# andy-sweet/fcdiff

Hardware: AMD Instinct MI355X
Metric: posterior samples/sec at R=200 ROIs, N=100 subj, 1024 chains; 1/2/4/8 GPUs (higher is better)
Workload: dtype f64

## Files before the change

### fcdiff_amd/csrc/fcd_api.hip

```cpp
#include <new>
#include <stdlib.h>

#include "fcd_common.h"
#include "fcd_fastmath.h"

#ifdef FCD_ABLATE
__device__ int fcd_abl_level[4];
__device__ unsigned long long *fcd_trace_buf;
void fcd_abl_refresh(hipStream_t s) {
    unsigned long long *tp = nullptr;
    if (const char *e = getenv("FCD_TRACE_PTR")) tp = (unsigned long long *)strtoull(e, nullptr, 0);
    (void)hipMemcpyToSymbolAsync(HIP_SYMBOL(fcd_trace_buf), &tp, sizeof(tp), 0, hipMemcpyHostToDevice, s);
    int v[4] = {0, 0, 0, 0};
    if (const char *e = getenv("FCD_ABL_F")) v[0] = atoi(e);
    if (const char *e = getenv("FCD_ABL_PANEL")) v[1] = atoi(e);
    if (const char *e = getenv("FCD_ABL_DIAG")) v[2] = atoi(e);
    if (const char *e = getenv("FCD_TRACE_ROW")) v[3] = atoi(e);
    (void)hipMemcpyToSymbolAsync(HIP_SYMBOL(fcd_abl_level), v, sizeof(v), 0, hipMemcpyHostToDevice, s);
}
#endif

int fcd_ws_reserve(fcd_ctx *ctx, size_t bytes) {
    if (bytes <= ctx->ws_bytes) return FCD_OK;
    FCD_HIP_TRY(hipDeviceSynchronize());
    if (ctx->ws) FCD_HIP_TRY(hipFree(ctx->ws));
    ctx->ws = nullptr;
    ctx->ws_bytes = 0;
    size_t want = bytes < (1u << 20) ? (1u << 20) : bytes;
    FCD_HIP_TRY(hipMalloc(&ctx->ws, want));
    ctx->ws_bytes = want;
    ctx->n_alloc += 1;
    return FCD_OK;
}

int fcd_fsq_reserve(fcd_ctx *ctx, size_t bytes) {
    if (bytes <= ctx->fsq_bytes) return FCD_OK;
    FCD_HIP_TRY(hipDeviceSynchronize());
    if (ctx->fsq) FCD_HIP_TRY(hipFree(ctx->fsq));
    ctx->fsq = nullptr;
    ctx->fsq_bytes = 0;
    FCD_HIP_TRY(hipMalloc(&ctx->fsq, bytes));
    ctx->fsq_bytes = bytes;
    ctx->n_alloc += 1;
    return FCD_OK;
}

int fcd_frec_reserve(fcd_ctx *ctx, size_t bytes) {
    if (bytes <= ctx->frec_bytes) return FCD_OK;
    FCD_HIP_TRY(hipDeviceSynchronize());
    if (ctx->frec) FCD_HIP_TRY(hipFree(ctx->frec));
    ctx->frec = nullptr;
    ctx->frec_bytes = 0;
    FCD_HIP_TRY(hipMalloc(&ctx->frec, bytes));
    ctx->frec_bytes = bytes;
    ctx->n_alloc += 1;
    return FCD_OK;
}

static double knob_env(const char *name) {
    const char *e = getenv(name);
    return (e && *e) ? atof(e) : 0.0;
}

void fcd_prof_begin(fcd_ctx *ctx, int slot, hipStream_t s) {
    if (!ctx->prof_on) return;
    if (ctx->prof_n[slot] >= ctx->prof_cap[slot]) {
        const int cap = ctx->prof_cap[slot] ? ctx->prof_cap[slot] * 2 : 256;
        hipEvent_t *ev = new (std::nothrow) hipEvent_t[2 * cap];
        if (!ev) return;
        for (int i = 0; i < 2 * ctx->prof_cap[slot]; ++i) ev[i] = ctx->prof_ev[slot][i];
        for (int i = 2 * ctx->prof_cap[slot]; i < 2 * cap; ++i)
            if (hipEventCreate(&ev[i]) != hipSuccess) { delete[] ev; return; }
        delete[] ctx->prof_ev[slot];
        ctx->prof_ev[slot] = ev;
        ctx->prof_cap[slot] = cap;
    }
    (void)hipEventRecord(ctx->prof_ev[slot][2 * ctx->prof_n[slot]], s);
}

void fcd_prof_end(fcd_ctx *ctx, int slot, hipStream_t s) {
    if (!ctx->prof_on || ctx->prof_n[slot] >= ctx->prof_cap[slot]) return;
    (void)hipEventRecord(ctx->prof_ev[slot][2 * ctx->prof_n[slot] + 1], s);
    ctx->prof_n[slot] += 1;
}

extern "C" {

int fcd_prof_enable(fcd_ctx *ctx, int on) {
    if (!ctx) return FCD_ERR_ARG;
    ctx->prof_on = on ? 1 : 0;
    for (int i = 0; i < FCD_PROF_SLOTS; ++i) ctx->prof_n[i] = 0;
    return FCD_OK;
}

int fcd_prof_collect(fcd_ctx *ctx, int slot, double *total_ms, int64_t *count) {
    if (!ctx || slot < 0 || slot >= FCD_PROF_SLOTS || !total_ms || !count) return FCD_ERR_ARG;
    double tot = 0.0;
    for (int i = 0; i < ctx->prof_n[slot]; ++i) {
        FCD_HIP_TRY(hipEventSynchronize(ctx->prof_ev[slot][2 * i + 1]));
        float ms = 0.f;
        FCD_HIP_TRY(hipEventElapsedTime(&ms, ctx->prof_ev[slot][2 * i], ctx->prof_ev[slot][2 * i + 1]));
        tot += ms;
    }
    *total_ms = tot;
    *count = ctx->prof_n[slot];
    ctx->prof_n[slot] = 0;
    return FCD_OK;
}

int fcd_abi_version(void) { return FCD_ABI_VERSION; }

const char *fcd_strerror(int code) {
    switch (code) {
        case FCD_OK: return "ok";
        case FCD_ERR_ARG: return "invalid argument (null pointer or non-positive size)";
        case FCD_ERR_SHAPE: return "invalid shape (number of connections must be a triangular number, Nreg >= 2)";
        case FCD_ERR_UNSUPPORTED: return "shape outside what the gfx950 kernels are built for";
        case FCD_ERR_INDEX: return "reference edge id out of range";
        case FCD_ERR_DEVICE: return "a kernel abandoned a device-side wait; the chain state is unusable";
        case FCD_ERR_COMM: return "RCCL: library not found or a call failed";
        default: break;
    }
    if (code > 0) return hipGetErrorString((hipError_t)code);
    return "unknown fcdiff_hip error";
}

const char *fcd_last_message(const fcd_ctx *ctx) { return ctx ? ctx->msg : ""; }

int fcd_ctx_create(fcd_ctx **out) {
    if (!out) return FCD_ERR_ARG;
    *out = nullptr;
    int dev = 0;
    FCD_HIP_TRY(hipGetDevice(&dev));
    hipDeviceProp_t prop;
    FCD_HIP_TRY(hipGetDeviceProperties(&prop, dev));
    fcd_ctx *ctx = new (std::nothrow) fcd_ctx();
    if (!ctx) return (int)hipErrorOutOfMemory;
    ctx->device = dev;
    ctx->num_cu = prop.multiProcessorCount > 0 ? prop.multiProcessorCount : 256;
    ctx->ws = nullptr;
    ctx->ws_bytes = 0;
    ctx->log_tab = nullptr;
    ctx->dev_err = nullptr;
    ctx->f_sure_hint = nullptr;
    ctx->fsq = nullptr;
    ctx->fsq_bytes = 0;
    ctx->frec = nullptr;
    ctx->frec_bytes = 0;
    ctx->noise_rec = nullptr;
    ctx->noise_rec_bytes = 0;
    for (int k = 0; k < FCD_ACC_N; ++k) ctx->sweep_acc[k] = fcd_sweep_acc{{nullptr, nullptr}, 0, 0, 1};
    ctx->count_ws = nullptr;
    ctx->count_ws_bytes = 0;
    ctx->rs_dev = nullptr;
    ctx->rs_J = ctx->rs_smax = 0;
    ctx->rs_max_member = -1;
    ctx->pg_dev = nullptr;
    ctx->pg_J = ctx->pg_P = ctx->pg_umax = ctx->pg_total = ctx->pg_bins_max = 0;
    ctx->pg_max_member = -1;
    ctx->pg_with_rs = 0;
    ctx->pt_dev = nullptr;
    ctx->pt_Q = ctx->pt_U = ctx->pt_umax = 0;
    ctx->pt_with_rs = 0;
    ctx->acc = nullptr;
    ctx->nan_slots = nullptr;
    ctx->dbg = nullptr;
    ctx->comm = nullptr;
    ctx->comm_world = ctx->comm_rank = 0;
    ctx->pool_counts = nullptr;
    ctx->corr_tickets = nullptr;
    ctx->corr_tickets_n = 0;
    ctx->prof_on = 0;
    for (int i = 0; i < FCD_PROF_SLOTS; ++i) {
        ctx->prof_ev[i] = nullptr;
        ctx->prof_n[i] = ctx->prof_cap[i] = 0;
    }
    ctx->msg[0] = 0;
    ctx->n_alloc = 0;
    for (int i = 0; i < FCD_KA_N; ++i) ctx->lds_attr[i] = 0;
    for (int i = 0; i < 3; ++i) ctx->pipe_occ[i] = -1;
    ctx->pipe_grid = ctx->pipe_capacity = 0;
    ctx->knobs.r_path = (int)knob_env("FCD_R_PATH");
    ctx->knobs.r_ub = (int)knob_env("FCD_R_UB");
    ctx->knobs.r_nopad = (int)knob_env("FCD_R_NOPAD");
    ctx->knobs.r_dsplit = (int)knob_env("FCD_R_DSPLIT");
    ctx->knobs.r_coop = (int)knob_env("FCD_R_COOP") == 1 ? 1 : 0;
    ctx->knobs.qr_form = (int)knob_env("FCD_QR_FORM");
    ctx->knobs.r_refill = (int)knob_env("FCD_R_REFILL");
    ctx->knobs.r_tol = knob_env("FCD_R_TOL");
    ctx->knobs.f_tol = knob_env("FCD_F_TOL");
    ctx->knobs.f_form = (int)knob_env("FCD_F_FORM");
    ctx->knobs.f_pack = (int)knob_env("FCD_F_PACK");
    ctx->knobs.corr_form = (int)knob_env("FCD_CORR_FORM");
    ctx->knobs.r_poll_limit = 0;
    ctx->knobs.r_withhold = 0;
    ctx->knobs.f_records = 0;
    ctx->knobs.f_sure = 0;
    ctx->knobs.f_runs = 0;
    ctx->knobs.r_sure = 0;
    ctx->knobs.r_sure_x = 0.0;
    ctx->knobs.partial_chunk = 0;
    ctx->knobs.tangent_chunk = 0;
    ctx->knobs.tally_in_r = (int)knob_env("FCD_TALLY_IN_R");
    ctx->knobs.r_keep_words = (int)knob_env("FCD_R_KEEP_WORDS");
    ctx->r_form_last = 0;
    ctx->n_pack = 0;
    ctx->n_pack_tally = 0;
    ctx->n_r_tally = 0;
    ctx->n_frec_pass = ctx->n_frec_build = ctx->n_fsure_pass = ctx->n_frun_pass = 0;
    ctx->n_rsure_pass = ctx->n_rsure_build = 0;
    int rc = fcd_ws_reserve(ctx, 1u << 20);
    if (rc == FCD_OK) {
        void *pin = nullptr;
        rc = (int)hipHostMalloc(&pin, sizeof(unsigned), hipHostMallocDefault);
        if (rc == FCD_OK) {
            ctx->dev_err = (volatile unsigned *)pin;
            *ctx->dev_err = 0u;
            rc = (int)hipHostMalloc(&pin, 2 * sizeof(unsigned), hipHostMallocDefault);
        }
        if (rc == FCD_OK) {
            ctx->f_sure_hint = (volatile unsigned *)pin;
            ctx->f_sure_hint[0] = 0u;
            ctx->f_sure_hint[1] = 0u;
        }
    }
    if (rc) {
        if (ctx->ws) (void)hipFree(ctx->ws);
        if (ctx->dev_err) (void)hipHostFree((void *)ctx->dev_err);
        if (ctx->f_sure_hint) (void)hipHostFree((void *)ctx->f_sure_hint);
        delete ctx;
        return rc;
    }
    {
        struct { double exp_tab[FCD_EXP_CELLS]; fcd_log_cell log_tab[FCD_LOG_CELLS]; } tabs;
        fcd_fm_make_tables(tabs.exp_tab, tabs.log_tab, exp2, log);
        hipError_t e = hipMalloc(&ctx->log_tab, sizeof(tabs));
        ctx->n_alloc += 1;
        if (e == hipSuccess) e = hipMemcpy(ctx->log_tab, &tabs, sizeof(tabs), hipMemcpyHostToDevice);
        if (e == hipSuccess) e = hipMalloc(&ctx->acc, 8 * sizeof(unsigned long long));
        ctx->n_alloc += 1;
        if (e == hipSuccess) e = hipMemset(ctx->acc, 0, 8 * sizeof(unsigned long long));
        if (e == hipSuccess) e = hipMalloc(&ctx->nan_slots, FCD_NAN_SLOTS * 16 * sizeof(unsigned long long));
        ctx->n_alloc += 1;
        if (e == hipSuccess) e = hipMemset(ctx->nan_slots, 0, FCD_NAN_SLOTS * 16 * sizeof(unsigned long long));
        if (e == hipSuccess) e = hipMalloc(&ctx->dbg, 16 * sizeof(unsigned long long));
        ctx->n_alloc += 1;
        if (e == hipSuccess) e = hipMemset(ctx->dbg, 0, 16 * sizeof(unsigned long long));
        if (e != hipSuccess) {
            fcd_ctx_destroy(ctx);
            return (int)e;
        }
    }
    *out = ctx;
    return FCD_OK;
}

int fcd_ctx_destroy(fcd_ctx *ctx) {
    if (!ctx) return FCD_OK;
    (void)fcd_comm_destroy(ctx);
    if (ctx->pool_counts) (void)hipFree(ctx->pool_counts);
    hipError_t e = hipSuccess;
    if (ctx->ws) e = hipFree(ctx->ws);
    if (ctx->log_tab) (void)hipFree(ctx->log_tab);
    if (ctx->dev_err) (void)hipHostFree((void *)ctx->dev_err);
    if (ctx->f_sure_hint) (void)hipHostFree((void *)ctx->f_sure_hint);
    if (ctx->fsq) (void)hipFree(ctx->fsq);
    if (ctx->frec) (void)hipFree(ctx->frec);
    if (ctx->noise_rec) (void)hipFree(ctx->noise_rec);
    if (ctx->count_ws) (void)hipFree(ctx->count_ws);
    if (ctx->rs_dev) (void)hipFree(ctx->rs_dev);
    if (ctx->pg_dev) (void)hipFree(ctx->pg_dev);
    if (ctx->pt_dev) (void)hipFree(ctx->pt_dev);
    if (ctx->acc) (void)hipFree(ctx->acc);
    if (ctx->nan_slots) (void)hipFree(ctx->nan_slots);
    if (ctx->dbg) (void)hipFree(ctx->dbg);
    if (ctx->corr_tickets) (void)hipFree(ctx->corr_tickets);
    for (int i = 0; i < FCD_PROF_SLOTS; ++i) {
        for (int j = 0; j < 2 * ctx->prof_cap[i]; ++j) (void)hipEventDestroy(ctx->prof_ev[i][j]);
        delete[] ctx->prof_ev[i];
    }
    delete ctx;
    return (int)e;
}

int fcd_ctx_reserve(fcd_ctx *ctx, int64_t Nreg, int64_t U, int64_t G) {
    if (!ctx || Nreg < 2 || U < 1 || G < 1) return fcd_fail(ctx, FCD_ERR_ARG, "fcd_ctx_reserve: bad argument");
    const int64_t GW = (G + 63) / 64;
    size_t need = (size_t)64 * GW * 64 * sizeof(double);
    const size_t en = (size_t)ctx->num_cu * 8 * 8 * sizeof(double);
    if (en > need) need = en;
    const fcd_sweep_plan pl = fcd_sweep_plan_for(ctx, Nreg, U, GW);
    if (pl.ws_bytes > need) need = pl.ws_bytes;
    int rc = fcd_ws_reserve(ctx, need);
    if (rc) return rc;
    if (pl.fsq_bytes) {
        rc = fcd_fsq_reserve(ctx, pl.fsq_bytes);
        if (rc) return rc;
    }
    if (pl.frec_bytes && ctx->knobs.f_records != 1 && fcd_frec_reserve(ctx, pl.frec_bytes) != FCD_OK) (void)hipGetLastError();
    return FCD_OK;
}

int fcd_ctx_set_knob(fcd_ctx *ctx, const char *name, double value) {
    if (!ctx || !name) return FCD_ERR_ARG;
    fcd_knobs &k = ctx->knobs;
    if (!strcmp(name, "r_path")) k.r_path = (int)value;
    else if (!strcmp(name, "r_ub")) k.r_ub = (int)value;
    else if (!strcmp(name, "r_nopad")) k.r_nopad = (int)value;
    else if (!strcmp(name, "r_dsplit")) k.r_dsplit = (int)value;
    else if (!strcmp(name, "r_coop")) k.r_coop = (int)value;
    else if (!strcmp(name, "qr_form")) k.qr_form = (int)value;
    else if (!strcmp(name, "r_refill")) k.r_refill = (int)value;
    else if (!strcmp(name, "r_tol")) k.r_tol = value;
    else if (!strcmp(name, "f_tol")) k.f_tol = value;
    else if (!strcmp(name, "f_form")) k.f_form = (int)value;
    else if (!strcmp(name, "f_pack")) k.f_pack = (int)value;
    else if (!strcmp(name, "f_records")) k.f_records = (int)value;
    else if (!strcmp(name, "f_sure")) k.f_sure = (int)value;
    else if (!strcmp(name, "f_runs")) k.f_runs = (int)value;
    else if (!strcmp(name, "r_sure")) k.r_sure = (int)value;
    else if (!strcmp(name, "r_sure_x")) k.r_sure_x = value;
    else if (!strcmp(name, "corr_form")) k.corr_form = (int)value;
    else if (!strcmp(name, "partial_chunk")) k.partial_chunk = (int)value;
    else if (!strcmp(name, "tangent_chunk")) k.tangent_chunk = (int)value;
    else if (!strcmp(name, "tally_in_r")) k.tally_in_r = (int)value;
    else if (!strcmp(name, "r_keep_words")) k.r_keep_words = (int)value;
    else if (!strcmp(name, "r_poll_limit")) k.r_poll_limit = (int)value;
    else if (!strcmp(name, "r_withhold")) k.r_withhold = (int)value;
    else return fcd_fail(ctx, FCD_ERR_ARG, "fcd_ctx_set_knob: unknown knob");
    return FCD_OK;
}

int fcd_ctx_check(fcd_ctx *ctx) {
    if (!ctx) return FCD_ERR_ARG;
    if (ctx->dev_err && *ctx->dev_err == 2u)
        return fcd_fail(ctx, FCD_ERR_DEVICE, "fcd_site_harmonize: a site id outside 0..B-1 reached the device");
    if (ctx->dev_err && *ctx->dev_err)
        return fcd_fail(ctx, FCD_ERR_DEVICE, "a device-side wait of the pipelined r pass was abandoned: the chain state is unusable");
    return FCD_OK;
}

int fcd_ctx_clear_error(fcd_ctx *ctx) {
    if (!ctx) return FCD_ERR_ARG;
    if (ctx->dev_err) *ctx->dev_err = 0u;
    if (ctx->acc) FCD_HIP_TRY(hipMemset(ctx->acc, 0, 8 * sizeof(unsigned long long)));
    if (ctx->nan_slots) FCD_HIP_TRY(hipMemset(ctx->nan_slots, 0, FCD_NAN_SLOTS * 16 * sizeof(unsigned long long)));
    if (ctx->corr_tickets && ctx->corr_tickets_n > 0)
        FCD_HIP_TRY(hipMemset(ctx->corr_tickets, 0, (size_t)ctx->corr_tickets_n * sizeof(unsigned)));
    return FCD_OK;
}

int fcd_ctx_stat(const fcd_ctx *ctx, const char *name, int64_t *out) {
    if (!ctx || !name || !out) return FCD_ERR_ARG;
    if (!strcmp(name, "n_alloc")) *out = ctx->n_alloc;
    else if (!strcmp(name, "ws_bytes")) *out = (int64_t)ctx->ws_bytes;
    else if (!strcmp(name, "fsq_bytes")) *out = (int64_t)ctx->fsq_bytes;
    else if (!strcmp(name, "r_form_last")) *out = ctx->r_form_last;
    else if (!strcmp(name, "pack_launches")) *out = ctx->n_pack;
    else if (!strcmp(name, "tally_f_in_pack")) *out = ctx->n_pack_tally;
    else if (!strcmp(name, "tally_f_in_r")) *out = ctx->n_r_tally;
    else if (!strcmp(name, "tally_in_r_max_rounds")) *out = R_TALLY_MAX_ROUNDS;
    else if (!strcmp(name, "f_rec_passes")) *out = ctx->n_frec_pass;
    else if (!strcmp(name, "f_rec_builds")) *out = ctx->n_frec_build;
    else if (!strcmp(name, "f_rec_bytes")) *out = (int64_t)ctx->frec_bytes;
    else if (!strcmp(name, "f_rec_min_sweeps")) *out = F_REC_MIN_SWEEPS;
    else if (!strcmp(name, "f_sure_passes")) *out = ctx->n_fsure_pass;
    else if (!strcmp(name, "f_run_passes")) *out = ctx->n_frun_pass;
    else if (!strcmp(name, "r_sure_passes")) *out = ctx->n_rsure_pass;
    else if (!strcmp(name, "r_sure_builds")) *out = ctx->n_rsure_build;
    else if (!strcmp(name, "r_sure_sites") || !strcmp(name, "r_sure_exceptions")) {
        unsigned long long v[16];
        FCD_HIP_TRY(hipMemcpy(v, ctx->dbg, sizeof(v), hipMemcpyDeviceToHost));
        *out = (int64_t)v[!strcmp(name, "r_sure_sites") ? 8 : 9];
    }
    else if (!strcmp(name, "pipe_grid")) *out = ctx->pipe_grid;
    else if (!strcmp(name, "pipe_capacity")) *out = ctx->pipe_capacity;
    else if (!strcmp(name, "comm_world")) *out = ctx->comm ? ctx->comm_world : 0;
    else if (!strcmp(name, "dev_err")) *out = ctx->dev_err ? (int64_t)*ctx->dev_err : 0;
    else if (!strcmp(name, "f_repeats") || !strcmp(name, "r_exact_rows") || !strcmp(name, "f_sure_tiles") || !strcmp(name, "f_sure_fallbacks")) {
        unsigned long long v[8];
        FCD_HIP_TRY(hipMemcpy(v, ctx->dbg, sizeof(v), hipMemcpyDeviceToHost));
        *out = (int64_t)v[name[0] == 'r' ? 1 : !strcmp(name, "f_repeats") ? 0 : !strcmp(name, "f_sure_tiles") ? 2 : 3];
    }
    else return FCD_ERR_ARG;
    return FCD_OK;
}

int64_t fcd_N_to_C(int64_t Nreg) { return fcd_tri(Nreg); }

int64_t fcd_C_to_N(int64_t C) {
    if (C < 1) return FCD_ERR_SHAPE;
    int64_t n = (int64_t)((sqrt(8.0 * (double)C + 1.0) - 1.0) * 0.5) + 1;
    while (fcd_tri(n) > C) --n;
    while (fcd_tri(n + 1) <= C) ++n;
    return fcd_tri(n) == C ? n : (int64_t)FCD_ERR_SHAPE;
}

int64_t fcd_nm_to_c(int64_t n, int64_t m) { return fcd_tri(n) + m; }

int fcd_c_to_nm(int64_t c, int64_t *n, int64_t *m) {
    if (c < 0 || !n || !m) return FCD_ERR_ARG;
    int nn, mm;
    fcd_edge_to_pair(c, nn, mm);
    *n = nn;
    *m = mm;
    return FCD_OK;
}

int64_t fcd_f_run_count(int64_t Nreg) { return Nreg < 2 ? (int64_t)FCD_ERR_SHAPE : fpr_runs((Nreg + 1) / 2); }

int fcd_f_run_locate(int64_t Nreg, int64_t t, int64_t *out9) {
    if (Nreg < 2 || Nreg > (1 << 20) || !out9 || t < 0 || t >= fpr_runs((Nreg + 1) / 2)) return FCD_ERR_ARG;
    const fpr_run R = fpr_locate((int)t, (int)Nreg);
    const int64_t v[9] = {R.n0, R.mb, R.cnt0, R.cnt1, R.tile0, R.ntile, R.cr0, R.cr1, fpr_philox_blocks(R)};
    for (int i = 0; i < 9; ++i) out9[i] = v[i];
    return FCD_OK;
}

}
```

### fcdiff_amd/csrc/fcd_common.h

```cpp
#pragma once
#include <hip/hip_runtime.h>
#include <stdint.h>
#include <stdio.h>
#include <string.h>

#include "../../include/fcdiff_hip.h"

#define FCD_PROF_SLOTS 4
#define FCD_PROF_LIK 0
#define FCD_PROF_F 1
#define FCD_PROF_RSTEP 2
#define FCD_PROF_PACK 3

struct fcd_knobs {
    int r_path;
    int r_ub;
    int r_nopad;
    int r_refill;
    int qr_form;
    int r_coop;
    int r_dsplit;
    double r_tol;
    double f_tol;
    int r_poll_limit;
    int r_withhold;
    int corr_form;
    int f_form;
    int f_pack;
    int f_records;
    int f_sure;
    int f_runs;
    int tally_in_r;
    int partial_chunk;
    int tangent_chunk;
    int r_keep_words;
    int r_sure;
    double r_sure_x;
};

enum { FCD_KA_F_GENERIC = 0, FCD_KA_F_COND, FCD_KA_F_DIFF, FCD_KA_F_PAIR, FCD_KA_F_PAIR_T = FCD_KA_F_PAIR + 4,
       FCD_KA_F_PAIR_R = FCD_KA_F_PAIR_T + 4, FCD_KA_F_PAIR_S = FCD_KA_F_PAIR_R + 4,
       FCD_KA_F_PAIR_BIG = FCD_KA_F_PAIR_S + 4, FCD_KA_R_STEP = FCD_KA_F_PAIR_BIG + 4, FCD_KA_R_PIPE = FCD_KA_R_STEP + 4, FCD_KA_CORR = FCD_KA_R_PIPE + 4, FCD_KA_COMPONENTS = FCD_KA_CORR + 1,
       FCD_KA_GLM = FCD_KA_COMPONENTS + 1,
       FCD_KA_PARTIAL = FCD_KA_GLM + 12,
       FCD_KA_EIGH = FCD_KA_PARTIAL + 1,
       FCD_KA_N = FCD_KA_EIGH + 1 };

#define FCD_NAN_SLOTS 256

enum { FCD_ACC_PAIR, FCD_ACC_COUNT, FCD_ACC_COANOMALY, FCD_ACC_REGION_SET, FCD_ACC_PATIENT_GROUP, FCD_ACC_PATIENT_TRAIT, FCD_ACC_N };
struct fcd_sweep_acc {
    uint32_t *buf[2];
    int64_t nreg, u, every;
};

struct fcd_ctx {
    int device;
    int num_cu;
    void *ws;
    size_t ws_bytes;
    fcd_knobs knobs;
    long long n_alloc;
    size_t lds_attr[FCD_KA_N];
    int pipe_occ[3];
    size_t pipe_occ_shmem[3];
    int pipe_occ_threads[3];
    int64_t pipe_grid;
    int64_t pipe_capacity;
    int r_form_last;
    long long n_pack;
    long long n_pack_tally;
    long long n_r_tally;
    long long n_frec_pass;
    long long n_frec_build;
    long long n_fsure_pass;
    long long n_frun_pass;
    long long n_rsure_pass;
    long long n_rsure_build;
    volatile unsigned *f_sure_hint;
    void *log_tab;
    volatile unsigned *dev_err;
    void *acc;
    void *nan_slots;
    void *comm;
    int comm_world, comm_rank;
    void *pool_counts;
    void *dbg;
    void *corr_tickets;
    size_t corr_tickets_n;
    void *fsq;
    size_t fsq_bytes;
    void *frec;
    size_t frec_bytes;
    void *noise_rec;
    size_t noise_rec_bytes;
    fcd_sweep_acc sweep_acc[FCD_ACC_N];
    void *count_ws;
    size_t count_ws_bytes;
    void *rs_dev;
    int64_t rs_J, rs_smax, rs_max_member;
    void *pg_dev;
    int64_t pg_J, pg_P, pg_umax, pg_max_member;
    int64_t pg_total, pg_bins_max;
    int pg_with_rs;
    void *pt_dev;
    int64_t pt_Q, pt_U, pt_umax;
    int pt_with_rs;
    int prof_on;
    hipEvent_t *prof_ev[FCD_PROF_SLOTS];
    int prof_n[FCD_PROF_SLOTS];
    int prof_cap[FCD_PROF_SLOTS];
    char msg[256];
};

#define FCD_HIP_TRY(expr)                       \
    do {                                        \
        hipError_t e__ = (expr);                \
        if (e__ != hipSuccess) return (int)e__; \
    } while (0)

#define FCD_LAUNCH_CHECK()                      \
    do {                                        \
        hipError_t e__ = hipGetLastError();     \
        if (e__ != hipSuccess) return (int)e__; \
    } while (0)

static inline int fcd_fail(fcd_ctx *ctx, int code, const char *fmt, long long a = 0, long long b = 0) {
    if (ctx) snprintf(ctx->msg, sizeof(ctx->msg), fmt, a, b);
    return code;
}
static inline int fcd_fail_who(fcd_ctx *ctx, int code, const char *who, const char *fmt, long long a = 0, long long b = 0) {
    if (ctx) {
        char tail[192];
        snprintf(tail, sizeof(tail), fmt, a, b);
        snprintf(ctx->msg, sizeof(ctx->msg), "%s: %s", who, tail);
    }
    return code;
}

static inline int fcd_sweep_acc_set(fcd_ctx *ctx, int slot, uint32_t *b0, uint32_t *b1, int64_t Nreg, int64_t U, int64_t every,
                                    const char *msg_together, const char *msg_shape, const char *msg_limit,
                                    const char *msg_every) {
    if (!ctx) return FCD_ERR_ARG;
    if (!b0 && !b1) {
        ctx->sweep_acc[slot] = fcd_sweep_acc{{nullptr, nullptr}, 0, 0, 1};
        return FCD_OK;
    }
    if (!b0 || !b1) return fcd_fail(ctx, FCD_ERR_ARG, msg_together);
    if (Nreg < 2 || U < 1) return fcd_fail(ctx, FCD_ERR_SHAPE, msg_shape, Nreg, U);
    if (msg_limit) return fcd_fail(ctx, FCD_ERR_UNSUPPORTED, msg_limit, Nreg, U);
    if (every < 1) return fcd_fail(ctx, FCD_ERR_ARG, msg_every, every);
    ctx->sweep_acc[slot] = fcd_sweep_acc{{b0, b1}, Nreg, U, every};
    return FCD_OK;
}

static inline int fcd_static_lds_check(fcd_ctx *ctx, const void *fn, int *done) {
    if (*done) return FCD_OK;
    hipFuncAttributes fa;
    hipError_t e = hipFuncGetAttributes(&fa, fn);
    if (e != hipSuccess) return (int)e;
    if (fa.sharedSizeBytes != 0) {
        return fcd_fail(ctx, FCD_ERR_UNSUPPORTED, "kernel carries %lld bytes of static LDS: its table addresses assume none",
                        (long long)fa.sharedSizeBytes);
    }
    *done = 1;
    return FCD_OK;
}

int fcd_comm_allreduce_counts(fcd_ctx *ctx, long long *counts, hipStream_t stream);
int fcd_ws_reserve(fcd_ctx *ctx, size_t bytes);
int fcd_corr_edges_at(fcd_ctx *ctx, const double *ts, int64_t S, int64_t Nreg, int64_t T, int fisher_z, double *out, size_t ws_off,
                      int64_t S_slices, hipStream_t stream);
size_t fcd_corr_edges_ws_bytes(const fcd_ctx *ctx, int64_t S, int64_t Nreg, int64_t T, int64_t S_slices);
struct fcd_shrunk_ws {
    size_t o_redge, o_A, o_live, o_rowF, o_F, o_mean, o_isd, o_q, end;
    int PL, RT, NBT;
};
void fcd_corr_shrunk_plan(int64_t SC, int64_t Nreg, int64_t T, size_t base, fcd_shrunk_ws &w, bool with_A = true);
int fcd_corr_shrunk_at(fcd_ctx *ctx, const double *x, int64_t Sc, int64_t Nreg, int64_t T, const int32_t *n_frames, int64_t s0,
                       int64_t S_call, int shrink_mode, double shrink_value, const fcd_shrunk_ws &w, size_t edges_off, double *A,
                       double *alpha, int32_t *info, hipStream_t stream);
int fcd_fsq_reserve(fcd_ctx *ctx, size_t bytes);
int fcd_frec_reserve(fcd_ctx *ctx, size_t bytes);
static inline int fcd_lds_attr(fcd_ctx *ctx, int slot, const void *fn, size_t shmem) {
    if (shmem <= 64 * 1024 || shmem <= ctx->lds_attr[slot]) return FCD_OK;
    hipError_t e = hipFuncSetAttribute(fn, hipFuncAttributeMaxDynamicSharedMemorySize, (int)shmem);
    if (e != hipSuccess) return (int)e;
    ctx->lds_attr[slot] = shmem;
    return FCD_OK;
}
struct fcd_tally_f {
    const uint8_t *f_state;
    int64_t C, G;
    int GW;
    unsigned long long *acc;
    uint32_t *cnt_f;
};
constexpr int R_TALLY_MAX_ROUNDS = 5;
struct fcd_geo;
template <typename T>
int fcd_pair_tally_launch(fcd_ctx *ctx, const uint8_t *f_state, const uint64_t *r_bits, int64_t Nreg, int64_t U, int64_t G,
                          const fcd_geo &g, T *acc, bool accumulate, hipStream_t s);
int fcd_count_ws_reserve(fcd_ctx *ctx, int64_t Nreg, int64_t U, int64_t G);
int fcd_count_ws_grow(fcd_ctx *ctx, size_t bytes);
int fcd_count_tally_launch(fcd_ctx *ctx, const uint64_t *r_bits, int64_t Nreg, int64_t U, int64_t G, const fcd_geo &g,
                           uint32_t *hist_patient, uint32_t *hist_region, hipStream_t s);
int fcd_coanomaly_tally_launch(fcd_ctx *ctx, const uint64_t *r_bits, int64_t Nreg, int64_t U, int64_t G, const fcd_geo &g,
                               uint32_t *region_pairs, uint32_t *patient_pairs, hipStream_t s);
int fcd_region_set_ws_reserve(fcd_ctx *ctx, int64_t Nreg, int64_t U, int64_t G);
int fcd_region_set_tally_launch(fcd_ctx *ctx, const uint64_t *r_bits, int64_t Nreg, int64_t U, int64_t G, const fcd_geo &g,
                                uint32_t *hist_set, uint32_t *hist_prev, hipStream_t s);
int fcd_patient_group_ws_reserve(fcd_ctx *ctx, int64_t Nreg, int64_t U, int64_t G);
int fcd_patient_group_tally_launch(fcd_ctx *ctx, const uint64_t *r_bits, int64_t Nreg, int64_t U, int64_t G, const fcd_geo &g,
                                   uint32_t *hist_group, uint32_t *hist_joint, hipStream_t s);
int fcd_patient_trait_ws_reserve(fcd_ctx *ctx, int64_t Nreg, int64_t U, int64_t G);
int fcd_patient_trait_tally_launch(fcd_ctx *ctx, const uint64_t *r_bits, int64_t Nreg, int64_t U, int64_t G, const fcd_geo &g,
                                   uint32_t *trait_hist, int64_t *trait_sum, hipStream_t s);
void fcd_prof_begin(fcd_ctx *ctx, int slot, hipStream_t s);
void fcd_prof_end(fcd_ctx *ctx, int slot, hipStream_t s);

#define FCD_H_LNGAMMA 0
#define FCD_H_LNPI0 3
#define FCD_H_LNPI1 4

#define FCD_KIND_INIT_F 0u
#define FCD_KIND_INIT_R 1u
#define FCD_KIND_F 2u
#define FCD_KIND_R 3u

__host__ __device__ static inline int64_t fcd_tri(int64_t n) { return n * (n - 1) / 2; }

__host__ __device__ static inline void fcd_edge_to_pair(int64_t c, int &n, int &m) {
    int64_t nn = (int64_t)((sqrt(8.0 * (double)c + 1.0) - 1.0) * 0.5) + 1;
    while (fcd_tri(nn) > c) --nn;
    while (fcd_tri(nn + 1) <= c) ++nn;
    n = (int)nn;
    m = (int)(c - fcd_tri(nn));
}

__host__ __device__ static inline int64_t fcd_pair_to_edge(int n, int m, int mode) {
    if (mode == FCD_EDGE_REFERENCE || n > m) return fcd_tri(n) + m;
    return fcd_tri(m) + n;
}

struct fcd_u4 {
    uint32_t x, y, z, w;
};

__host__ __device__ static inline fcd_u4 fcd_philox(uint32_t c0, uint32_t c1, uint32_t c2, uint32_t c3,
                                                    uint32_t k0, uint32_t k1) {
#pragma unroll
    for (int r = 0; r < 10; ++r) {
        uint64_t p0 = (uint64_t)0xD2511F53u * c0;
        uint64_t p1 = (uint64_t)0xCD9E8D57u * c2;
        uint32_t n0 = (uint32_t)(p1 >> 32) ^ c1 ^ k0;
        uint32_t n1 = (uint32_t)p1;
        uint32_t n2 = (uint32_t)(p0 >> 32) ^ c3 ^ k1;
        uint32_t n3 = (uint32_t)p0;
        c0 = n0; c1 = n1; c2 = n2; c3 = n3;
        k0 += 0x9E3779B9u;
        k1 += 0xBB67AE85u;
    }
    return fcd_u4{c0, c1, c2, c3};
}

__host__ __device__ static inline double fcd_u53(uint32_t hi, uint32_t lo) {
    uint64_t w = ((uint64_t)hi << 32) | lo;
    return (double)(w >> 11) * (1.0 / 9007199254740992.0);
}

__host__ __device__ static inline double fcd_u32(uint32_t w) { return (double)w * (1.0 / 4294967296.0); }
__host__ __device__ static inline uint32_t fcd_word(const fcd_u4 &x, int i) { return i == 0 ? x.x : i == 1 ? x.y : i == 2 ? x.z : x.w; }

__host__ __device__ static inline double fcd_site_uniform(uint64_t seed, uint32_t idx, uint32_t chain,
                                                          uint32_t sweep, uint32_t kind, int half) {
    fcd_u4 x = fcd_philox(idx, chain, sweep, kind, (uint32_t)seed, (uint32_t)(seed >> 32));
    return half ? fcd_u53(x.z, x.w) : fcd_u53(x.x, x.y);
}

__device__ static inline int fcd_draw_f(double a0, double a1, double a2, double x) {
    double mx = fmax(a0, fmax(a1, a2));
    double e0 = exp(a0 - mx), e1 = exp(a1 - mx), e2 = exp(a2 - mx);
    double t = x * ((e0 + e1) + e2);
    return (t < e0) ? 0 : ((t < e0 + e1) ? 1 : 2);
}

#define FCD_DRAW_F_MARGIN 1e-6f
__host__ __device__ static inline float fcd_draw_f_eta(float delta) { return expm1f(2.0f * delta) * 1.001f + 2e-5f; }
__device__ static inline int fcd_draw_f_fast(double b1, double b2, double x, float eta, float floor_rel, bool *amb) {
    const double mx = fmax(0.0, fmax(b1, b2));
    const float e0 = __expf((float)(0.0 - mx)), e1 = __expf((float)(b1 - mx)), e2 = __expf((float)(b2 - mx));
    const float s = (e0 + e1) + e2;
    const float t = (float)x * s;
    const float m = 2.0f * eta * (s - 1.0f) + floor_rel * s;
    *amb = !(fabsf(t - e0) >= m && fabsf(t - (e0 + e1)) >= m);
    return (t < e0) ? 0 : ((t < e0 + e1) ? 1 : 2);
}
__device__ static inline int fcd_draw_f_fast32(float bf1, float bf2, float xf, float eta, float floor_rel, bool *amb) {
    const float mx = fmaxf(0.f, fmaxf(bf1, bf2));
    const float e0 = __expf(0.f - mx), e1 = __expf(bf1 - mx), e2 = __expf(bf2 - mx);
    const float s = (e0 + e1) + e2;
    const float t = xf * s;
    const float m = 2.0f * eta * (s - 1.0f) + floor_rel * s;
    *amb = !(fabsf(t - e0) >= m && fabsf(t - (e0 + e1)) >= m);
    return (t < e0) ? 0 : ((t < e0 + e1) ? 1 : 2);
}
__device__ static inline bool fcd_draw_f_sure(float bf1, float bf2, float xf, float eta, int *k) {
    const float mx = fmaxf(0.f, fmaxf(bf1, bf2)), mn = fminf(0.f, fminf(bf1, bf2));
    const float mid = ((bf1 + bf2) - mx) - mn;
    *k = (bf2 >= mx) ? 2 : ((bf1 >= mx) ? 1 : 0);
    return (mx - mid) - eta > 15.01f && xf > 1e-6f && xf < 0.999999f;
}
__host__ __device__ static inline float fcd_f32_sum_err(int n_terms, float B) { return (float)(n_terms + 1) * 5.97e-8f * 1.01f * B; }
__host__ __device__ static inline float fcd_f32_offset_err(float cm, float B) { return 2.0f * 5.97e-8f * 1.01f * (cm + B); }

__device__ static inline double fcd_logit(double x) { return log(x / (1.0 - x)); }
__device__ static inline int fcd_draw_r(double s0, double s1, double x) { return fcd_logit(x) < (s1 - s0) ? 1 : 0; }
#define FCD_LOGIT_FAST_ERR 2e-5
__device__ static inline double fcd_logit_fast(double x) {
    const float a = __log2f((float)x), b = __log2f((float)(1.0 - x));
    return (double)((a - b) * 0.69314718f);
}

__device__ static inline double fcd_wave_sum(double v) {
#pragma unroll
    for (int o = 32; o > 0; o >>= 1) v += __shfl_xor(v, o, 64);
    return v;
}

__device__ static inline uint32_t fcd_sel_mask(uint32_t a, uint32_t b, uint64_t mask) {
    uint32_t out;
    asm("v_cndmask_b32 %0, %1, %2, %3" : "=v"(out) : "v"(a), "v"(b), "s"(mask));
    return out;
}

__host__ __device__ static inline uint64_t fcd_active_mask(int w, int64_t G) {
    const int64_t rem = G - (int64_t)w * 64;
    return rem >= 64 ? ~0ull : ((1ull << rem) - 1ull);
}

#ifdef __HIPCC__
constexpr int R_NB = 16;
__device__ __forceinline__ uint2 spread2(uint32_t x16) {
    uint32_t lo = x16 & 0xFFu, hi = (x16 >> 8) & 0xFFu;
    lo = (lo | (lo << 12)) & 0x000F000Fu;
    hi = (hi | (hi << 12)) & 0x000F000Fu;
    lo = (lo | (lo << 6)) & 0x03030303u;
    hi = (hi | (hi << 6)) & 0x03030303u;
    return make_uint2(lo, hi);
}
__device__ __forceinline__ uint64_t fcd_lane_word(uint64_t v, int j) {
    const uint32_t lo = (uint32_t)__builtin_amdgcn_readlane((int)(uint32_t)v, j);
    const uint32_t hi = (uint32_t)__builtin_amdgcn_readlane((int)(uint32_t)(v >> 32), j);
    return ((uint64_t)hi << 32) | lo;
}
__device__ __forceinline__ uint2 fcd_r_pair_bytes(const uint64_t *__restrict__ r_bits, int Nreg, int U, int w, int u, int b,
                                                  int lane) {
    const int ml = b * R_NB + (lane & (R_NB - 1));
    const uint64_t mine = r_bits[((int64_t)w * Nreg + (ml < Nreg ? ml : Nreg - 1)) * U + u];
    uint32_t v = 0;
#pragma unroll
    for (int j = 0; j < R_NB; ++j) {
        const int m = b * R_NB + j;
        v |= (m < Nreg ? (uint32_t)((fcd_lane_word(mine, j) >> lane) & 1ull) : 0u) << j;
    }
    return spread2(v);
}

template <int CTRL>
__device__ __forceinline__ uint32_t fcd_dpp_u32(uint32_t v) {
    return (uint32_t)__builtin_amdgcn_update_dpp(0, (int)v, CTRL, 0xF, 0xF, false);
}
__device__ __forceinline__ uint32_t fcd_wave_sum4(const uint32_t (&p)[4], int lane) {
    const bool b0 = lane & 1, b1 = lane & 2;
    const uint32_t x01 = (b0 ? p[1] : p[0]) + fcd_dpp_u32<0xB1>(b0 ? p[0] : p[1]);
    const uint32_t x23 = (b0 ? p[3] : p[2]) + fcd_dpp_u32<0xB1>(b0 ? p[2] : p[3]);
    uint32_t y = (b1 ? x23 : x01) + fcd_dpp_u32<0x4E>(b1 ? x01 : x23);
    y += fcd_dpp_u32<0x124>(y);
    y += fcd_dpp_u32<0x128>(y);
    y += __shfl_xor(y, 16, 64);
    y += __shfl_xor(y, 32, 64);
    return y;
}

template <int WAVES>
__device__ __forceinline__ void fcd_tally_f_block(const fcd_tally_f &a, int lin, int nblk, unsigned long long (*red)[3]) {
    const uint8_t *__restrict__ f_state = a.f_state;
    uint32_t *cnt_f = a.cnt_f;
    const int64_t C = a.C, G = a.G;
    const int GW = a.GW;
    const int lane = threadIdx.x & 63, wave = __builtin_amdgcn_readfirstlane((int)(threadIdx.x >> 6));
    const int sub = lane & 3, wrow = lane >> 2;
    unsigned long long tot1 = 0, tot2 = 0, n_edges = 0;
    const int own_e = ((lane * 11) >> 5) & 3, own_j = lane - 3 * own_e;
    constexpr int TE = 4;
    for (int64_t c0 = ((int64_t)lin * WAVES + wave) * TE; c0 < C; c0 += (int64_t)nblk * WAVES * TE) {
        const int ne = (int)(C - c0 < TE ? C - c0 : TE);
        const bool owner = cnt_f && lane < 3 * ne;
        uint32_t old = 0;
        if (owner) old = cnt_f[c0 * 3 + lane];
        uint32_t s1 = 0, s2 = 0;
        for (int wg = 0; wg < GW; wg += 16) {
            const int w = wg + wrow;
            uint4 vv[TE];
#pragma unroll
            for (int t = 0; t < TE; ++t) {
                const int64_t c = (c0 + t < C) ? c0 + t : C - 1;
                vv[t] = *reinterpret_cast<const uint4 *>(f_state + ((int64_t)(w < GW ? w : 0) * C + c) * 64 + sub * 16);
            }
            const uint32_t act = (w < GW) ? (uint32_t)(fcd_active_mask(w, G) >> (sub * 16)) & 0xFFFFu : 0u;
            uint32_t p[TE];
#pragma unroll
            for (int t = 0; t < TE; ++t) {
                uint4 v = vv[t];
                if (act != 0xFFFFu) {
                    v.x &= (((act & 15u) * 0x00204081u) & 0x01010101u) * 0xFFu;
                    v.y &= ((((act >> 4) & 15u) * 0x00204081u) & 0x01010101u) * 0xFFu;
                    v.z &= ((((act >> 8) & 15u) * 0x00204081u) & 0x01010101u) * 0xFFu;
                    v.w &= ((((act >> 12) & 15u) * 0x00204081u) & 0x01010101u) * 0xFFu;
                }
                const uint32_t ones = __popc(v.x & 0x01010101u) + __popc(v.y & 0x01010101u) + __popc(v.z & 0x01010101u) +
                                      __popc(v.w & 0x01010101u);
                const uint32_t twos = __popc(v.x & 0x02020202u) + __popc(v.y & 0x02020202u) + __popc(v.z & 0x02020202u) +
                                      __popc(v.w & 0x02020202u);
                p[t] = ones | (twos << 16);
            }
            const uint32_t s = fcd_wave_sum4(p, lane);
            s1 += s & 0xFFFFu;
            s2 += s >> 16;
        }
#pragma unroll
        for (int t = 0; t < TE; ++t) {
            if (t < ne) {
                tot1 += (uint32_t)__builtin_amdgcn_readlane((int)s1, t);
                tot2 += (uint32_t)__builtin_amdgcn_readlane((int)s2, t);
            }
        }
        const uint32_t ones = __shfl(s1, own_e, 64), twos = __shfl(s2, own_e, 64);
        const uint32_t add = own_j == 0 ? (uint32_t)G - ones - twos : (own_j == 1 ? ones : twos);
        n_edges += (unsigned long long)ne;
        if (owner) cnt_f[c0 * 3 + lane] = old + add;
    }
    if (!a.acc) return;
    if (lane == 0) {
        red[wave][0] = n_edges * (unsigned long long)G - tot1 - tot2;
        red[wave][1] = tot1;
        red[wave][2] = tot2;
    }
    __syncthreads();
    if (threadIdx.x < 3) {
        unsigned long long t = 0;
        for (int q = 0; q < WAVES; ++q) t += red[q][threadIdx.x];
        if (t) {
            const unsigned long long old = atomicAdd(&a.acc[1 + threadIdx.x], t);
            asm volatile("" ::"v"(old));
        }
    }
    __syncthreads();
}
#endif

struct fcd_geo {
    int64_t C;
    int GW;
};

static inline int fcd_geo_check(fcd_ctx *ctx, int64_t Nreg, int64_t U, int64_t G, int64_t chain0, fcd_geo &g) {
    if (!ctx) return FCD_ERR_ARG;
    if (Nreg < 2 || U < 1 || G < 1)
        return fcd_fail(ctx, FCD_ERR_SHAPE, "need Nreg >= 2, U >= 1, G >= 1 (Nreg=%lld, U=%lld)", Nreg, U);
    if (Nreg > 46340 || U > (1 << 20) || G > (1ll << 31) || chain0 < 0 || chain0 + G > (1ll << 32))
        return fcd_fail(ctx, FCD_ERR_UNSUPPORTED, "shape out of range (Nreg=%lld, G=%lld)", Nreg, G);
    g.C = fcd_tri(Nreg);
    g.GW = (int)((G + 63) / 64);
    if (g.GW > 65535) return fcd_fail(ctx, FCD_ERR_UNSUPPORTED, "G=%lld exceeds 65535 chain words per launch", G);
    if ((Nreg + 1) / 2 * U > (1ll << 32) || (g.C + 1) / 2 > (1ll << 32))
        return fcd_fail(ctx, FCD_ERR_UNSUPPORTED, "site index exceeds the 32-bit counter word");
    return FCD_OK;
}

enum { FCD_F_GENERIC = 0, FCD_F_PAIR = 1, FCD_F_PAIRX = 2, FCD_F_DIFF = 3 };
constexpr int FP_EC = 8;
constexpr int FT_W = FP_EC / 2;
__host__ __device__ static inline int64_t fpt_tiles(int64_t i) {
    const int64_t j = i >> 1;
    return (i & 1) ? (j + 1) * (j + 1) : j * (j + 1);
}
constexpr int FR_W = 4 * FT_W;
constexpr int FR_WAVES = 8;
struct fpr_run {
    int n0, mb;
    int cnt0, cnt1;
    int tile0, ntile;
    int64_t cr0, cr1;
};
__host__ __device__ static inline int64_t fpr_runs(int64_t i) {
    const int64_t q = i >> 3;
    return 4 * q * (q + 1) + (i & 7) * (q + 1);
}
__host__ __device__ static inline fpr_run fpr_locate(int t, int Nreg) {
    int q = (int)((sqrtf((float)t + 1.f) - 1.f) * 0.5f);
    while ((int64_t)4 * (q + 1) * (q + 2) <= t) ++q;
    while ((int64_t)4 * q * (q + 1) > t) --q;
    const int rem = t - 4 * q * (q + 1);
    const int i = 8 * q + rem / (q + 1);
    fpr_run R;
    R.n0 = 2 * i;
    R.mb = FR_W * (rem % (q + 1));
    const int c0 = R.n0 - R.mb, c1 = R.n0 + 1 - R.mb;
    R.cnt0 = c0 < FR_W ? c0 : FR_W;
    R.cnt1 = R.n0 + 1 < Nreg ? (c1 < FR_W ? c1 : FR_W) : 0;
    R.tile0 = (int)fpt_tiles(i) + R.mb / FT_W;
    R.ntile = ((c1 + 1 < FR_W ? c1 + 1 : FR_W) + FT_W - 1) / FT_W;
    R.cr0 = ((int64_t)R.n0 * (R.n0 - 1) >> 1) + R.mb;
    R.cr1 = R.cr0 + R.n0;
    return R;
}
__host__ __device__ static inline int fpr_philox_blocks(const fpr_run &R) {
    int n = 0;
    if (R.cnt0 > 0) n += (int)(((R.cr0 + R.cnt0 - 1) >> 2) - (R.cr0 >> 2)) + 1;
    if (R.cnt1 > 0) n += (int)(((R.cr1 + R.cnt1 - 1) >> 2) - (R.cr1 >> 2)) + 1;
    return n;
}
constexpr int F_REC_PIECES = 6;
struct fcd_f_edge_rec {
    double d1, d2;
    float a;
    float b[6];
    float pad;
};
#define FCD_F_SURE_T 16.0
#define FCD_F_SURE_DELTA_CAP 0.03125f
#define FCD_F_SURE_DRIFT 6.0
__host__ __device__ static inline int fcd_f_edge_mode(double c1, double c2, const float *b, float delta, double T) {
    if (!(delta <= FCD_F_SURE_DELTA_CAP)) return -1;
    const double c12 = c1 - c2;
    if (-(c1 + (double)b[1]) > T && -(c2 + (double)b[3]) > T) return 0;
    if (c1 + (double)b[0] > T && c12 + (double)b[4] > T) return 1;
    if (c2 + (double)b[2] > T && -(c12 + (double)b[5]) > T) return 2;
    return -1;
}
__host__ __device__ static inline float fcd_f_edge_delta(double c1, double c2, int NPAIR, float a) {
    const float cm = fmaxf((float)fabs(c1), (float)fabs(c2)) * 1.0000002f;
    return fcd_f32_sum_err(NPAIR, a) + fcd_f32_offset_err(cm, a);
}
constexpr size_t F_REC_CAP = (size_t)256 << 20;
constexpr int F_REC_MIN_SWEEPS = 10;
struct fcd_sweep_plan {
    int f_form, f_EC;
    size_t f_shmem;
    int f_NW;
    bool r_blocked, r_idx32;
    int r_ub;
    size_t r_shmem;
    size_t fsq_bytes;
    size_t frec_bytes, frec_edge, frec_votes, f_shmem_rec;
    size_t P[2], f_S, r_S, r_Sn, marks, r_U, ws_bytes;
    size_t rs_bnd, rs_dtab, rs_mword, rs_rowflag, rs_visit, rs_fneq, rs_bytes;
};
fcd_sweep_plan fcd_sweep_plan_for(const fcd_ctx *ctx, int64_t Nreg, int64_t U, int64_t GW);
struct fcd_sweep_call {
    const double *S_B, *lM, *lMf, *lMd, *hyper;
    uint8_t *f_state;
    uint64_t *r_bits;
    int64_t Nreg, U, G, chain0;
    uint64_t seed;
    int edge_mode;
    hipStream_t s;
    fcd_geo g;
    fcd_sweep_plan pl;
};
int fcd_sweep_call_check(fcd_ctx *ctx, fcd_sweep_call &c, bool f_pass, bool r_pass, const char *who);
struct fcd_sweep_step {
    int64_t sweep;
    uint8_t *fsq;
    bool f_packed;
    bool r_packed;
    bool ru_ready;
    const void *f_rec;
    bool sentinels_in_place;
    const fcd_tally_f *tally_f;
    bool tally_f_done;
    bool r_flip;
    bool f_sure;
    bool f_all;
    bool r_sure;
};
int fcd_gibbs_f_pass(fcd_ctx *ctx, const fcd_sweep_call &c, const fcd_sweep_step &st);
int fcd_gibbs_r_pass(fcd_ctx *ctx, const fcd_sweep_call &c, fcd_sweep_step &st);
#define R_SURE_T 16.0
#define R_SURE_X 1e-6
constexpr double R_SURE_MIN_SHARE = 0.9;
int fcd_gibbs_r_bounds_build(fcd_ctx *ctx, const fcd_sweep_call &c);

#ifdef FCD_ABLATE
extern __device__ int fcd_abl_level[4];
#ifdef FCD_TRACE_ONLY
#define FCD_ABL(slot, lvl) false
#else
#define FCD_ABL(slot, lvl) (fcd_abl_level[slot] >= (lvl))
#endif
void fcd_abl_refresh(hipStream_t s);
extern __device__ unsigned long long *fcd_trace_buf;
#define FCD_TRACE(rec, slot)                                                                      \
    do {                                                                                          \
        if (fcd_trace_buf && threadIdx.x == 0) fcd_trace_buf[(size_t)(rec) * 8 + (slot)] = wall_clock64(); \
    } while (0)
#define FCD_TRACE_VAL(rec, slot, v)                                                               \
    do {                                                                                          \
        if (fcd_trace_buf && threadIdx.x == 0) fcd_trace_buf[(size_t)(rec) * 8 + (slot)] = (unsigned long long)(v); \
    } while (0)
#define FCD_TRACE_AT(t0, rec, slot)                                                               \
    do {                                                                                          \
        if (fcd_trace_buf && threadIdx.x == (t0)) fcd_trace_buf[(size_t)(rec) * 8 + (slot)] = wall_clock64(); \
    } while (0)
#define FCD_TRACE_VAL_AT(t0, rec, slot, v)                                                        \
    do {                                                                                          \
        if (fcd_trace_buf && threadIdx.x == (t0)) fcd_trace_buf[(size_t)(rec) * 8 + (slot)] = (unsigned long long)(v); \
    } while (0)
#else
#define FCD_ABL(slot, lvl) false
#define FCD_TRACE(rec, slot) do { } while (0)
#define FCD_TRACE_VAL(rec, slot, v) do { } while (0)
#define FCD_TRACE_AT(t0, rec, slot) do { } while (0)
#define FCD_TRACE_VAL_AT(t0, rec, slot, v) do { } while (0)
static inline void fcd_abl_refresh(hipStream_t) {}
#endif
```

### fcdiff_amd/csrc/fcd_gibbs.hip

```cpp
#include "fcd_common.h"
#include <chrono>

namespace {

__global__ __launch_bounds__(256) void gibbs_init_f(uint8_t *__restrict__ f_state, int64_t C, int GW, uint32_t chain0,
                                                    uint64_t seed) {
    const int lane = threadIdx.x & 63;
    const int64_t item = (int64_t)blockIdx.x * 4 + (threadIdx.x >> 6);
    const int64_t n_pairs = (C + 1) / 2;
    if (item >= n_pairs * GW) return;
    const int w = (int)(item / n_pairs);
    const int64_t pr = item % n_pairs;
    const uint32_t chain = chain0 + (uint32_t)w * 64u + lane;
    const fcd_u4 x = fcd_philox((uint32_t)pr, chain, 0u, FCD_KIND_INIT_F, (uint32_t)seed, (uint32_t)(seed >> 32));
    const int f0 = min((int)(fcd_u53(x.x, x.y) * 3.0), 2);
    const int f1 = min((int)(fcd_u53(x.z, x.w) * 3.0), 2);
    const int64_t c = pr * 2;
    f_state[((int64_t)w * C + c) * 64 + lane] = (uint8_t)f0;
    if (c + 1 < C) f_state[((int64_t)w * C + c + 1) * 64 + lane] = (uint8_t)f1;
}

__global__ __launch_bounds__(256) void gibbs_init_r(uint64_t *__restrict__ r_bits, int Nreg, int U, int GW,
                                                    uint32_t chain0, uint64_t seed, double pi) {
    const int lane = threadIdx.x & 63;
// ... 735 lines not shown
#ifdef FCD_ABLATE
    FCD_TRACE_VAL(trec, 4, tr_terms);
    FCD_TRACE_VAL(trec, 5, tr_draw);
    FCD_TRACE_VAL(trec, 6, tr_rest);
#endif
    FCD_TRACE(trec, 3);
}

__global__ __launch_bounds__(64 * FP_EC) void gibbs_f_records_kernel(const double *__restrict__ S_B, const double *__restrict__ lMf,
                                                                     const double *__restrict__ hyper, int Nreg, int U,
                                                                     char *__restrict__ frec, unsigned *__restrict__ any_tile,
                                                                     unsigned *__restrict__ votes, int n_votes) {
    const int NPAIR = (U + 1) >> 1;
    const fpt_tile T = fpt_locate((int)blockIdx.x, Nreg);
    for (int i = (int)(blockIdx.x * blockDim.x + threadIdx.x); i < n_votes; i += (int)(gridDim.x * blockDim.x)) votes[i] = 0u;
    auto has = [&](int e) -> bool { return (e % FT_W) < (e < FT_W ? T.cnt0 : T.cnt1); };
    auto cid = [&](int e) -> int64_t { return (e < FT_W ? T.cr0 : T.cr1) + (e % FT_W); };
    fcd_f4v *dst4 = reinterpret_cast<fcd_f4v *>(frec) + (size_t)blockIdx.x * NPAIR * (FP_EC * F_REC_PIECES);
    for (int ep = threadIdx.x; ep < FP_EC * NPAIR; ep += blockDim.x) {
        const int e = ep / NPAIR, pr = ep - e * NPAIR;
        if (!has(e)) continue;
        const int u = 2 * pr;
        const double2 *su = reinterpret_cast<const double2 *>(lMf + cid(e) * U * 6) + u * 3;
        double2 A[3], B[3];
#pragma unroll
        for (int l = 0; l < 3; ++l) {
            A[l] = su[l];
            B[l] = (u + 1 < U) ? su[3 + l] : make_double2(0.0, 0.0);
        }
#pragma unroll
        for (int s2 = 0; s2 < 8; ++s2)
            if (s2 != 5 && s2 != 7) dst4[(pr * FP_EC + e) * F_REC_PIECES + (s2 < 5 ? s2 : 5)] = fp_pair_piece(A, B, s2);
    }
    const int e = (int)(threadIdx.x >> 6), lane = threadIdx.x & 63;
    __shared__ int open_edges;
    if (threadIdx.x == 0) open_edges = 0;
    __syncthreads();
    if (has(e)) {
        const int64_t c = cid(e);
        const double2 *su = reinterpret_cast<const double2 *>(lMf + c * U * 6) + (lane < U ? lane : 0) * 3;
        const float a = fp_edge_bound(su, lane < U);
        double b[6] = {0.0, 0.0, 0.0, 0.0, 0.0, 0.0};
        bool finite = true;
        if (lane < U) {
#pragma unroll
            for (int l = 0; l < 3; ++l) {
                const double v[3] = {su[l].x, su[l].y, su[l].x - su[l].y};
                finite = finite && isfinite(v[0]) && isfinite(v[1]);
#pragma unroll
                for (int q = 0; q < 3; ++q) {
                    b[2 * q] = l == 0 ? v[q] : fmin(b[2 * q], v[q]);
                    b[2 * q + 1] = l == 0 ? v[q] : fmax(b[2 * q + 1], v[q]);
                }
            }
        }
        finite = __ballot(!finite) == 0ull;
#pragma unroll
        for (int q = 0; q < 6; ++q) b[q] = fcd_wave_sum(b[q]);
        if (lane == 0) {
            fcd_f_edge_rec k = {};
            const double sb0 = S_B[c * 3 + 0];
            k.d1 = S_B[c * 3 + 1] - sb0;
            k.d2 = S_B[c * 3 + 2] - sb0;
            k.a = a;
            const double slack = 8e-15 * (double)a;
#pragma unroll
            for (int q = 0; q < 6; ++q)
                k.b[q] = !finite ? __builtin_nanf("") : (q & 1) ? __double2float_ru(b[q] + slack) : __double2float_rd(b[q] - slack);
            reinterpret_cast<fcd_f_edge_rec *>(frec + (size_t)gridDim.x * NPAIR * (FP_EC * F_REC_PIECES * 16))[c] = k;
            const double c1 = (hyper[FCD_H_LNGAMMA + 1] - hyper[FCD_H_LNGAMMA + 0]) + k.d1;
            const double c2 = (hyper[FCD_H_LNGAMMA + 2] - hyper[FCD_H_LNGAMMA + 0]) + k.d2;
            if (fcd_f_edge_mode(c1, c2, k.b, fcd_f_edge_delta(c1, c2, NPAIR, a), FCD_F_SURE_T - FCD_F_SURE_DRIFT) < 0) open_edges = 1;
        }
    }
    __syncthreads();
    if (threadIdx.x == 0 && (T.cnt0 > 0 || T.cnt1 > 0)) any_tile[open_edges ? 1 : 0] = 1u;
}
__global__ void gibbs_f_hint_kernel(unsigned *__restrict__ any_tile, volatile unsigned *hint, unsigned build, const double *lM,
                                    const double *hyper) {
    const unsigned any = any_tile[0] != 0u ? 1u : 0u, all = (any && any_tile[1] == 0u) ? 1u : 0u;
    any_tile[0] = 0u;
    any_tile[1] = 0u;
    reinterpret_cast<unsigned long long *>(any_tile)[1] = (unsigned long long)(uintptr_t)lM;
    reinterpret_cast<unsigned long long *>(any_tile)[2] = (unsigned long long)(uintptr_t)hyper;
    for (int i = 0; i < 5; ++i) reinterpret_cast<double *>(any_tile)[7 + i] = hyper[i];
    __hip_atomic_store(const_cast<unsigned *>(hint), 4u * build + 2u * all + any, __ATOMIC_RELEASE, __HIP_MEMORY_SCOPE_SYSTEM);
}

constexpr int FPR_AMB = 8;
__device__ __attribute__((noinline)) int fcd_f_run_edge(const char *__restrict__ rec, const fcd_f_edge_rec *__restrict__ ke_p,
                                                        const double *__restrict__ hyper, uint4 Z, int U, uint32_t xw, float margin) {
    const int NPAIR = (U + 1) >> 1, NG = (NPAIR + 7) >> 3;
    auto term = [&](int p, uint32_t slot) -> fcd_f2v {
        const uint32_t s2 = slot >> 1;
        return *reinterpret_cast<const fcd_f2v *>(rec + (size_t)p * (FP_EC * F_REC_PIECES * 16) + (s2 < 5 ? s2 : 5) * 16 + (slot & 1u) * 8);
    };
    fcd_f2v acc = {0.f, 0.f}, acc1 = {0.f, 0.f};
#pragma unroll 1
    for (int g = 0; g < NG; ++g) {
        const uint32_t zs = g == 0 ? Z.x : g == 1 ? Z.y : g == 2 ? Z.z : Z.w;
        const int np = NPAIR - 8 * g;
        if (np >= 8) {
#pragma unroll 1
            for (int p = 0; p < 8; p += 2) {
                const fcd_f2v v0 = term(8 * g + p, (zs >> (4 * p)) & 15u), v1 = term(8 * g + p + 1, (zs >> (4 * p + 4)) & 15u);
                if (g == 0 && p == 0) {
                    acc = v0;
                    acc1 = v1;
                } else {
                    acc += v0;
                    acc1 += v1;
                }
            }
        } else {
#pragma unroll 1
            for (int p = 0; p < np; ++p) acc += term(8 * g + p, (zs >> (4 * p)) & 15u);
        }
    }
    acc += acc1;
    const fcd_f_edge_rec ke = *ke_p;
    const double lg1 = hyper[FCD_H_LNGAMMA + 1] - hyper[FCD_H_LNGAMMA + 0], lg2 = hyper[FCD_H_LNGAMMA + 2] - hyper[FCD_H_LNGAMMA + 0];
    const double c1 = lg1 + ke.d1, c2 = lg2 + ke.d2;
    const float cm = fmaxf((float)fabs(c1), (float)fabs(c2)) * 1.0000002f;
    const float eta = fcd_draw_f_eta(fcd_f32_sum_err(NPAIR, ke.a) + fcd_f32_offset_err(cm, ke.a));
    const float bf1 = (float)c1 + acc.x, bf2 = (float)c2 + acc.y, xf = (float)xw * 2.3283064e-10f;
    bool amb = false;
    int k;
    if (margin > 1.f || __ballot(!fcd_draw_f_sure(bf1, bf2, xf, eta, &k)) != 0ull) k = fcd_draw_f_fast32(bf1, bf2, xf, eta, margin, &amb);
    return k | (__ballot(amb) != 0ull ? FPR_AMB : 0);
}

__device__ __forceinline__ uint32_t fpr_spread16(uint32_t m) {
    m = (m | (m << 8)) & 0x00FF00FFu;
    m = (m | (m << 4)) & 0x0F0F0F0Fu;
    m = (m | (m << 2)) & 0x33333333u;
    return (m | (m << 1)) & 0x55555555u;
}
__device__ __forceinline__ uint2 fpr_row_word(uint32_t K) {
    const uint32_t v = 3u * (K & 0x33333333u) + ((K >> 2) & 0x33333333u);
    uint32_t lo = v & 0xFFFFu, hi = v >> 16;
    lo = (lo | (lo << 8)) & 0x00FF00FFu;
    hi = (hi | (hi << 8)) & 0x00FF00FFu;
    lo = (lo | (lo << 4)) & 0x0F0F0F0Fu;
    hi = (hi | (hi << 4)) & 0x0F0F0F0Fu;
    return make_uint2(lo << 2, hi << 2);
}

__global__ __launch_bounds__(64 * FR_WAVES) void gibbs_f_run_kernel(const double *__restrict__ S_B, const double *__restrict__ lMf,
                                                           const double *__restrict__ hyper, uint8_t *__restrict__ f_state,
                                                           const uint32_t *__restrict__ r_U, int Nreg, int U, int64_t C, int GW,
                                                           uint32_t chain0, uint64_t seed, uint32_t sweep, float margin,
                                                           uint2 *__restrict__ f_S, int NBLK, unsigned long long *__restrict__ dbg,
                                                           const char *__restrict__ frec, const double *__restrict__ lM, int n_tiles,
                                                           unsigned *__restrict__ votes) {
    static_assert(16 % FR_WAVES == 0, "a workgroup's chain words lie in one group of 16");
    static_assert(FR_W == R_NB && FR_W == 16 && FT_W == 4, "a run is one block of the r pass's f words: sixteen columns, four tiles");
    __shared__ uint32_t vote[FR_WAVES];
    const int NPAIR = (U + 1) >> 1;
    const fpr_run R = fpr_locate((int)blockIdx.x, Nreg);
    const int lane = threadIdx.x & 63;
    const int wv = (int)(threadIdx.x >> 6);
    const int w = __builtin_amdgcn_readfirstlane((int)(blockIdx.y * (blockDim.x >> 6)) + wv);
    const size_t rec_tile = (size_t)NPAIR * (FP_EC * F_REC_PIECES * 16);
    const fcd_f_edge_rec *edge_c = reinterpret_cast<const fcd_f_edge_rec *>(frec + (size_t)n_tiles * rec_tile);
    const int lr = (lane >> 4) & 1, lj = lane & (FR_W - 1);
    const bool present = lane < 2 * FR_W && lj < (lr ? R.cnt1 : R.cnt0);
    int mode = -1;
    if (present) {
        const fcd_f_edge_rec k = edge_c[(lr ? R.cr1 : R.cr0) + lj];
        const double c1 = (hyper[FCD_H_LNGAMMA + 1] - hyper[FCD_H_LNGAMMA + 0]) + k.d1;
        const double c2 = (hyper[FCD_H_LNGAMMA + 2] - hyper[FCD_H_LNGAMMA + 0]) + k.d2;
        mode = fcd_f_edge_mode(c1, c2, k.b, fcd_f_edge_delta(c1, c2, NPAIR, k.a), FCD_F_SURE_T);
    }
    const uint32_t pm = (uint32_t)__ballot(present), dm = (uint32_t)__ballot(mode >= 0);
    const uint32_t m1 = (uint32_t)__ballot(mode == 1), m2 = (uint32_t)__ballot(mode == 2);
    uint32_t oe = 0;
    if (w < GW) {
        const uint32_t chain = chain0 + (uint32_t)w * 64u + lane;
        uint32_t out = 0;
#pragma unroll
        for (int r = 0; r < 2; ++r) {
            const int cnt = r ? R.cnt1 : R.cnt0;
            if (cnt == 0) continue;
            const int64_t cr = r ? R.cr1 : R.cr0;
            const int64_t b1 = (cr + cnt - 1) >> 2;
#pragma unroll 1
            for (int64_t b = cr >> 2; b <= b1; ++b) {
                const fcd_u4 rnd = fcd_philox((uint32_t)b, chain, sweep, FCD_KIND_F, (uint32_t)seed, (uint32_t)(seed >> 32));
                const int j0 = (int)(4 * b - cr);
#pragma unroll
                for (int q = 0; q < 4; ++q) {
                    const float xf = (float)fcd_word(rnd, q) * 2.3283064e-10f;
                    const bool bad = !(xf > 1e-6f && xf < 0.999999f);
                    if (bad && j0 + q >= 0 && j0 + q < cnt) out |= 1u << (FR_W * r + j0 + q);
                }
            }
        }
        if (__ballot(out != 0u) != 0ull) {
#pragma unroll
            for (int o = 32; o > 0; o >>= 1) out |= (uint32_t)__shfl_xor((int)out, o, 64);
            oe = (uint32_t)__builtin_amdgcn_readfirstlane((int)out);
        }
        uint32_t K0 = (fpr_spread16(m1 & 0xFFFFu) | (fpr_spread16(m2 & 0xFFFFu) << 1));
        uint32_t K1 = (fpr_spread16(m1 >> 16) | (fpr_spread16(m2 >> 16) << 1));
        const uint32_t X = (pm & ~dm) | oe;
        if (__builtin_expect(X != 0u, 0)) {
            const uint4 *__restrict__ ru = reinterpret_cast<const uint4 *>(r_U) + (int64_t)w * Nreg * 64;
            uint32_t x = X;
#pragma unroll 1
            while (x != 0u) {
                const int e = __builtin_ctz(x);
                x &= x - 1u;
                const int r = e >> 4, j = e & (FR_W - 1);
                const int64_t c = (r ? R.cr1 : R.cr0) + j;
                const char *rec = frec + (size_t)(R.tile0 + j / FT_W) * rec_tile + (size_t)(r * FT_W + j % FT_W) * (F_REC_PIECES * 16);
                const fcd_u4 rnd = fcd_philox((uint32_t)(c >> 2), chain, sweep, FCD_KIND_F, (uint32_t)seed, (uint32_t)(seed >> 32));
                const uint32_t xw = fcd_word(rnd, (int)(c & 3));
                const int n = R.n0 + r, m = R.mb + j;
                const uint4 vn = ru[(uint32_t)(n * 64) + (uint32_t)lane], vm = ru[(uint32_t)(m * 64) + (uint32_t)lane];
                const uint4 Z = make_uint4((vn.x ^ vm.x) | ((vn.x & vm.x) << 2), (vn.y ^ vm.y) | ((vn.y & vm.y) << 2),
                                           (vn.z ^ vm.z) | ((vn.z & vm.z) << 2), (vn.w ^ vm.w) | ((vn.w & vm.w) << 2));
                uint32_t k = (uint32_t)fcd_f_run_edge(rec, edge_c + c, hyper, Z, U, xw, margin);
                if (k & FPR_AMB) {
                    const double lg1 = hyper[FCD_H_LNGAMMA + 1] - hyper[FCD_H_LNGAMMA + 0], lg2 = hyper[FCD_H_LNGAMMA + 2] - hyper[FCD_H_LNGAMMA + 0];
                    k = (uint32_t)fcd_f_exact_edge(lMf + c * U * 6, lg1 + (S_B[c * 3 + 1] - S_B[c * 3 + 0]), lg2 + (S_B[c * 3 + 2] - S_B[c * 3 + 0]),
                                                   Z.x, Z.y, Z.z, Z.w, U, xw);
                    if (lane == 0) atomicAdd(dbg, 1ull);
                    const bool open = (k & FCD_F_OPEN) != 0;
                    k &= 3u;
                    if (__ballot(open) != 0ull) {
                        const uint32_t ka = (uint32_t)fcd_f_abs_edge(lM, S_B, hyper, ru, c, n, m, U, chain, sweep, seed);
                        if (open) k = ka;
                    }
                }
                if (r) K1 = (K1 & ~(3u << (2 * j))) | (k << (2 * j));
                else K0 = (K0 & ~(3u << (2 * j))) | (k << (2 * j));
            }
        }
#pragma unroll
        for (int r = 0; r < 2; ++r) {
            const int cnt = r ? R.cnt1 : R.cnt0;
            if (cnt == 0) continue;
            uint8_t *line = f_state + ((int64_t)w * C + (r ? R.cr1 : R.cr0)) * 64;
            const uint32_t Kr = r ? K1 : K0;
            if (((X >> (FR_W * r)) & 0xFFFFu) == 0u) {
                if ((lane >> 2) < cnt) {
                    const uint32_t v = ((Kr >> (2 * (lane >> 2))) & 3u) * 0x01010101u;
                    reinterpret_cast<uint4 *>(line)[lane] = make_uint4(v, v, v, v);
                }
            } else {
#pragma unroll 1
                for (int j = 0; j < cnt; ++j) (line + j * 64)[(uint32_t)lane] = (uint8_t)((Kr >> (2 * j)) & 3u);
            }
        }
        if (f_S) {
            const bool full = R.n0 + 2 - R.mb >= FR_W;
            if (full) {
                const int jd = R.n0 + 1 - R.mb;
                const uint32_t K0d = jd < FR_W ? K0 | (((K1 >> (2 * (jd - 1))) & 3u) << (2 * jd)) : K0;
                uint2 *word = f_S + (int64_t)w * Nreg * NBLK * 64 + lane;
                word[(int64_t)(R.n0 * NBLK + R.mb / R_NB) * 64] = fpr_row_word(K0d);
                if (R.n0 + 1 < Nreg) word[(int64_t)((R.n0 + 1) * NBLK + R.mb / R_NB) * 64] = fpr_row_word(K1);
            }
#pragma unroll 1
            for (int q = 0; q < R.ntile; ++q) {
                fpt_tile T;
                T.n0 = R.n0;
                T.mb = R.mb + FT_W * q;
                T.cnt0 = min(FT_W, T.n0 - T.mb);
                T.cnt1 = T.n0 + 1 < Nreg ? min(FT_W, T.n0 + 1 - T.mb) : 0;
                T.cr0 = R.cr0 + FT_W * q;
                T.cr1 = R.cr1 + FT_W * q;
                const uint32_t kt = ((K0 >> (8 * q)) & 0xFFu) | (((K1 >> (8 * q)) & 0xFFu) << 8);
                if (full) fpt_write_f_words<false>(T, kt, w, lane, f_S, Nreg, NBLK);
                else fpt_write_f_words<true>(T, kt, w, lane, f_S, Nreg, NBLK);
            }
        }
    }
    uint32_t ot = 0;
#pragma unroll
    for (int q = 0; q < 4; ++q)
        if (oe & (0x000F000Fu << (FT_W * q))) ot |= 1u << q;
    if (lane == 0) vote[wv] = ot;
    __syncthreads();
    if (wv == 0) {
        const uint32_t v = lane < (int)(blockDim.x >> 6) ? vote[lane & (FR_WAVES - 1)] : 0u;
        uint32_t bm = 0;
#pragma unroll
        for (int q = 0; q < 4; ++q)
            if (__ballot((v >> q) & 1u) != 0ull) bm |= 1u << q;
        const int w0 = (int)(blockIdx.y * (blockDim.x >> 6)), wpg = (int)(blockDim.x >> 6);
        const int n_wg = (min(16, GW - (w0 & ~15)) + wpg - 1) / wpg;
        bool last = true;
        if (n_wg > 1) {
            uint32_t all = 0;
            if (lane == 0) {
                unsigned *word = votes + (size_t)blockIdx.x * (size_t)((GW + 15) >> 4) + (size_t)(w0 >> 4);
                const uint32_t mine = 0x10000u | (bm << (4 * ((w0 & 15) / wpg)));
                all = atomicAdd(word, mine) + mine;
                if ((int)(all >> 16) == n_wg) atomicExch(word, 0u);
            }
            all = (uint32_t)__builtin_amdgcn_readfirstlane((int)all);
            last = (int)(all >> 16) == n_wg;
            bm = (all | (all >> 4) | (all >> 8) | (all >> 12)) & 15u;
        }
        uint32_t n_sure = 0, n_back = 0;
#pragma unroll
        for (int q = 0; q < 4; ++q) {
            const uint32_t tm = (0x000F000Fu << (FT_W * q)) & pm;
            if (last && tm != 0u && (tm & ~dm) == 0u) {
                if ((bm >> q) & 1u) n_back += 1;
                else n_sure += 1;
            }
        }
        if (lane == 0) {
            if (n_sure) atomicAdd(dbg + 2, (unsigned long long)n_sure);
            if (n_back) atomicAdd(dbg + 3, (unsigned long long)n_back);
        }
    }
}

template <int EC>
__global__ __launch_bounds__(1024, 8) void gibbs_f_pairx_kernel(const double *__restrict__ S_B, const double *__restrict__ lMf,
                                                                const double *__restrict__ hyper, uint8_t *__restrict__ f_state,
                                                                const uint32_t *__restrict__ r_U, int Nreg, int U, int64_t C,
                                                                int GW, uint32_t chain0, uint64_t seed, uint32_t sweep,
                                                                float margin, uint8_t *__restrict__ fsq,
                                                                unsigned long long *__restrict__ dbg, const double *__restrict__ lM) {
    extern __shared__ __attribute__((aligned(256))) double ptile[];
    const int NPAIR = (U + 1) >> 1, NW16 = (U + 15) >> 4;
    const int64_t c0 = (int64_t)blockIdx.x * EC;
    const int ne = (int)((C - c0 < EC) ? (C - c0) : EC);
    const int lane = threadIdx.x & 63;
    const int w = __builtin_amdgcn_readfirstlane((int)(blockIdx.y * (blockDim.x >> 6) + (threadIdx.x >> 6)));
    int wn, wm;
    fcd_edge_to_pair(c0, wn, wm);
    const uint32_t *__restrict__ ru = r_U + (int64_t)(w < GW ? w : 0) * Nreg * (NW16 <= 4 ? 4 : NW16) * 64;
    const uint32_t ul = (uint32_t)lane;
    const uint32_t sn = NW16 <= 4 ? 256u : (uint32_t)NW16 * 64u, sg = NW16 <= 4 ? 1u : 64u, lo = NW16 <= 4 ? ul * 4u : ul;
    auto ruw = [&](int n, int g) -> uint32_t { return ru[(uint32_t)n * sn + (uint32_t)g * sg + lo]; };
    uint32_t rn_c = ruw(wn, 0), rm_c = ruw(wm, 0);
    float4 *edge_k = reinterpret_cast<float4 *>(reinterpret_cast<char *>(ptile) + (size_t)EC * NPAIR * 128);
    if (threadIdx.x < EC) edge_k[threadIdx.x] = make_float4(0.f, 0.f, 0.f, 0.f);
    __syncthreads();
    {
        const int wv = (int)(threadIdx.x >> 6);
        double2 *scratch = reinterpret_cast<double2 *>(reinterpret_cast<char *>(edge_k) + 128) + wv * (2 * 24);
        fcd_f2v *dst = reinterpret_cast<fcd_f2v *>(ptile);
        const int slot = lane & 15, pl = lane >> 4;
        const int x0 = slot & 1, x1 = (slot >> 1) & 1, a0 = (slot >> 2) & 1, a1 = slot >> 3;
        const bool valid = !((x0 & a0) | (x1 & a1));
        const int l0 = a0 ? 1 : (x0 ? 2 : 0), l1 = a1 ? 1 : (x1 ? 2 : 0);
        const int NG4 = (NPAIR + 3) >> 2;
        const int groups = ne * NG4, nwv = (int)(blockDim.x >> 6);
        const int row_d2 = U * 3;
        const double2 *__restrict__ src = reinterpret_cast<const double2 *>(lMf + c0 * U * 6);
        for (int g0 = wv; g0 < groups; g0 += 2 * nwv) {
            double2 v[2];
            int eq[2][2];
#pragma unroll
            for (int t = 0; t < 2; ++t) {
                const int g = g0 + t * nwv;
                const int gc = g < groups ? g : groups - 1;
                const int e = gc / NG4, q = gc - e * NG4;
                eq[t][0] = e;
                eq[t][1] = q;
                const int i2 = q * 24 + lane;
                if (lane < 24 && i2 < row_d2) {
                    const double *p2 = reinterpret_cast<const double *>(src + (e * row_d2 + i2));
                    v[t] = make_double2(__builtin_nontemporal_load(p2), __builtin_nontemporal_load(p2 + 1));
                } else {
                    v[t] = make_double2(0.0, 0.0);
                }
            }
#pragma unroll
            for (int t = 0; t < 2; ++t)
                if (lane < 24) scratch[t * 24 + lane] = v[t];
            __builtin_amdgcn_fence(__ATOMIC_RELEASE, "wavefront");
            __builtin_amdgcn_wave_barrier();
            __builtin_amdgcn_fence(__ATOMIC_ACQUIRE, "wavefront");
#pragma unroll
            for (int t = 0; t < 2; ++t) {
                const int g = g0 + t * nwv;
                const int pr = eq[t][1] * 4 + pl;
                const double2 va = scratch[t * 24 + pl * 6 + l0], vb = scratch[t * 24 + pl * 6 + 3 + l1];
                fcd_f2v r = {0.f, 0.f};
                if (valid) {
                    r.x = (float)(va.x + vb.x);
                    r.y = (float)(va.y + vb.y);
                }
                if (g < groups && pr < NPAIR) dst[(eq[t][0] * NPAIR + pr) * 16 + slot] = r;
                if (g < groups && lane < 8) {
                    float a = 0.f;
#pragma unroll
                    for (int l = 0; l < 3; ++l) {
                        const double2 q = scratch[t * 24 + lane * 3 + l];
                        a = fmaxf(a, fmaxf((float)fabs(q.x), (float)fabs(q.y)));
                    }
                    atomicAdd(&edge_k[eq[t][0]].w, a * 1.0000002f);
                }
            }
            __builtin_amdgcn_fence(__ATOMIC_RELEASE, "wavefront");
            __builtin_amdgcn_wave_barrier();
            __builtin_amdgcn_fence(__ATOMIC_ACQUIRE, "wavefront");
        }
    }
    __syncthreads();
    const double lg1 = hyper[FCD_H_LNGAMMA + 1] - hyper[FCD_H_LNGAMMA + 0];
    const double lg2 = hyper[FCD_H_LNGAMMA + 2] - hyper[FCD_H_LNGAMMA + 0];
    if ((int)threadIdx.x < ne) {
        const int64_t c = c0 + threadIdx.x;
        const double c1 = lg1 + (S_B[c * 3 + 1] - S_B[c * 3 + 0]), c2 = lg2 + (S_B[c * 3 + 2] - S_B[c * 3 + 0]);
        const float cm = fmaxf((float)fabs(c1), (float)fabs(c2)) * 1.0000002f;
        const float a = edge_k[threadIdx.x].w;
        edge_k[threadIdx.x] = make_float4((float)c1, (float)c2, fcd_draw_f_eta(fcd_f32_sum_err(NPAIR + 1, a) + fcd_f32_offset_err(cm, a)), 0.f);
    }
    __syncthreads();
    if (w >= GW) return;
    if (FCD_ABL(0, 3)) return;
    const uint32_t chain = chain0 + (uint32_t)w * 64u + lane;
    const uint32_t k0 = (uint32_t)seed, k1 = (uint32_t)(seed >> 32);
    fcd_u4 rnd = {0, 0, 0, 0};
    const int NG = (NPAIR + 7) >> 3;
    const uint32_t tile_off = (uint32_t)(uintptr_t)(__attribute__((address_space(3))) char *)ptile;

    for (int e = 0; e < ne; ++e) {
        const int64_t c = c0 + e;
        int nn = wn, nm = wm + 1;
        if (nm == nn) {
            nm = 0;
            nn = (nn + 1 < Nreg) ? nn + 1 : nn;
        }
        const uint32_t tb = __builtin_amdgcn_readfirstlane(tile_off + (uint32_t)(e * NPAIR * 128));
        fcd_f2v acc = {0.f, 0.f}, acc1 = {0.f, 0.f};
        for (int g = 0; g < NG; ++g) {
            const bool last = g + 1 == NG;
            const int pn = last ? nn : wn, pm = last ? nm : wm, pg = last ? 0 : g + 1;
// ... 232 lines not shown
    }
    partial[((int64_t)s * GW + w) * 64 + lane] = acc;
}

__global__ __launch_bounds__(64) void gibbs_rsum_kernel(const uint64_t *__restrict__ r_bits, int64_t NU, int64_t G,
                                                        unsigned int *__restrict__ out) {
    const int w = blockIdx.x, lane = threadIdx.x;
    const uint64_t *rw = r_bits + (int64_t)w * NU;
    unsigned int ones = 0;
    for (int64_t i = blockIdx.y; i < NU; i += gridDim.y) ones += (unsigned int)((rw[i] >> lane) & 1ull);
    const int64_t g = (int64_t)w * 64 + lane;
    if (g < G && ones) atomicAdd(&out[g], ones);
}

__global__ void gibbs_logjoint_fold(const double *__restrict__ partial, int64_t GWx64, int64_t G, double *__restrict__ out) {
    const int64_t g = (int64_t)blockIdx.x * blockDim.x + threadIdx.x;
    if (g >= G) return;
    double acc = 0.0;
    for (int s = 0; s < LJ_SLICES; ++s) acc += partial[(int64_t)s * GWx64 + g];
    out[g] = acc;
}

__global__ void export_f_kernel(const uint8_t *__restrict__ f_state, int64_t C, int64_t G, uint8_t *__restrict__ f) {
    const int64_t i = (int64_t)blockIdx.x * blockDim.x + threadIdx.x;
    if (i >= G * C) return;
    const int64_t g = i / C, c = i % C;
    f[i] = f_state[((g >> 6) * C + c) * 64 + (g & 63)];
}
__global__ void export_r_kernel(const uint64_t *__restrict__ r_bits, int64_t NU, int64_t G, uint8_t *__restrict__ r) {
    const int64_t i = (int64_t)blockIdx.x * blockDim.x + threadIdx.x;
    if (i >= G * NU) return;
    const int64_t g = i / NU, j = i % NU;
    r[i] = (uint8_t)((r_bits[(g >> 6) * NU + j] >> (g & 63)) & 1ull);
}
__global__ void import_f_kernel(const uint8_t *__restrict__ f, int64_t C, int64_t G, int GW, uint8_t *__restrict__ f_state) {
    const int64_t i = (int64_t)blockIdx.x * blockDim.x + threadIdx.x;
    if (i >= (int64_t)GW * C * 64) return;
    const int64_t lane = i & 63, c = (i >> 6) % C, w = (i >> 6) / C;
    const int64_t g = w * 64 + lane;
    f_state[i] = g < G ? f[g * C + c] : 0;
}
__global__ __launch_bounds__(256) void import_r_kernel(const uint8_t *__restrict__ r, int64_t NU, int64_t G, int GW,
                                                       uint64_t *__restrict__ r_bits) {
    const int lane = threadIdx.x & 63;
    const int64_t word = (int64_t)blockIdx.x * 4 + (threadIdx.x >> 6);
    if (word >= (int64_t)GW * NU) return;
    const int64_t w = word / NU, j = word % NU;
    const int64_t g = w * 64 + lane;
    const uint64_t ball = __ballot(g < G ? (r[g * NU + j] != 0) : false);
    if (lane == 0) r_bits[word] = ball;
}

__global__ void philox_uniforms_kernel(const uint32_t *__restrict__ ctr4, int64_t n, uint64_t seed, double *__restrict__ out) {
    const int64_t i = (int64_t)blockIdx.x * blockDim.x + threadIdx.x;
    if (i >= n) return;
    const fcd_u4 x = fcd_philox(ctr4[i * 4 + 0], ctr4[i * 4 + 1], ctr4[i * 4 + 2], ctr4[i * 4 + 3], (uint32_t)seed,
                                (uint32_t)(seed >> 32));
    out[i * 2 + 0] = fcd_u53(x.x, x.y);
    out[i * 2 + 1] = fcd_u53(x.z, x.w);
}

void f_step_geometry(int64_t U, int GW, int &Ec, int &wpb, size_t &shmem) {
    wpb = GW < 16 ? GW : 16;
    const size_t per_edge = (size_t)U * 72;
    int64_t e = (int64_t)(32 * 1024 / per_edge);
    if (e < 1) e = 1;
    if (e > 8) e = 8;
    if (e > 1) e &= ~1ll;
    Ec = (int)e;
    shmem = per_edge * Ec;
}

template <bool COND>
int launch_f(fcd_ctx *ctx, const double *S_B, const double *lM, const double *hyper, uint8_t *f_state,
             const uint64_t *r_bits, int64_t Nreg, int64_t U, int64_t G, const fcd_geo &g, int64_t chain0, uint64_t seed,
             int64_t sweep, double *cond_f, hipStream_t s) {
    int Ec, wpb;
    size_t shmem;
    f_step_geometry(U, g.GW, Ec, wpb, shmem);
    if (shmem > 160 * 1024)
        return fcd_fail(ctx, FCD_ERR_UNSUPPORTED, "f step: one edge's table row (U=%lld patients) exceeds the 160 KiB LDS", U);
    {
        int rc = fcd_lds_attr(ctx, COND ? FCD_KA_F_COND : FCD_KA_F_GENERIC, reinterpret_cast<const void *>(&gibbs_f_kernel<COND>), shmem);
        if (rc) return rc;
    }
    dim3 grid((unsigned)((g.C + Ec - 1) / Ec), (unsigned)((g.GW + wpb - 1) / wpb));
    hipLaunchKernelGGL(gibbs_f_kernel<COND>, grid, dim3(64 * wpb), shmem, s, S_B, lM, hyper, f_state, r_bits, (int)Nreg,
                       (int)U, g.C, g.GW, G, Ec, (uint32_t)chain0, seed, (uint32_t)sweep, cond_f);
    FCD_LAUNCH_CHECK();
    return FCD_OK;
}

}

extern "C" int fcd_gibbs_state_size(int64_t Nreg, int64_t U, int64_t G, size_t *f_bytes, size_t *r_bytes) {
    if (Nreg < 2 || U < 1 || G < 1 || !f_bytes || !r_bytes) return FCD_ERR_ARG;
    const int64_t GW = (G + 63) / 64;
    *f_bytes = (size_t)(GW * fcd_tri(Nreg) * 64);
    *r_bytes = (size_t)(GW * Nreg * U * 8);
    return FCD_OK;
}

extern "C" int fcd_gibbs_init(fcd_ctx *ctx, uint8_t *f_state, uint64_t *r_bits, int64_t Nreg, int64_t U, int64_t G,
                              int64_t chain0, uint64_t seed, double pi, fcd_stream stream) {
    fcd_geo g;
    int rc = fcd_geo_check(ctx, Nreg, U, G, chain0, g);
    if (rc) return rc;
    if (!f_state || !r_bits) return fcd_fail(ctx, FCD_ERR_ARG, "fcd_gibbs_init: null pointer");
    hipStream_t s = (hipStream_t)stream;
    const int64_t items_f = (g.C + 1) / 2 * g.GW;
    hipLaunchKernelGGL(gibbs_init_f, dim3((unsigned)((items_f + 3) / 4)), dim3(256), 0, s, f_state, g.C, g.GW,
                       (uint32_t)chain0, seed);
    FCD_LAUNCH_CHECK();
    const int64_t items_r = (Nreg + 1) / 2 * U * g.GW;
    hipLaunchKernelGGL(gibbs_init_r, dim3((unsigned)((items_r + 3) / 4)), dim3(256), 0, s, r_bits, (int)Nreg, (int)U, g.GW,
                       (uint32_t)chain0, seed, pi);
    FCD_LAUNCH_CHECK();
    return FCD_OK;
}

extern "C" int fcd_gibbs_edge_tables(fcd_ctx *ctx, const double *lM, int64_t Nreg, int64_t U, double *lMf,
                                     fcd_stream stream) {
    if (!ctx || !lM || !lMf) return fcd_fail(ctx, FCD_ERR_ARG, "fcd_gibbs_edge_tables: null pointer");
    if (Nreg < 2 || U < 1) return fcd_fail(ctx, FCD_ERR_SHAPE, "need Nreg >= 2 and U >= 1 (Nreg=%lld, U=%lld)", Nreg, U);
    const int64_t n_items = fcd_tri(Nreg) * U;
    int64_t blocks = (n_items + 255) / 256;
    const int64_t cap = (int64_t)ctx->num_cu * 16;
    if (blocks > cap) blocks = cap;
    hipLaunchKernelGGL(edge_tables_kernel, dim3((unsigned)blocks), dim3(256), 0, (hipStream_t)stream, lM, n_items, lMf);
    FCD_LAUNCH_CHECK();
    return FCD_OK;
}

int fcd_sweep_call_check(fcd_ctx *ctx, fcd_sweep_call &c, bool f_pass, bool r_pass, const char *who) {
    int rc = fcd_geo_check(ctx, c.Nreg, c.U, c.G, c.chain0, c.g);
    if (rc) return rc;
    const bool null = (f_pass && !c.S_B) || !c.lM || !c.hyper || !c.f_state || !c.r_bits;
    if (null || (r_pass && c.edge_mode != FCD_EDGE_REFERENCE && c.edge_mode != FCD_EDGE_SYMMETRIC)) {
        snprintf(ctx->msg, sizeof(ctx->msg), null ? "%s: null pointer" : "%s: bad edge_mode", who);
        return FCD_ERR_ARG;
    }
    if (r_pass && c.edge_mode == FCD_EDGE_REFERENCE && c.Nreg == 2)
        return fcd_fail(ctx, FCD_ERR_INDEX, "reference edge ids: index 1 is out of bounds for axis 0 with size 1 (Nreg=2)");
    c.pl = fcd_sweep_plan_for(ctx, c.Nreg, c.U, c.g.GW);
    return FCD_OK;
}

extern "C" int fcd_gibbs_f_step(fcd_ctx *ctx, const double *S_B, const double *lM, const double *lMf, const double *hyper,
                                uint8_t *f_state, const uint64_t *r_bits, int64_t Nreg, int64_t U, int64_t G,
                                int64_t chain0, uint64_t seed, int64_t sweep, fcd_stream stream) {
    fcd_sweep_call c = {S_B, lM, lMf, nullptr, hyper, f_state, const_cast<uint64_t *>(r_bits) , Nreg, U, G,
                        chain0, seed, FCD_EDGE_SYMMETRIC, (hipStream_t)stream};
    int rc = fcd_sweep_call_check(ctx, c, true, false, "fcd_gibbs_f_step");
    return rc ? rc : fcd_gibbs_f_pass(ctx, c, fcd_sweep_step{sweep});
}

int fcd_gibbs_f_pass(fcd_ctx *ctx, const fcd_sweep_call &c, const fcd_sweep_step &st) {
    const fcd_sweep_plan &pl = c.pl;
    const fcd_geo &g = c.g;
    const int64_t Nreg = c.Nreg, U = c.U;
    hipStream_t s = c.s;
    const int form = c.lMf ? pl.f_form : FCD_F_GENERIC;
    if (form == FCD_F_GENERIC)
        return launch_f<false>(ctx, c.S_B, c.lM, c.hyper, c.f_state, c.r_bits, Nreg, U, c.G, g, c.chain0, c.seed, st.sweep,
                               nullptr, s);
    fcd_abl_refresh(s);
    const int wpb = g.GW < 16 ? g.GW : 16;
    float margin = FCD_DRAW_F_MARGIN;
    if ((float)ctx->knobs.f_tol > margin) margin = (float)ctx->knobs.f_tol;
    int rc;
    if (form == FCD_F_PAIR || form == FCD_F_PAIRX) {
        rc = fcd_ws_reserve(ctx, pl.ws_bytes);
        if (rc) return rc;
        uint32_t *r_U = (uint32_t *)((char *)ctx->ws + pl.r_U);
        if (!st.ru_ready) {
            const int64_t items = (int64_t)g.GW * Nreg * pl.f_NW;
            hipLaunchKernelGGL(pack_ru_kernel, dim3((unsigned)((items + 3) / 4)), dim3(256), 0, s, c.r_bits, (int)Nreg, (int)U,
                               pl.f_NW, g.GW, r_U);
            FCD_LAUNCH_CHECK();
        }
        dim3 grid((unsigned)((g.C + pl.f_EC - 1) / pl.f_EC), (unsigned)((g.GW + wpb - 1) / wpb));
        const bool pt = st.f_packed && form == FCD_F_PAIR;
        if (st.f_rec && (!pt || !pl.frec_bytes || ctx->frec_bytes < pl.frec_bytes))
            return fcd_fail(ctx, FCD_ERR_ARG, "f pass: prebuilt records asked for where the plan has none");
        const size_t f_shmem = st.f_rec ? pl.f_shmem_rec : pl.f_shmem;
        if (st.f_packed && (form != FCD_F_PAIR || !pl.r_blocked || st.fsq))
            return fcd_fail(ctx, FCD_ERR_ARG, "f pass: packed f words asked for where the plan has none");
        uint2 *f_S = pt ? (uint2 *)((char *)ctx->ws + pl.f_S) : nullptr;
        const int NBLK = (int)((Nreg + R_NB - 1) / R_NB);
        if (pt) grid.x = (unsigned)fpt_tiles((Nreg + 1) / 2);
#define FCD_F_ARGS c.S_B, c.lMf, c.hyper, c.f_state, r_U, (int)Nreg, (int)U, g.C, g.GW, (uint32_t)c.chain0, c.seed, (uint32_t)st.sweep, margin, st.fsq
#define FCD_LAUNCH_F(KERN, SLOT, EXTRA)                                                                            \
    do {                                                                                                      \
        rc = fcd_lds_attr(ctx, SLOT, reinterpret_cast<const void *>(&KERN), f_shmem);                         \
        if (rc) return rc;                                                                                    \
        {                                                                                                     \
            static int lds0 = 0;               \
            rc = fcd_static_lds_check(ctx, reinterpret_cast<const void *>(&KERN), &lds0);                     \
            if (rc) return rc;                                                                                \
        }                                                                                                     \
        fcd_prof_begin(ctx, FCD_PROF_F, s);                                                                   \
        hipLaunchKernelGGL(KERN, grid, dim3(64 * wpb), f_shmem, s, FCD_F_ARGS, EXTRA);                        \
        fcd_prof_end(ctx, FCD_PROF_F, s);                                                                     \
    } while (0)
#define FCD_PX (unsigned long long *)ctx->dbg, c.lM
#define FCD_PT f_S, NBLK, (unsigned long long *)ctx->dbg, (const char *)st.f_rec, c.lM
        const bool sure = form == FCD_F_PAIR && pt && st.f_rec && st.f_sure && !(margin > 1.f) && ctx->knobs.f_sure != 1;
        if (sure && ctx->knobs.f_runs != 1 && (st.f_all || ctx->knobs.f_runs == 2)) {
            const int rw = wpb < FR_WAVES ? wpb : FR_WAVES;
            dim3 rgrid((unsigned)fpr_runs((Nreg + 1) / 2), (unsigned)((g.GW + rw - 1) / rw));
            fcd_prof_begin(ctx, FCD_PROF_F, s);
            hipLaunchKernelGGL(gibbs_f_run_kernel, rgrid, dim3(64 * rw), 0, s, c.S_B, c.lMf, c.hyper, c.f_state, r_U, (int)Nreg, (int)U, g.C,
                               g.GW, (uint32_t)c.chain0, c.seed, (uint32_t)st.sweep, margin, f_S, NBLK, (unsigned long long *)ctx->dbg,
                               (const char *)st.f_rec, c.lM, (int)grid.x, (unsigned *)((char *)st.f_rec + pl.frec_votes));
            fcd_prof_end(ctx, FCD_PROF_F, s);
            ctx->n_frec_pass += 1;
            ctx->n_fsure_pass += 1;
            ctx->n_frun_pass += 1;
        } else if (sure) {
            if (pl.f_NW == 1) FCD_LAUNCH_F((gibbs_f_pair_kernel<1, true, true, true>), FCD_KA_F_PAIR_S + 0, FCD_PT);
            else if (pl.f_NW == 2) FCD_LAUNCH_F((gibbs_f_pair_kernel<2, true, true, true>), FCD_KA_F_PAIR_S + 1, FCD_PT);
            else if (pl.f_NW == 3) FCD_LAUNCH_F((gibbs_f_pair_kernel<3, true, true, true>), FCD_KA_F_PAIR_S + 2, FCD_PT);
            else FCD_LAUNCH_F((gibbs_f_pair_kernel<4, true, true, true>), FCD_KA_F_PAIR_S + 3, FCD_PT);
            ctx->n_frec_pass += 1;
            ctx->n_fsure_pass += 1;
        } else if (form == FCD_F_PAIR && pt && st.f_rec) {
            if (pl.f_NW == 1) FCD_LAUNCH_F((gibbs_f_pair_kernel<1, true, true>), FCD_KA_F_PAIR_R + 0, FCD_PT);
            else if (pl.f_NW == 2) FCD_LAUNCH_F((gibbs_f_pair_kernel<2, true, true>), FCD_KA_F_PAIR_R + 1, FCD_PT);
            else if (pl.f_NW == 3) FCD_LAUNCH_F((gibbs_f_pair_kernel<3, true, true>), FCD_KA_F_PAIR_R + 2, FCD_PT);
            else FCD_LAUNCH_F((gibbs_f_pair_kernel<4, true, true>), FCD_KA_F_PAIR_R + 3, FCD_PT);
            ctx->n_frec_pass += 1;
        } else if (form == FCD_F_PAIR && pt) {
            if (pl.f_NW == 1) FCD_LAUNCH_F((gibbs_f_pair_kernel<1, true>), FCD_KA_F_PAIR_T + 0, FCD_PT);
            else if (pl.f_NW == 2) FCD_LAUNCH_F((gibbs_f_pair_kernel<2, true>), FCD_KA_F_PAIR_T + 1, FCD_PT);
            else if (pl.f_NW == 3) FCD_LAUNCH_F((gibbs_f_pair_kernel<3, true>), FCD_KA_F_PAIR_T + 2, FCD_PT);
            else FCD_LAUNCH_F((gibbs_f_pair_kernel<4, true>), FCD_KA_F_PAIR_T + 3, FCD_PT);
        } else if (form == FCD_F_PAIR) {
            if (pl.f_NW == 1) FCD_LAUNCH_F((gibbs_f_pair_kernel<1, false>), FCD_KA_F_PAIR + 0, FCD_PT);
            else if (pl.f_NW == 2) FCD_LAUNCH_F((gibbs_f_pair_kernel<2, false>), FCD_KA_F_PAIR + 1, FCD_PT);
            else if (pl.f_NW == 3) FCD_LAUNCH_F((gibbs_f_pair_kernel<3, false>), FCD_KA_F_PAIR + 2, FCD_PT);
            else FCD_LAUNCH_F((gibbs_f_pair_kernel<4, false>), FCD_KA_F_PAIR + 3, FCD_PT);
        } else {
            if (pl.f_EC == 8) FCD_LAUNCH_F(gibbs_f_pairx_kernel<8>, FCD_KA_F_PAIR_BIG + 0, FCD_PX);
            else if (pl.f_EC == 4) FCD_LAUNCH_F(gibbs_f_pairx_kernel<4>, FCD_KA_F_PAIR_BIG + 1, FCD_PX);
            else if (pl.f_EC == 2) FCD_LAUNCH_F(gibbs_f_pairx_kernel<2>, FCD_KA_F_PAIR_BIG + 2, FCD_PX);
            else FCD_LAUNCH_F(gibbs_f_pairx_kernel<1>, FCD_KA_F_PAIR_BIG + 3, FCD_PX);
        }
#undef FCD_PT
#undef FCD_PX
#undef FCD_LAUNCH_F
#undef FCD_F_ARGS
        FCD_LAUNCH_CHECK();
        return FCD_OK;
    }
    rc = fcd_lds_attr(ctx, FCD_KA_F_DIFF, reinterpret_cast<const void *>(&gibbs_f_diff_kernel), pl.f_shmem);
    if (rc) return rc;
    dim3 grid((unsigned)((g.C + pl.f_EC - 1) / pl.f_EC), (unsigned)((g.GW + wpb - 1) / wpb));
    fcd_prof_begin(ctx, FCD_PROF_F, s);
    hipLaunchKernelGGL(gibbs_f_diff_kernel, grid, dim3(64 * wpb), pl.f_shmem, s, c.S_B, c.lMf, c.hyper, c.f_state, c.r_bits,
                       (int)Nreg, (int)U, g.C, g.GW, pl.f_EC, (uint32_t)c.chain0, c.seed, (uint32_t)st.sweep, margin, c.lM);
    fcd_prof_end(ctx, FCD_PROF_F, s);
    FCD_LAUNCH_CHECK();
    return FCD_OK;
}

extern "C" int fcd_gibbs_mstep(fcd_ctx *ctx, const int64_t *counts, int64_t Nreg, int64_t U, double *hyper,
                               fcd_stream stream) {
    if (!ctx || !counts || !hyper) return fcd_fail(ctx, FCD_ERR_ARG, "fcd_gibbs_mstep: null pointer");
    if (Nreg < 2 || U < 1) return fcd_fail(ctx, FCD_ERR_SHAPE, "need Nreg >= 2 and U >= 1 (Nreg=%lld, U=%lld)", Nreg, U);
    hipLaunchKernelGGL(gibbs_mstep_kernel, dim3(1), dim3(1), 0, (hipStream_t)stream,
                       reinterpret_cast<const long long *>(counts), (double)fcd_tri(Nreg), (double)(Nreg * U), hyper);
    FCD_LAUNCH_CHECK();
    return FCD_OK;
}

static int launch_tally(fcd_ctx *ctx, const uint8_t *f_state, const uint64_t *r_bits, int64_t Nreg, int64_t U, int64_t G,
                        const fcd_geo &g, int64_t *counts, uint32_t *cnt_f, uint32_t *cnt_r, double *hyper, uint32_t *r_U,
                        int ru_words, hipStream_t s, bool f_done = false, uint2 *r_S = nullptr, uint32_t *marks = nullptr) {
    tally_args a;
    a.f_state = f_state; a.r_bits = r_bits;
    a.C = g.C; a.NU = Nreg * U; a.G = G;
    a.GW = g.GW; a.Nreg = (int)Nreg; a.U = (int)U; a.NW = ru_words;
    a.marks = r_U ? marks : nullptr; a.r_S = a.marks ? r_S : nullptr;
    a.NBLK = (int)((Nreg + R_NB - 1) / R_NB);
    a.acc = (counts || hyper) ? (unsigned long long *)ctx->acc : nullptr;
    a.counts_out = reinterpret_cast<unsigned long long *>(counts);
    a.cnt_f = cnt_f; a.cnt_r = cnt_r;
    a.hyper = hyper; a.r_U = r_U;
    int64_t blocks = (g.C + 63) / 64;
    const int64_t cap = (int64_t)ctx->num_cu * 2;
    if (blocks > cap) blocks = cap;
    a.n_f_blocks = f_done ? 0 : (int)blocks;
    {
        int64_t rb = (a.NU + 1023) / 1024;
        if (rb > 64) rb = 64;
        a.n_r_blocks = (int)rb;
        if (rb > a.n_f_blocks) blocks = rb;
    }
    if (r_U) {
        const int64_t n_marks = a.marks ? (int64_t)g.GW * U * a.NBLK : 0;
        int64_t ru_blocks = ((int64_t)g.GW * Nreg * a.NW + (a.r_S ? n_marks : (n_marks + 63) / 64) + 15) / 16;
        if (ru_blocks > ctx->num_cu) ru_blocks = ctx->num_cu;
        blocks += ru_blocks;
    }
    hipLaunchKernelGGL(gibbs_tally_kernel, dim3((unsigned)blocks), dim3(1024), 0, s, a);
    FCD_LAUNCH_CHECK();
    return FCD_OK;
}

extern "C" int fcd_gibbs_tally(fcd_ctx *ctx, const uint8_t *f_state, const uint64_t *r_bits, int64_t Nreg, int64_t U,
                               int64_t G, int64_t *counts, uint32_t *cnt_f, uint32_t *cnt_r, fcd_stream stream) {
    fcd_geo g;
    int rc = fcd_geo_check(ctx, Nreg, U, G, 0, g);
    if (rc) return rc;
    if (!f_state || !r_bits) return fcd_fail(ctx, FCD_ERR_ARG, "fcd_gibbs_tally: null pointer");
    if ((cnt_f == nullptr) != (cnt_r == nullptr)) return fcd_fail(ctx, FCD_ERR_ARG, "fcd_gibbs_tally: cnt_f and cnt_r go together");
    if (!counts && !cnt_f) return FCD_OK;
    return launch_tally(ctx, f_state, r_bits, Nreg, U, G, g, counts, cnt_f, cnt_r, nullptr, nullptr, 0, (hipStream_t)stream);
}

extern "C" int fcd_gibbs_stats(fcd_ctx *ctx, const uint8_t *f_state, const uint64_t *r_bits, int64_t Nreg, int64_t U,
                               int64_t G, int64_t *counts, fcd_stream stream) {
    fcd_geo g;
    int rc = fcd_geo_check(ctx, Nreg, U, G, 0, g);
    if (rc) return rc;
    if (!f_state || !r_bits || !counts) return fcd_fail(ctx, FCD_ERR_ARG, "fcd_gibbs_stats: null pointer");
    return launch_tally(ctx, f_state, r_bits, Nreg, U, G, g, counts, nullptr, nullptr, nullptr, nullptr, 0, (hipStream_t)stream);
}

extern "C" int fcd_gibbs_accumulate(fcd_ctx *ctx, const uint8_t *f_state, const uint64_t *r_bits, int64_t Nreg,
                                    int64_t U, int64_t G, uint32_t *cnt_f, uint32_t *cnt_r, fcd_stream stream) {
    fcd_geo g;
    int rc = fcd_geo_check(ctx, Nreg, U, G, 0, g);
    if (rc) return rc;
    if (!f_state || !r_bits || !cnt_f || !cnt_r) return fcd_fail(ctx, FCD_ERR_ARG, "fcd_gibbs_accumulate: null pointer");
    return launch_tally(ctx, f_state, r_bits, Nreg, U, G, g, nullptr, cnt_f, cnt_r, nullptr, nullptr, 0, (hipStream_t)stream);
}

static int acc_launch_pair(fcd_ctx *ctx, const fcd_sweep_call &c, const fcd_geo &g, const fcd_sweep_acc &a, hipStream_t s) {
    return fcd_pair_tally_launch<uint32_t>(ctx, c.f_state, c.r_bits, c.Nreg, c.U, c.G, g, a.buf[0], true, s);
}
static int acc_launch_count(fcd_ctx *ctx, const fcd_sweep_call &c, const fcd_geo &g, const fcd_sweep_acc &a, hipStream_t s) {
    return fcd_count_tally_launch(ctx, c.r_bits, c.Nreg, c.U, c.G, g, a.buf[0], a.buf[1], s);
}
static int acc_launch_coanomaly(fcd_ctx *ctx, const fcd_sweep_call &c, const fcd_geo &g, const fcd_sweep_acc &a, hipStream_t s) {
    return fcd_coanomaly_tally_launch(ctx, c.r_bits, c.Nreg, c.U, c.G, g, a.buf[0], a.buf[1], s);
}
static int acc_launch_region_set(fcd_ctx *ctx, const fcd_sweep_call &c, const fcd_geo &g, const fcd_sweep_acc &a, hipStream_t s) {
    return fcd_region_set_tally_launch(ctx, c.r_bits, c.Nreg, c.U, c.G, g, a.buf[0], a.buf[1], s);
}
static int acc_launch_patient_group(fcd_ctx *ctx, const fcd_sweep_call &c, const fcd_geo &g, const fcd_sweep_acc &a, hipStream_t s) {
    return fcd_patient_group_tally_launch(ctx, c.r_bits, c.Nreg, c.U, c.G, g, a.buf[0], a.buf[1], s);
}
static int acc_launch_patient_trait(fcd_ctx *ctx, const fcd_sweep_call &c, const fcd_geo &g, const fcd_sweep_acc &a, hipStream_t s) {
    return fcd_patient_trait_tally_launch(ctx, c.r_bits, c.Nreg, c.U, c.G, g, a.buf[0], (int64_t *)a.buf[1], s);
}
static const struct {
    const char *msg_shape;
    int (*launch)(fcd_ctx *, const fcd_sweep_call &, const fcd_geo &, const fcd_sweep_acc &, hipStream_t);
    int (*reserve)(fcd_ctx *, int64_t Nreg, int64_t U, int64_t G);
} SWEEP_ACC[FCD_ACC_N] = {
    {"fcd_gibbs_run: the attached pair accumulator was made for Nreg=%lld, U=%lld", acc_launch_pair, nullptr},
    {"fcd_gibbs_run: the attached count accumulator was made for Nreg=%lld, U=%lld", acc_launch_count, fcd_count_ws_reserve},
    {"fcd_gibbs_run: the attached co-anomaly accumulator was made for Nreg=%lld, U=%lld", acc_launch_coanomaly, nullptr},
    {"fcd_gibbs_run: the attached region-set accumulator was made for Nreg=%lld, U=%lld", acc_launch_region_set,
     fcd_region_set_ws_reserve},
    {"fcd_gibbs_run: the attached patient-group accumulator was made for Nreg=%lld, U=%lld", acc_launch_patient_group,
     fcd_patient_group_ws_reserve},
    {"fcd_gibbs_run: the attached patient-trait accumulator was made for Nreg=%lld, U=%lld", acc_launch_patient_trait,
     fcd_patient_trait_ws_reserve},
};

static int fcd_f_sure_hint_wait(fcd_ctx *ctx, hipStream_t s, bool &any, bool &all) {
    const unsigned build = (unsigned)(ctx->n_frec_build & 0x3fffffff);
    const auto t0 = std::chrono::steady_clock::now();
    unsigned v = *ctx->f_sure_hint;
    for (unsigned spin = 1; (v >> 2) != build; ++spin, v = *ctx->f_sure_hint) {
        if ((spin & 1023u) == 0 && std::chrono::steady_clock::now() - t0 > std::chrono::seconds(2)) {
            FCD_HIP_TRY(hipStreamSynchronize(s));
            v = *ctx->f_sure_hint;
            if ((v >> 2) != build) return fcd_fail(ctx, FCD_ERR_DEVICE, "f pass: the record build left no hint");
            break;
        }
    }
    any = (v & 1u) != 0u;
    all = (v & 2u) != 0u;
    return FCD_OK;
}
static int fcd_r_sure_hint_wait(fcd_ctx *ctx, hipStream_t s, bool &share, bool &any) {
    const unsigned build = (unsigned)(ctx->n_rsure_build & 0x3fffffff);
    const auto t0 = std::chrono::steady_clock::now();
    unsigned v = ctx->f_sure_hint[1];
    for (unsigned spin = 1; (v >> 2) != build; ++spin, v = ctx->f_sure_hint[1]) {
        if ((spin & 1023u) == 0 && std::chrono::steady_clock::now() - t0 > std::chrono::seconds(2)) {
            FCD_HIP_TRY(hipStreamSynchronize(s));
            v = ctx->f_sure_hint[1];
            if ((v >> 2) != build) return fcd_fail(ctx, FCD_ERR_DEVICE, "r pass: the bound build left no hint");
            break;
        }
    }
    share = (v & 1u) != 0u;
    any = (v & 2u) != 0u;
    return FCD_OK;
}

static int sweep_loop(fcd_ctx *ctx, const fcd_sweep_call &c, int64_t sweep0, int64_t n_sweeps, int64_t mstep_every,
                      int64_t accumulate_from, int64_t *counts, uint32_t *cnt_f, uint32_t *cnt_r, double *hyper_m,
                      unsigned acc_mask) {
    if (n_sweeps < 0 || sweep0 < 0 || sweep0 + n_sweeps > (1ll << 32))
        return fcd_fail(ctx, FCD_ERR_ARG, "sweep range [%lld, +%lld) outside the 32-bit counter word", sweep0, n_sweeps);
    const fcd_sweep_plan &pl = c.pl;
    const fcd_geo &g = c.g;
    const int64_t Nreg = c.Nreg, U = c.U, G = c.G;
    hipStream_t s = c.s;
    const bool pair_form = c.lMf && (pl.f_form == FCD_F_PAIR || pl.f_form == FCD_F_PAIRX);
    fcd_sweep_step st = {sweep0};
    uint8_t *fsq = nullptr;
    if (pl.fsq_bytes && c.lMf && c.lMd && c.edge_mode == FCD_EDGE_SYMMETRIC) {
        int rc = fcd_fsq_reserve(ctx, pl.fsq_bytes);
        if (rc) return rc;
        fsq = (uint8_t *)ctx->fsq;
    }
    const bool packed_ok = pl.f_form == FCD_F_PAIR && c.lMf && c.lMd && pl.r_blocked && pl.r_idx32 &&
                           c.edge_mode == FCD_EDGE_SYMMETRIC && ctx->knobs.f_pack != 1 && !ctx->knobs.r_refill;
    if (pair_form) {
        int rc = fcd_ws_reserve(ctx, pl.ws_bytes);
        if (rc) return rc;
    }
    const int64_t pt_sweeps = packed_ok ? n_sweeps - 1 : 0;
    bool use_rec = pl.frec_bytes && ctx->knobs.f_records != 1 && pt_sweeps >= (ctx->knobs.f_records == 2 ? 1 : F_REC_MIN_SWEEPS);
    if (use_rec && fcd_frec_reserve(ctx, pl.frec_bytes) != FCD_OK) {
        (void)hipGetLastError();
        use_rec = false;
    }
    bool rec_built = false;
    if (use_rec) {
        ctx->n_frec_build += 1;
        hipLaunchKernelGGL(gibbs_f_records_kernel, dim3((unsigned)fpt_tiles((Nreg + 1) / 2)), dim3(64 * FP_EC), 0, s, c.S_B, c.lMf,
                           c.hyper, (int)Nreg, (int)U, (char *)ctx->frec, (unsigned *)((unsigned long long *)ctx->dbg + 4),
                           (unsigned *)((char *)ctx->frec + pl.frec_votes), (int)((pl.frec_bytes - pl.frec_votes) / sizeof(unsigned)));
        FCD_LAUNCH_CHECK();
        hipLaunchKernelGGL(gibbs_f_hint_kernel, dim3(1), dim3(1), 0, s, (unsigned *)((unsigned long long *)ctx->dbg + 4), ctx->f_sure_hint,
                           (unsigned)(ctx->n_frec_build & 0x3fffffff), c.lM, c.hyper);
        FCD_LAUNCH_CHECK();
        rec_built = true;
    }
    const fcd_knobs &kn = ctx->knobs;
    const bool rs_ok = pl.rs_bytes && kn.r_sure != 1 && !(kn.r_tol > 16.0 * FCD_LOGIT_FAST_ERR) && !kn.r_path && !kn.r_coop &&
                       !kn.r_dsplit;
    int rs_state = 0;
    for (int64_t i = 0; i < n_sweeps; ++i) {
        st.sweep = sweep0 + i;
        st.f_packed = packed_ok && st.r_packed;
        st.fsq = st.f_packed ? nullptr : fsq;
        if (rs_state == 1 && st.f_packed) {
            bool share = false, any = false;
            int rc = fcd_r_sure_hint_wait(ctx, s, share, any);
            if (rc) return rc;
            rs_state = (kn.r_sure == 2 || share) ? 2 : -1;
        }
        if (rec_built && st.f_packed && !st.f_rec) {
            int rc = fcd_f_sure_hint_wait(ctx, s, st.f_sure, st.f_all);
            if (rc) return rc;
            st.f_rec = ctx->frec;
            if (rs_ok && (st.f_sure || kn.r_sure == 2)) {
                rc = fcd_gibbs_r_bounds_build(ctx, c);
                if (rc) return rc;
                rs_state = 1;
            } else {
                rs_state = -1;
            }
        }
        st.r_sure = rs_state == 2 && st.f_packed && st.r_packed;
        int rc = fcd_gibbs_f_pass(ctx, c, st);
        if (rc) return rc;
        const bool last = i + 1 == n_sweeps;
        const bool do_m = mstep_every > 0 && (i + 1) % mstep_every == 0;
        const bool do_a = cnt_f && st.sweep >= accumulate_from;
        fcd_tally_f tf;
        tf.f_state = c.f_state; tf.C = g.C; tf.G = G; tf.GW = g.GW;
        tf.acc = (do_m || (last && counts)) ? (unsigned long long *)ctx->acc : nullptr;
        tf.cnt_f = do_a ? cnt_f : nullptr;
        st.tally_f = (tf.acc || tf.cnt_f) ? &tf : nullptr;
        rc = fcd_gibbs_r_pass(ctx, c, st);
        if (rc) {
            if (tf.acc) (void)hipMemsetAsync(ctx->acc, 0, 8 * sizeof(unsigned long long), s);
            return rc;
        }
        st.sentinels_in_place = pair_form && ctx->r_form_last == 2;
        uint32_t *r_U_next = (pair_form && !last) ? (uint32_t *)((char *)ctx->ws + pl.r_U) : nullptr;
        const bool r_next = packed_ok && r_U_next;
        const bool keep_words = ctx->knobs.r_keep_words == 1;
        uint2 *r_S_next = (r_next && keep_words) ? (uint2 *)((char *)ctx->ws + (st.r_flip ? pl.r_Sn : pl.r_S)) : nullptr;
        int64_t *cts = (last ? counts : nullptr);
        const bool pooled = do_m && ctx->comm != nullptr;
        int64_t *tally_counts = pooled ? (int64_t *)ctx->pool_counts : cts;
        if (do_m || do_a || cts || r_U_next) {
            rc = launch_tally(ctx, c.f_state, c.r_bits, Nreg, U, G, g, tally_counts, do_a ? cnt_f : nullptr, do_a ? cnt_r : nullptr,
                              (do_m && !pooled) ? hyper_m : nullptr, r_U_next, pl.f_NW, s, st.tally_f_done, r_S_next,
                              r_next ? (uint32_t *)((char *)ctx->ws + pl.marks) : nullptr);
            if (rc) {
                if (tf.acc) (void)hipMemsetAsync(ctx->acc, 0, 8 * sizeof(unsigned long long), s);
                return rc;
            }
        }
        if (pooled) {
            rc = fcd_comm_allreduce_counts(ctx, (long long *)ctx->pool_counts, s);
            if (rc) return rc;
            hipLaunchKernelGGL(gibbs_mstep_kernel, dim3(1), dim3(1), 0, s, (const long long *)ctx->pool_counts, (double)g.C,
                               (double)(Nreg * U), hyper_m);
            FCD_LAUNCH_CHECK();
            if (cts) FCD_HIP_TRY(hipMemcpyAsync(cts, ctx->pool_counts, 8 * sizeof(long long), hipMemcpyDeviceToDevice, s));
        } else if (cts && ctx->comm) {
            rc = fcd_comm_allreduce_counts(ctx, (long long *)cts, s);
            if (rc) return rc;
        }
        if (acc_mask && st.sweep >= accumulate_from) {
            for (int k = 0; k < FCD_ACC_N; ++k) {
                const fcd_sweep_acc &a = ctx->sweep_acc[k];
                if (!(acc_mask >> k & 1u) || (st.sweep - accumulate_from) % a.every != 0) continue;
                rc = SWEEP_ACC[k].launch(ctx, c, g, a, s);
                if (rc) return rc;
            }
        }
        st.ru_ready = r_U_next != nullptr;
        st.r_packed = r_next;
        if (r_next && !keep_words) st.r_flip = !st.r_flip;
    }
    return FCD_OK;
}

extern "C" int fcd_gibbs_run(fcd_ctx *ctx, const double *S_B, const double *lM, const double *lMf, const double *lMd,
                             double *hyper, uint8_t *f_state, uint64_t *r_bits, int64_t Nreg, int64_t U, int64_t G,
                             int64_t chain0, uint64_t seed, int64_t sweep0, int64_t n_sweeps, int edge_mode,
                             int64_t mstep_every, int64_t accumulate_from, int64_t *counts, uint32_t *cnt_f, uint32_t *cnt_r,
                             fcd_stream stream) {
    fcd_sweep_call c = {S_B, lM, lMf, lMd, hyper, f_state, r_bits, Nreg, U, G, chain0, seed, edge_mode, (hipStream_t)stream};
    int rc = fcd_sweep_call_check(ctx, c, true, true, "fcd_gibbs_run");
    if (rc) return rc;
    if ((cnt_f == nullptr) != (cnt_r == nullptr)) return fcd_fail(ctx, FCD_ERR_ARG, "fcd_gibbs_run: cnt_f and cnt_r go together");
    if (mstep_every < 0) return fcd_fail(ctx, FCD_ERR_ARG, "fcd_gibbs_run: mstep_every < 0");
    unsigned acc_mask = 0;
    for (int k = 0; k < FCD_ACC_N; ++k) {
        const fcd_sweep_acc &a = ctx->sweep_acc[k];
        if (!a.buf[0]) continue;
        if (a.nreg != Nreg || a.u != U) return fcd_fail(ctx, FCD_ERR_SHAPE, SWEEP_ACC[k].msg_shape, a.nreg, a.u);
        acc_mask |= 1u << k;
    }
    for (int k = 0; k < FCD_ACC_N; ++k) {
        if (!(acc_mask >> k & 1u) || !SWEEP_ACC[k].reserve) continue;
        rc = SWEEP_ACC[k].reserve(ctx, Nreg, U, G);
        if (rc) return rc;
    }
    return sweep_loop(ctx, c, sweep0, n_sweeps, mstep_every, accumulate_from, counts, cnt_f, cnt_r, hyper, acc_mask);
}

extern "C" int fcd_gibbs_sweeps(fcd_ctx *ctx, const double *S_B, const double *lM, const double *lMf, const double *lMd,
                                const double *hyper,
                                uint8_t *f_state, uint64_t *r_bits, int64_t Nreg, int64_t U, int64_t G, int64_t chain0,
                                uint64_t seed, int64_t sweep0, int64_t n_sweeps, int edge_mode, int64_t *counts,
                                fcd_stream stream) {
    fcd_sweep_call c = {S_B, lM, lMf, lMd, hyper, f_state, r_bits, Nreg, U, G, chain0, seed, edge_mode, (hipStream_t)stream};
    int rc = fcd_sweep_call_check(ctx, c, true, true, "fcd_gibbs_sweeps");
    if (rc) return rc;
    rc = sweep_loop(ctx, c, sweep0, n_sweeps, 0, 0, nullptr, nullptr, nullptr, nullptr, 0u);
    if (rc) return rc;
    if (counts && n_sweeps > 0) return fcd_gibbs_stats(ctx, f_state, r_bits, Nreg, U, G, counts, stream);
    return FCD_OK;
}

extern "C" int fcd_gibbs_logjoint(fcd_ctx *ctx, const double *S_B, const double *lM, const double *hyper,
                                  const uint8_t *f_state, const uint64_t *r_bits, int64_t Nreg, int64_t U, int64_t G,
                                  double *out, fcd_stream stream) {
    fcd_geo g;
    int rc = fcd_geo_check(ctx, Nreg, U, G, 0, g);
    if (rc) return rc;
    if (!S_B || !lM || !hyper || !f_state || !r_bits || !out) return fcd_fail(ctx, FCD_ERR_ARG, "fcd_gibbs_logjoint: null pointer");
    const size_t need = (size_t)LJ_SLICES * g.GW * 64 * sizeof(double);
    rc = fcd_ws_reserve(ctx, need);
    if (rc) return rc;
    hipStream_t s = (hipStream_t)stream;
    hipLaunchKernelGGL(gibbs_logjoint_kernel, dim3((unsigned)g.GW, LJ_SLICES), dim3(64), 0, s, S_B, lM, hyper, f_state,
                       r_bits, (int)Nreg, (int)U, g.C, g.GW, (double *)ctx->ws);
    FCD_LAUNCH_CHECK();
    hipLaunchKernelGGL(gibbs_logjoint_fold, dim3((unsigned)((G + 255) / 256)), dim3(256), 0, s, (const double *)ctx->ws,
                       (int64_t)g.GW * 64, G, out);
    FCD_LAUNCH_CHECK();
    return FCD_OK;
}

extern "C" int fcd_gibbs_chain_rsum(fcd_ctx *ctx, const uint64_t *r_bits, int64_t Nreg, int64_t U, int64_t G, uint32_t *out,
                                    fcd_stream stream) {
    fcd_geo g;
    int rc = fcd_geo_check(ctx, Nreg, U, G, 0, g);
    if (rc) return rc;
    if (!r_bits || !out) return fcd_fail(ctx, FCD_ERR_ARG, "fcd_gibbs_chain_rsum: null pointer");
    hipStream_t s = (hipStream_t)stream;
    FCD_HIP_TRY(hipMemsetAsync(out, 0, (size_t)G * sizeof(uint32_t), s));
    const int64_t NU = Nreg * U;
    const int slices = (int)(NU < 64 ? NU : 64);
    hipLaunchKernelGGL(gibbs_rsum_kernel, dim3((unsigned)g.GW, (unsigned)slices), dim3(64), 0, s, r_bits, NU, G, out);
    FCD_LAUNCH_CHECK();
    return FCD_OK;
}

extern "C" int fcd_gibbs_conditionals(fcd_ctx *ctx, const double *S_B, const double *lM, const double *hyper,
                                      const uint8_t *f_state, const uint64_t *r_bits, int64_t Nreg, int64_t U,
                                      int64_t G, int edge_mode, double *cond_f, double *cond_r, fcd_stream stream) {
    fcd_geo g;
    int rc = fcd_geo_check(ctx, Nreg, U, G, 0, g);
    if (rc) return rc;
    if (!S_B || !lM || !hyper || !f_state || !r_bits) return fcd_fail(ctx, FCD_ERR_ARG, "fcd_gibbs_conditionals: null pointer");
    if (edge_mode != FCD_EDGE_REFERENCE && edge_mode != FCD_EDGE_SYMMETRIC)
        return fcd_fail(ctx, FCD_ERR_ARG, "fcd_gibbs_conditionals: edge_mode %lld", edge_mode);
    if (edge_mode == FCD_EDGE_REFERENCE && Nreg == 2 && cond_r)
        return fcd_fail(ctx, FCD_ERR_INDEX, "reference edge ids: index 1 is out of bounds for axis 0 with size 1 (Nreg=2)");
    hipStream_t s = (hipStream_t)stream;
    if (cond_f) {
        rc = launch_f<true>(ctx, S_B, lM, hyper, const_cast<uint8_t *>(f_state), r_bits, Nreg, U, G, g, 0, 0, 0, cond_f, s);
        if (rc) return rc;
    }
    if (cond_r) {
        if (U > 65535 || Nreg > 65535) return fcd_fail(ctx, FCD_ERR_UNSUPPORTED, "fcd_gibbs_conditionals: grid too large");
        hipLaunchKernelGGL(gibbs_cond_r_kernel, dim3((unsigned)U, (unsigned)g.GW, (unsigned)Nreg), dim3(64), 0, s, lM, hyper,
                           f_state, r_bits, (int)Nreg, (int)U, g.C, G, edge_mode, cond_r);
        FCD_LAUNCH_CHECK();
    }
    return FCD_OK;
}

extern "C" int fcd_gibbs_export_state(fcd_ctx *ctx, const uint8_t *f_state, const uint64_t *r_bits, int64_t Nreg,
                                      int64_t U, int64_t G, uint8_t *f, uint8_t *r, fcd_stream stream) {
    fcd_geo g;
    int rc = fcd_geo_check(ctx, Nreg, U, G, 0, g);
    if (rc) return rc;
    if (!f_state || !r_bits || !f || !r) return fcd_fail(ctx, FCD_ERR_ARG, "fcd_gibbs_export_state: null pointer");
    hipStream_t s = (hipStream_t)stream;
    hipLaunchKernelGGL(export_f_kernel, dim3((unsigned)((G * g.C + 255) / 256)), dim3(256), 0, s, f_state, g.C, G, f);
    FCD_LAUNCH_CHECK();
// ... 31 lines not shown
```

### fcdiff_amd/csrc/fcd_gibbs_r.hip

```cpp
#include <stdlib.h>

#include <type_traits>

#include "fcd_common.h"

namespace {


__global__ __launch_bounds__(256) void region_tables_kernel(const double *__restrict__ lM, int Nreg, int U, int mode,
                                                            double *__restrict__ lMd) {
    const int64_t total = (int64_t)U * Nreg * Nreg;
    for (int64_t rec = (int64_t)blockIdx.x * blockDim.x + threadIdx.x; rec < total; rec += (int64_t)gridDim.x * blockDim.x) {
        const int m = (int)(rec % Nreg);
        const int n = (int)((rec / Nreg) % Nreg);
        const int u = (int)(rec / ((int64_t)Nreg * Nreg));
        double *o = lMd + rec * 6;
        if (m == n) {
#pragma unroll
            for (int x = 0; x < 6; ++x) o[x] = 0.0;
        } else {
            const double *p = lM + (fcd_pair_to_edge(n, m, mode) * U + u) * 9;
#pragma unroll
            for (int k = 0; k < 3; ++k) {
                o[k * 2 + 0] = p[k * 3 + 2] - p[k * 3 + 0];
// ... 993 lines not shown
                const uint2 fwb = fro[ulane], fwa = (fro - a_back)[ulane];
                const uint2 za = make_uint2(fwa.x | rpb.x, fwa.y | rpb.y), zb = make_uint2(fwb.x | rcur.x, fwb.y | rcur.y);
                const uint32_t ra = pb_off + (uint32_t)(stop * (R_NB / 2) * 288), rb = pb_off + (uint32_t)((R_NB + stop) * (R_NB / 2) * 288);
                vstop = (e + (four(za, ra, 0) + four(za, ra, 4))) + (four(zb, rb, 0) + four(zb, rb, 4));
            }
            if (__ballot(fabs(vstop) < a.tol) != 0ull) {
                uint32_t ul3 = ulane;
                asm volatile("" : "+v"(ul3));
                vstop += pipe_exact_corr((uint32_t)((B0 + stop) * ((U + 1) >> 1) + (u >> 1)), a.chain0 + (uint32_t)w * 64u + ul3,
                                         a.sweep, a.seed, u & 1);
            }
            const uint32_t t = vstop > 0.0 ? 1u : 0u;
            fresh |= t << stop;
            const int sh = 8 * ((stop >> 1) & 3) + (stop & 1);
            if ((stop >> 1) < 4) rcur.x = (rcur.x & ~(1u << sh)) | (t << sh);
            else rcur.y = (rcur.y & ~(1u << sh)) | (t << sh);
            i0 = stop + 1;
        }
#pragma unroll
        for (int i = 0; i < R_NB; ++i) {
            if (i < nb) {
                const uint64_t ball = __ballot((fresh >> i) & 1u);
                if (lane == 0) a.r_bits[((int64_t)w * Nreg + B0 + i) * U + u] = ball;
                __hip_atomic_store(reinterpret_cast<unsigned long long *>(const_cast<double *>(Pw) + i * 64 + ulane), R_SENT,
                                   __ATOMIC_RELAXED, __HIP_MEMORY_SCOPE_AGENT);
            }
        }
        rpb = spread2(fresh);
        FCD_TRACE_AT(tr0, trec, 2);
        {
            uint32_t ul2 = ulane;
            asm volatile("" : "+v"(ul2));
            unsigned long long *dst = reinterpret_cast<unsigned long long *>(a.r_Sn + (wu * NBLK + b) * 64 + ul2);
            const unsigned long long val = (unsigned long long)rpb.x | ((unsigned long long)rpb.y << 32);
            __hip_atomic_store(dst, val, __ATOMIC_RELAXED, __HIP_MEMORY_SCOPE_AGENT);
        }
        asm volatile("s_waitcnt vmcnt(0)" ::: "memory");
        if (lane == 0 && !a.withhold) __hip_atomic_store(a.flags + wu * NBLK + b, 1u, __ATOMIC_RELAXED, __HIP_MEMORY_SCOPE_AGENT);
        FCD_TRACE_AT(tr0, trec, 4);
        __builtin_amdgcn_s_setprio(0);
    }
}

template <int UB, int WPE>
__global__ __launch_bounds__(1024, WPE) void gibbs_r_pipe_kernel(const r_step_args a, volatile unsigned *err) {
    extern __shared__ __attribute__((aligned(16))) double smem[];
    const int blk = blockIdx.x;
    if (blk < a.nD) {
        if (a.tf.f_state) fcd_tally_f_block<16>(a.tf, blk, a.nD, reinterpret_cast<unsigned long long (*)[3]>(smem));
        const int half = a.dsplit ? blk / a.u_n : -1;
        for (int wg = 0; wg < a.nWG; ++wg) pipe_diag(a, a.u_lo + (a.dsplit ? blk % a.u_n : blk), wg, half, smem, err);
    } else {
        int item = blk - a.nD;
        if (a.npad) {
            if (blk >= a.ncu + a.nD) {
                item -= a.npad;
            } else if (blk >= a.ncu) {
                return;
            }
        }
        const int row = item % R_NB, uc = item / R_NB;
        for (int wg = 0; wg < a.nWG; ++wg) pipe_panel<UB>(a, row, uc, wg, smem, err);
    }
}

template <int UB, int WPE>
__global__ __launch_bounds__(1024, WPE) void gibbs_r_step_kernel(const r_step_args a) {
    extern __shared__ __attribute__((aligned(16))) double smem[];
    const int blk = blockIdx.x;
    if (blk < a.nD) {
        r_role_diag(a, a.s - 1, a.u_lo + blk % a.u_n, blk / a.u_n, smem);
    } else {
        int item = blk - a.nD;
        if (a.npad) {
            if (blk >= a.ncu + a.nD) {
                item -= a.npad;
            } else if (blk >= a.ncu) {
                return;
            }
        }
        const int rows = (a.Nreg - a.s * R_NB < R_NB) ? (a.Nreg - a.s * R_NB) : R_NB;
        const int nUC = (a.u_n + UB - 1) / UB;
        r_role_panel<UB>(a, a.s, item % rows, (item / rows) % nUC, item / (rows * nUC), smem);
    }
}

constexpr int R_WAVES = 4;
__global__ __launch_bounds__(64 * R_WAVES) void gibbs_r_simple(const double *__restrict__ lM, const double *__restrict__ hyper,
                                                               const uint8_t *__restrict__ f_state,
                                                               uint64_t *__restrict__ r_bits, int Nreg, int U, int64_t C,
                                                               uint32_t chain0, uint64_t seed, uint32_t sweep, int mode) {
    extern __shared__ uint64_t sh_r[];
    uint64_t *mask = sh_r;
    double *part = reinterpret_cast<double *>(sh_r + Nreg);
    const int u = blockIdx.x, w = blockIdx.y;
    const int tid = threadIdx.x, lane = tid & 63;
    const int wave = __builtin_amdgcn_readfirstlane(tid >> 6);
    uint64_t *__restrict__ rcol = r_bits + (int64_t)w * Nreg * U + u;
    for (int n = tid; n < Nreg; n += 64 * R_WAVES) mask[n] = rcol[(int64_t)n * U];
    __syncthreads();
    const uint8_t *__restrict__ fw = f_state + (int64_t)w * C * 64 + lane;
    const double *__restrict__ lMu = lM + (int64_t)u * 9;
    const double lnpi0 = hyper[FCD_H_LNPI0], lnpi1 = hyper[FCD_H_LNPI1];
    const uint32_t chain = chain0 + (uint32_t)w * 64u + lane;
    const uint32_t k0 = (uint32_t)seed, k1 = (uint32_t)(seed >> 32);
    fcd_u4 rnd = {0, 0, 0, 0};

    for (int n = 0; n < Nreg; ++n) {
        double s0 = 0.0, s1 = 0.0;
#pragma unroll 4
        for (int m = wave; m < Nreg; m += R_WAVES) {
            const bool valid = (m != n);
            const int64_t c = valid ? fcd_pair_to_edge(n, m, mode) : 0;
            const int k = fw[c * 64];
            const uint32_t bit = (uint32_t)((mask[m] >> lane) & 1ull);
            const double *p = lMu + (c * U) * 9 + k * 3;
            const double v0 = p[bit * 2];
            const double v1 = p[2 - bit];
            s0 += valid ? v0 : 0.0;
            s1 += valid ? v1 : 0.0;
        }
        part[(wave * 2 + 0) * 64 + lane] = s0;
        part[(wave * 2 + 1) * 64 + lane] = s1;
        __syncthreads();
        if (wave == 0) {
            double t0 = part[0 * 64 + lane], t1 = part[1 * 64 + lane];
#pragma unroll
            for (int j = 1; j < R_WAVES; ++j) {
                t0 += part[(j * 2 + 0) * 64 + lane];
                t1 += part[(j * 2 + 1) * 64 + lane];
            }
            rnd = fcd_philox((uint32_t)(n * ((U + 1) >> 1) + (u >> 1)), chain, sweep, FCD_KIND_R, k0, k1);
            const double x = (u & 1) ? fcd_u53(rnd.z, rnd.w) : fcd_u53(rnd.x, rnd.y);
            const uint64_t ball = __ballot(fcd_draw_r(lnpi0 + t0, lnpi1 + t1, x));
            if (lane == 0) mask[n] = ball;
        }
        __syncthreads();
    }
    for (int n = tid; n < Nreg; n += 64 * R_WAVES) rcol[(int64_t)n * U] = mask[n];
}

struct r_sparse_args {
    const double *lMd, *hyper;
    const uint2 *f_S;
    uint2 *r_Sn;
    uint64_t *r_bits;
    const double *bnd;
    const double *dtab;
    const uint2 *mword;
    const uint32_t *rowflag;
    uint64_t *visit;
    uint32_t *fneq;
    unsigned long long *cnt;
    int Nreg, U, NBLK, GW;
    int64_t G;
    uint32_t chain0, sweep;
    uint64_t seed;
    double tol, x_lo;
};

constexpr int RS_WAVES = 4;

__global__ __launch_bounds__(256) void gibbs_r_bounds_kernel(const double *__restrict__ lMd, const fcd_f_edge_rec *__restrict__ erec,
                                                             const double *__restrict__ hyper0, int Nreg, int U, int NBLK,
                                                             double *__restrict__ bnd, double *__restrict__ dtab,
                                                             uint2 *__restrict__ mword, uint32_t *__restrict__ rowflag,
                                                             unsigned long long *__restrict__ n_decided) {
    extern __shared__ uint8_t km[];
    __shared__ int open_row;
    const int n = (int)blockIdx.x, NPAIR = (U + 1) >> 1;
    if (threadIdx.x == 0) open_row = 0;
    __syncthreads();
    const double g1 = hyper0[FCD_H_LNGAMMA + 1] - hyper0[FCD_H_LNGAMMA + 0], g2 = hyper0[FCD_H_LNGAMMA + 2] - hyper0[FCD_H_LNGAMMA + 0];
    for (int m = threadIdx.x; m < NBLK * R_NB; m += blockDim.x) {
        int k = 0;
        if (m < Nreg && m != n) {
            const fcd_f_edge_rec rec = erec[fcd_pair_to_edge(n, m, FCD_EDGE_SYMMETRIC)];
            const double c1 = g1 + rec.d1, c2 = g2 + rec.d2;
            k = fcd_f_edge_mode(c1, c2, rec.b, fcd_f_edge_delta(c1, c2, NPAIR, rec.a), FCD_F_SURE_T - FCD_F_SURE_DRIFT);
            if (k < 0) {
                k = 3;
                open_row = 1;
            }
        }
        km[m] = (uint8_t)k;
    }
    __syncthreads();
    const bool open = open_row != 0;
    if (threadIdx.x == 0) rowflag[n] = open ? 1u : 0u;
    for (int b = threadIdx.x; b < NBLK; b += blockDim.x) {
        uint32_t v[2] = {0u, 0u};
        for (int p = 0; p < R_NB / 2; ++p) {
            const uint32_t k0 = km[b * R_NB + 2 * p] & 3u, k1 = km[b * R_NB + 2 * p + 1] & 3u;
            v[p >> 2] |= (((k0 == 3u ? 0u : k0) * 3u + (k1 == 3u ? 0u : k1)) << 2) << (8 * (p & 3));
        }
        mword[n * NBLK + b] = make_uint2(v[0], v[1]);
    }
    const int lane = threadIdx.x & 63, wave = (int)(threadIdx.x >> 6);
    const double off = hyper0[FCD_H_LNPI1] - hyper0[FCD_H_LNPI0];
    unsigned long long dec = 0;
    for (int u = wave; u < U; u += (int)(blockDim.x >> 6)) {
        const double *__restrict__ row = lMd + ((int64_t)u * Nreg + n) * Nreg * 6;
        double *__restrict__ drow = dtab + ((int64_t)u * Nreg + n) * Nreg;
        double hi = 0.0, lo = 0.0, base = 0.0, mag = 0.0;
        bool bad = false;
        for (int m = lane; m < Nreg; m += 64) {
            if (m == n) continue;
            const int k = km[m];
            const double *p = row + m * 6;
            double mx, mn;
            if (k < 3) {
                const double t0 = p[2 * k], t1 = p[2 * k + 1];
                bad = bad || !isfinite(t0) || !isfinite(t1);
                mx = fmax(t0, t1);
                mn = fmin(t0, t1);
                base += t0;
                drow[m] = t1 - t0;
            } else {
                drow[m] = 0.0;
                mx = mn = p[0];
                bad = bad || !isfinite(p[0]);
                for (int x = 1; x < 6; ++x) {
                    bad = bad || !isfinite(p[x]);
                    mx = fmax(mx, p[x]);
                    mn = fmin(mn, p[x]);
                }
            }
            hi += mx;
            lo += mn;
            mag += fmax(fabs(mx), fabs(mn));
        }
        hi = fcd_wave_sum(hi);
        lo = fcd_wave_sum(lo);
        base = fcd_wave_sum(base);
        mag = fcd_wave_sum(mag);
        bad = __ballot(bad) != 0ull;
        if (lane == 0) {
            const double slack = (double)(Nreg + 8) * 1.2e-16 * mag;
            const double nan = __builtin_nan("");
            const int64_t NU = (int64_t)Nreg * U, i = (int64_t)n * U + u;
            const double h = bad ? nan : hi + slack, l = bad ? nan : lo - slack;
            bnd[i] = h;
            bnd[NU + i] = l;
            drow[n] = (bad || open) ? nan : base;
            if (!open && (h + off < -R_SURE_T || l + off > R_SURE_T)) dec += 1;
        }
    }
    if (lane == 0 && dec) atomicAdd(n_decided, dec);
}

__global__ void gibbs_r_hint_kernel(unsigned long long *__restrict__ n_decided, volatile unsigned *hint, unsigned build,
                                    double total, double share) {
    const unsigned long long d = *n_decided;
    *n_decided = 0ull;
    __hip_atomic_store(const_cast<unsigned *>(hint), 4u * build + (d > 0ull ? 2u : 0u) + ((double)d >= share * total ? 1u : 0u),
                       __ATOMIC_RELEASE, __HIP_MEMORY_SCOPE_SYSTEM);
}

__global__ __launch_bounds__(64 * RS_WAVES) void gibbs_r_range_kernel(const r_sparse_args a) {
    __shared__ unsigned red[2];
    if (threadIdx.x < 2) red[threadIdx.x] = 0u;
    __syncthreads();
    const int lane = threadIdx.x & 63;
    const int n = __builtin_amdgcn_readfirstlane((int)(blockIdx.x * RS_WAVES + (threadIdx.x >> 6)));
    const int w = (int)blockIdx.y;
    const int Nreg = a.Nreg, U = a.U, NBLK = a.NBLK, NPAIR = (U + 1) >> 1;
    if (n < Nreg) {
        const uint64_t act = fcd_active_mask(w, a.G);
        const bool rf = a.rowflag[n] != 0u;
        bool neq = false;
        if (!rf) {
            const uint2 *__restrict__ fw = a.f_S + ((int64_t)w * Nreg + n) * NBLK * 64 + lane;
            const uint2 *__restrict__ mw = a.mword + n * NBLK;
            for (int b = 0; b < NBLK; ++b) {
                const uint2 f = fw[b * 64], m = mw[b];
                neq = neq || f.x != m.x || f.y != m.y;
            }
        }
        const bool off_modes = rf || (__ballot(neq) & act) != 0ull;
        const double off = a.hyper[FCD_H_LNPI1] - a.hyper[FCD_H_LNPI0];
        const double x_lo = a.x_lo, x_hi = 1.0 - a.x_lo;
        const uint32_t chain = a.chain0 + (uint32_t)w * 64u + (uint32_t)lane;
        const int64_t NU = (int64_t)Nreg * U;
        uint64_t dec0, dec1;
        {
            const int ul = lane < U ? lane : U - 1;
            const double hi = a.bnd[(int64_t)n * U + ul], lo = a.bnd[NU + (int64_t)n * U + ul];
            const bool d0 = hi + off < -R_SURE_T, d1 = !d0 && lo + off > R_SURE_T;
            dec0 = __ballot(!rf && lane < U && d0);
            dec1 = __ballot(!rf && lane < U && d1);
        }
        const uint64_t all_u = U >= 64 ? ~0ull : ((1ull << U) - 1ull);
        uint64_t visit = all_u & ~(dec0 | dec1), ones = 0ull;
        unsigned n_sure = 0u, n_exc = 0u;
        if (off_modes) {
            n_exc = (unsigned)__builtin_popcountll(dec0 | dec1);
            visit = all_u;
        } else {
            for (int j = 0; j < NPAIR; ++j) {
                if ((((dec0 | dec1) >> (2 * j)) & 3ull) == 0ull) continue;
                const fcd_u4 x = fcd_philox((uint32_t)(n * NPAIR + j), chain, a.sweep, FCD_KIND_R, (uint32_t)a.seed, (uint32_t)(a.seed >> 32));
#pragma unroll
                for (int h = 0; h < 2; ++h) {
                    const int u = 2 * j + h;
                    const bool d0 = (dec0 >> u) & 1ull, d1 = (dec1 >> u) & 1ull;
                    if (u >= U || !(d0 || d1)) continue;
                    const double xx = h ? fcd_u53(x.z, x.w) : fcd_u53(x.x, x.y);
                    const bool out = d0 ? !(xx >= x_lo) : !(xx <= x_hi);
                    if ((__ballot(out) & act) != 0ull) {
                        n_exc += 1u;
                        visit |= 1ull << u;
                    } else {
                        n_sure += 1u;
                        if (d1) ones |= 1ull << u;
                    }
                }
            }
        }
        if (lane == 0) {
            a.visit[(int64_t)w * Nreg + n] = visit;
            a.fneq[(int64_t)w * Nreg + n] = off_modes ? 1u : 0u;
            if (n_sure) atomicAdd(&red[0], n_sure);
            if (n_exc) atomicAdd(&red[1], n_exc);
        }
        if (lane < U && !((visit >> lane) & 1ull)) a.r_bits[((int64_t)w * Nreg + n) * U + lane] = ((ones >> lane) & 1ull) ? act : 0ull;
    }
    __syncthreads();
    if (threadIdx.x < 2 && red[threadIdx.x]) atomicAdd(&a.cnt[threadIdx.x], (unsigned long long)red[threadIdx.x]);
}

__device__ __forceinline__ void rs_wave_sync() {
    __builtin_amdgcn_fence(__ATOMIC_RELEASE, "wavefront");
    __builtin_amdgcn_wave_barrier();
    __builtin_amdgcn_fence(__ATOMIC_ACQUIRE, "wavefront");
}

constexpr int RS_SEG = 32;
constexpr int RS_MAXCH = 16;
static_assert(RS_SEG == 16 || RS_SEG == 32, "the walk's segment is 16 or 32 sites");
static inline size_t rs_walk_lds(int NBLK) {
    return (size_t)(RS_SEG * 64 + RS_SEG * RS_SEG + NBLK * R_NB + 2 * RS_MAXCH) * 8 + (size_t)RS_SEG * 64 * 4 + (size_t)RS_SEG * 4;
}
__device__ __forceinline__ double rs_lane_f64(double v, int j) {
    return __longlong_as_double((long long)fcd_lane_word((uint64_t)__double_as_longlong(v), j));
}
__device__ __forceinline__ uint64_t rs_uniform64(uint64_t v) {
    const uint32_t lo = (uint32_t)__builtin_amdgcn_readfirstlane((int)(uint32_t)v);
    const uint32_t hi = (uint32_t)__builtin_amdgcn_readfirstlane((int)(uint32_t)(v >> 32));
    return ((uint64_t)hi << 32) | lo;
}
__global__ __launch_bounds__(64) void gibbs_r_sparse_kernel(const r_sparse_args a) {
    extern __shared__ uint64_t rs_lds[];
    constexpr int S = RS_SEG;
    const int lane = (int)threadIdx.x;
    const int Nreg = a.Nreg, U = a.U, NBLK = a.NBLK, NP = NBLK * R_NB, NPAIR = (U + 1) >> 1;
    const int u = (int)(blockIdx.x % (unsigned)U), w = (int)(blockIdx.x / (unsigned)U);
    double *Pl = reinterpret_cast<double *>(rs_lds);
    double *Dl = Pl + S * 64;
    uint64_t *rm = reinterpret_cast<uint64_t *>(Dl + S * S);
    uint64_t *vm = rm + NP;
    uint64_t *sw = vm + RS_MAXCH;
    float *thl = reinterpret_cast<float *>(sw + RS_MAXCH);
    int *sn = reinterpret_cast<int *>(thl + S * 64);
    uint64_t *__restrict__ rcol = a.r_bits + (int64_t)w * Nreg * U + u;
    const int nchunk = (Nreg + 63) >> 6;
    for (int c0 = 0; c0 < nchunk; c0 += 4) {
        uint64_t col[4], vis[4];
#pragma unroll
        for (int k = 0; k < 4; ++k) {
            const int m = (c0 + k) * 64 + lane, mc = m < Nreg ? m : 0;
            col[k] = rcol[(int64_t)mc * U];
            vis[k] = a.visit[(int64_t)w * Nreg + mc];
        }
#pragma unroll
        for (int k = 0; k < 4; ++k) {
            const int m = (c0 + k) * 64 + lane;
            if (m < NP) rm[m] = m < Nreg ? col[k] : 0ull;
            const uint64_t todo = __ballot(m < Nreg && ((vis[k] >> u) & 1ull));
            if (lane == 0 && c0 + k < nchunk) vm[c0 + k] = todo;
        }
    }
    rs_wave_sync();
    const double off = a.hyper[FCD_H_LNPI1] - a.hyper[FCD_H_LNPI0];
    const uint32_t chain = a.chain0 + (uint32_t)w * 64u + (uint32_t)lane;
    const uint32_t k0 = (uint32_t)a.seed, k1 = (uint32_t)(a.seed >> 32);
    const double *__restrict__ utab = a.dtab + (int64_t)u * Nreg * Nreg;
    auto uniform_of = [&](int n) -> double {
        const fcd_u4 x = fcd_philox((uint32_t)(n * NPAIR + (u >> 1)), chain, a.sweep, FCD_KIND_R, k0, k1);
        return (u & 1) ? fcd_u53(x.z, x.w) : fcd_u53(x.x, x.y);
    };
    int pos = 0;
    for (;;) {
        int cnt = 0, last = -1;
        for (int c = 0; c < nchunk; ++c) {
            uint64_t t = rs_uniform64(vm[c]);
            if (c < (pos >> 6) || cnt >= S) t = 0ull;
            else if (c == (pos >> 6)) t &= ~0ull << (pos & 63);
            const int before = (int)__builtin_popcountll(t & ((1ull << lane) - 1ull));
            const bool mine = ((t >> lane) & 1ull) && cnt + before < S;
            const uint64_t take = __ballot(mine);
            if (mine) sn[cnt + before] = c * 64 + lane;
            if (lane == 0) sw[c] = take;
            if (take) last = c * 64 + 63 - (int)__builtin_clzll(take);
            cnt += (int)__builtin_popcountll(take);
        }
        if (cnt == 0) break;
        pos = last + 1;
        rs_wave_sync();
        const int nj = sn[lane < cnt ? lane : 0];
        const double basej = utab[(int64_t)nj * Nreg + nj];
        const uint32_t fnj = a.fneq[(int64_t)w * Nreg + nj];
        const uint64_t wj = lane < cnt ? rm[nj] : 0ull;
        double d[S];
#pragma unroll
        for (int i = 0; i < S; ++i) d[i] = 0.0;
// ... 178 lines not shown
        r_step_args ac = a;
        volatile unsigned *errp = ctx->dev_err;
        void *kargs[2] = {(void *)&ac, (void *)&errp};
        hipError_t e = hipLaunchCooperativeKernel(fn, dim3((unsigned)(a.nD + a.nP + a.npad)), dim3(threads), kargs, (unsigned)shmem, s);
        if (e == hipErrorCooperativeLaunchTooLarge) {
            (void)hipGetLastError();
            *fits = false;
            return FCD_OK;
        }
        if (e != hipSuccess) return (int)e;
    } else {
        hipLaunchKernelGGL((gibbs_r_pipe_kernel<UB, WPE>), dim3((unsigned)(a.nD + a.nP + a.npad)), dim3(threads), shmem, s, a, ctx->dev_err);
    }
    fcd_prof_end(ctx, FCD_PROF_RSTEP, s);
    FCD_LAUNCH_CHECK();
    return FCD_OK;
}

template <class F>
int with_ub(int ub, F &&f) {
    if (ub == 4) return f(std::integral_constant<int, 4>(), std::integral_constant<int, 4>());
    if (ub == 2) return f(std::integral_constant<int, 2>(), std::integral_constant<int, 8>());
    return f(std::integral_constant<int, 1>(), std::integral_constant<int, 8>());
}
}

fcd_sweep_plan fcd_sweep_plan_for(const fcd_ctx *ctx, int64_t Nreg, int64_t U, int64_t GW) {
    fcd_sweep_plan p = {};
    p.f_NW = (int)((U + 15) / 16);
    const int f_form = ctx->knobs.f_form;
    const bool words_ok = GW * Nreg * p.f_NW < INT32_MAX / 4;
    const size_t pair_shmem = (size_t)FP_EC * ((U + 1) / 2) * 128 + FP_EC * 16 + (size_t)FP_EC * U * 48;
    const size_t per_edge = (size_t)((U + 1) / 2) * 128, extra = 128 + 16 * 48 * 16;
    if ((size_t)U * 48 > 160 * 1024) {
        p.f_form = FCD_F_GENERIC;
    } else if (f_form != FCD_F_PAIRX && f_form != FCD_F_DIFF && p.f_NW <= 4 && pair_shmem <= 96 * 1024 && words_ok) {
        p.f_form = FCD_F_PAIR;
        p.f_EC = FP_EC;
        p.f_shmem = pair_shmem;
    } else if (f_form != FCD_F_DIFF && words_ok && per_edge + extra <= 160 * 1024) {
        int ec = 8;
        while (ec > 1 && (size_t)ec * per_edge + extra > 80 * 1024) ec >>= 1;
        p.f_form = FCD_F_PAIRX;
        p.f_EC = ec;
        p.f_shmem = (size_t)ec * per_edge + extra;
    } else {
        int64_t e = (int64_t)(24 * 1024 / ((size_t)U * 48));
        if (e < 1) e = 1;
        if (e > 8) e = 8;
        if (e > 1) e &= ~1ll;
        p.f_form = FCD_F_DIFF;
        p.f_EC = (int)e;
        p.f_shmem = (size_t)U * 48 * e;
    }
    const bool pair_form = p.f_form == FCD_F_PAIR || p.f_form == FCD_F_PAIRX;
    const int64_t NBLK = (Nreg + R_NB - 1) / R_NB;
    const size_t per_u = (size_t)NBLK * ((R_NB / 2) * 36 + R_NB * 6) * sizeof(double);
    p.r_blocked = per_u <= 156 * 1024 && Nreg + U <= 65535;
    p.r_idx32 = GW * Nreg * NBLK <= INT32_MAX / 4 && fcd_tri(Nreg) * 64 <= INT32_MAX && GW * U * R_NB <= INT32_MAX / 64;
    p.r_ub = ((size_t)4 * per_u <= 160 * 1024 && U >= 2) ? 2 : 1;
    {
        const int v = ctx->knobs.r_ub;
        if ((v == 1 || v == 2 || v == 4) && (size_t)v * per_u <= 156 * 1024) p.r_ub = v;
    }
    const size_t d_need = (size_t)(GW < 16 ? D_LDS_SPREAD : D_LDS_COMPACT) * sizeof(double);
    p.r_shmem = (size_t)p.r_ub * per_u > d_need ? (size_t)p.r_ub * per_u : d_need;
    const size_t fsq = (size_t)GW * Nreg * Nreg * 64;
    p.fsq_bytes = (pair_form && fsq <= ((size_t)8 << 30)) ? fsq : 0;
    if (p.f_form == FCD_F_PAIR && p.r_blocked && p.r_idx32) {
        const size_t NPAIR = (size_t)(U + 1) / 2;
        p.f_shmem_rec = (size_t)FP_EC * NPAIR * 128 + FP_EC * 16 + 64;
        p.frec_edge = (size_t)fpt_tiles((Nreg + 1) / 2) * NPAIR * FP_EC * F_REC_PIECES * 16;
        p.frec_votes = p.frec_edge + (size_t)fcd_tri(Nreg) * sizeof(fcd_f_edge_rec);
        p.frec_bytes = p.frec_votes + (size_t)fpr_runs((Nreg + 1) / 2) * (size_t)((GW + 15) / 16) * sizeof(unsigned);
        if (p.frec_bytes > F_REC_CAP) p.frec_bytes = 0;
    }
    size_t r_end = 0;
    if (p.r_blocked) {
        const size_t t_bytes = (size_t)GW * U * R_NB * 64 * sizeof(double);
        const size_t s_bytes = (size_t)GW * U * NBLK * 64 * sizeof(uint2);
        p.P[1] = t_bytes;
        p.f_S = 2 * t_bytes;
        p.r_S = p.f_S + (size_t)GW * Nreg * NBLK * 64 * sizeof(uint2);
        p.r_Sn = p.r_S + s_bytes;
        p.marks = p.r_Sn + s_bytes;
        r_end = p.marks + (size_t)GW * U * NBLK * sizeof(uint32_t) + 512;
    }
    p.r_U = (r_end + 511) / 512 * 512;
    p.ws_bytes = p.r_U + (pair_form ? (size_t)GW * Nreg * (p.f_NW <= 4 ? 4 : p.f_NW) * 64 * sizeof(uint32_t) : 0);
    if (p.frec_bytes && U <= 64) {
        auto up = [](size_t x) { return (x + 511) / 512 * 512; };
        p.rs_bnd = up(p.ws_bytes);
        p.rs_dtab = up(p.rs_bnd + (size_t)2 * Nreg * U * sizeof(double));
        p.rs_mword = up(p.rs_dtab + (size_t)U * Nreg * Nreg * sizeof(double));
        p.rs_rowflag = up(p.rs_mword + (size_t)Nreg * NBLK * sizeof(uint2));
        p.rs_visit = up(p.rs_rowflag + (size_t)Nreg * sizeof(uint32_t));
        p.rs_fneq = up(p.rs_visit + (size_t)GW * Nreg * sizeof(uint64_t));
        p.ws_bytes = up(p.rs_fneq + (size_t)GW * Nreg * sizeof(uint32_t));
        p.rs_bytes = p.ws_bytes - p.rs_bnd;
    }
    return p;
}

extern "C" int fcd_gibbs_region_tables(fcd_ctx *ctx, const double *lM, int64_t Nreg, int64_t U, int edge_mode, double *lMd,
                                       fcd_stream stream) {
    if (!ctx || !lM || !lMd) return fcd_fail(ctx, FCD_ERR_ARG, "fcd_gibbs_region_tables: null pointer");
    if (Nreg < 2 || U < 1) return fcd_fail(ctx, FCD_ERR_SHAPE, "need Nreg >= 2 and U >= 1 (Nreg=%lld, U=%lld)", Nreg, U);
    if (edge_mode != FCD_EDGE_REFERENCE && edge_mode != FCD_EDGE_SYMMETRIC)
        return fcd_fail(ctx, FCD_ERR_ARG, "fcd_gibbs_region_tables: edge_mode %lld", edge_mode);
    if (edge_mode == FCD_EDGE_REFERENCE && Nreg == 2)
        return fcd_fail(ctx, FCD_ERR_INDEX, "reference edge ids: index 1 is out of bounds for axis 0 with size 1 (Nreg=2)");
    const int64_t total = U * Nreg * Nreg;
    int64_t blocks = (total + 255) / 256;
    const int64_t cap = (int64_t)ctx->num_cu * 16;
    if (blocks > cap) blocks = cap;
    hipLaunchKernelGGL(region_tables_kernel, dim3((unsigned)blocks), dim3(256), 0, (hipStream_t)stream, lM, (int)Nreg, (int)U,
                       edge_mode, lMd);
    FCD_LAUNCH_CHECK();
    return FCD_OK;
}

extern "C" int fcd_gibbs_r_step(fcd_ctx *ctx, const double *lM, const double *lMd, const double *hyper,
                                const uint8_t *f_state, uint64_t *r_bits, int64_t Nreg, int64_t U, int64_t G,
                                int64_t chain0, uint64_t seed, int64_t sweep, int edge_mode, fcd_stream stream) {
    fcd_sweep_call c = {nullptr, lM, nullptr, lMd, hyper, const_cast<uint8_t *>(f_state) , r_bits, Nreg, U, G,
                        chain0, seed, edge_mode, (hipStream_t)stream};
    fcd_sweep_step st = {sweep};
    int rc = fcd_sweep_call_check(ctx, c, false, true, "fcd_gibbs_r_step");
    return rc ? rc : fcd_gibbs_r_pass(ctx, c, st);
}

int fcd_gibbs_r_bounds_build(fcd_ctx *ctx, const fcd_sweep_call &c) {
    const fcd_sweep_plan &pl = c.pl;
    if (!pl.rs_bytes || !ctx->frec || !c.lMd || !ctx->f_sure_hint)
        return fcd_fail(ctx, FCD_ERR_ARG, "r pass: bound build without the call's record table");
    int rc = fcd_ws_reserve(ctx, pl.ws_bytes);
    if (rc) return rc;
    char *ws = (char *)ctx->ws;
    const int Nreg = (int)c.Nreg, U = (int)c.U, NBLK = (Nreg + R_NB - 1) / R_NB;
    unsigned long long *dbg = (unsigned long long *)ctx->dbg;
    ctx->n_rsure_build += 1;
    hipLaunchKernelGGL(gibbs_r_bounds_kernel, dim3((unsigned)Nreg), dim3(256), (size_t)NBLK * R_NB, c.s, c.lMd,
                       (const fcd_f_edge_rec *)((const char *)ctx->frec + pl.frec_edge), (const double *)(dbg + 11), Nreg, U, NBLK,
                       (double *)(ws + pl.rs_bnd), (double *)(ws + pl.rs_dtab), (uint2 *)(ws + pl.rs_mword),
                       (uint32_t *)(ws + pl.rs_rowflag), dbg + 10);
    FCD_LAUNCH_CHECK();
    hipLaunchKernelGGL(gibbs_r_hint_kernel, dim3(1), dim3(1), 0, c.s, dbg + 10, ctx->f_sure_hint + 1,
                       (unsigned)(ctx->n_rsure_build & 0x3fffffff), (double)c.Nreg * (double)c.U, R_SURE_MIN_SHARE);
    FCD_LAUNCH_CHECK();
    return FCD_OK;
}

int fcd_gibbs_r_pass(fcd_ctx *ctx, const fcd_sweep_call &c, fcd_sweep_step &st) {
    st.tally_f_done = false;
    if (ctx->dev_err && *ctx->dev_err) return fcd_fail(ctx, FCD_ERR_DEVICE, "r pass: a device-side wait was abandoned in an earlier call");
    const fcd_sweep_plan &pl = c.pl;
    const fcd_geo &g = c.g;
    const int64_t Nreg = c.Nreg, U = c.U;
    const int edge_mode = c.edge_mode;
    hipStream_t s = c.s;
    if (!c.lMd || !pl.r_blocked) {
        const size_t shmem = (size_t)Nreg * 8 + (size_t)R_WAVES * 2 * 64 * 8;
        if (shmem > 64 * 1024) return fcd_fail(ctx, FCD_ERR_UNSUPPORTED, "r step: Nreg=%lld exceeds the LDS mask array", Nreg);
        if (U > 65535) return fcd_fail(ctx, FCD_ERR_UNSUPPORTED, "r step: U=%lld exceeds the grid", U);
        hipLaunchKernelGGL(gibbs_r_simple, dim3((unsigned)U, (unsigned)g.GW), dim3(64 * R_WAVES), shmem, s, c.lM, c.hyper,
                           c.f_state, c.r_bits, (int)Nreg, (int)U, g.C, (uint32_t)c.chain0, c.seed, (uint32_t)st.sweep, edge_mode);
        FCD_LAUNCH_CHECK();
        ctx->r_form_last = 0;
        return FCD_OK;
    }
    const int NBLK = (int)((Nreg + R_NB - 1) / R_NB);
    if (!pl.r_idx32)
        return fcd_fail(ctx, FCD_ERR_UNSUPPORTED, "r step: Nreg=%lld with G=%lld exceeds 32-bit item indices", Nreg, c.G);
    int rc = fcd_ws_reserve(ctx, pl.ws_bytes);
    if (rc) return rc;
    char *ws = (char *)ctx->ws;
    uint2 *f_S = (uint2 *)(ws + pl.f_S), *r_S = (uint2 *)(ws + (st.r_flip ? pl.r_Sn : pl.r_S));
    fcd_abl_refresh(s);
    const int ub = pl.r_ub;
    const size_t shmem = pl.r_shmem;
    r_step_args a;
    a.lMd = c.lMd; a.hyper = c.hyper; a.f_S = f_S;
    a.r_S = r_S; a.r_Sn = (uint2 *)(ws + (st.r_flip ? pl.r_S : pl.r_Sn)); a.r_bits = c.r_bits;
    a.Pbuf[0] = (double *)(ws + pl.P[0]); a.Pbuf[1] = (double *)(ws + pl.P[1]);
    a.flags = nullptr;
    a.Nreg = (int)Nreg; a.U = (int)U; a.NBLK = NBLK; a.GW = g.GW;
    a.u_lo = 0; a.u_n = (int)U;
    a.wpb = g.GW < 16 ? g.GW : 16;
    a.nWG = (g.GW + a.wpb - 1) / a.wpb;
    a.s = 0; a.nD = 0; a.nP = 0;
    a.ncu = ctx->num_cu; a.npad = 0;
    a.chain0 = (uint32_t)c.chain0; a.sweep = (uint32_t)st.sweep; a.seed = c.seed;
    a.tol = 16.0 * FCD_LOGIT_FAST_ERR;
    a.poll_limit = ctx->knobs.r_poll_limit > 0 ? ctx->knobs.r_poll_limit : R_POLL_LIMIT;
    a.withhold = ctx->knobs.r_withhold;
    a.tf.f_state = nullptr; a.tf.C = 0; a.tf.G = 0; a.tf.GW = 0; a.tf.acc = nullptr; a.tf.cnt_f = nullptr;
    if (ctx->knobs.r_tol > a.tol) a.tol = ctx->knobs.r_tol;
    if (st.r_sure) {
        if (!pl.rs_bytes || !st.f_packed || !st.r_packed) return fcd_fail(ctx, FCD_ERR_ARG, "r pass: sparse form without its tables");
        r_sparse_args q;
        q.lMd = c.lMd; q.hyper = c.hyper; q.f_S = f_S; q.r_Sn = a.r_Sn; q.r_bits = c.r_bits;
        q.bnd = (const double *)(ws + pl.rs_bnd); q.dtab = (const double *)(ws + pl.rs_dtab);
        q.mword = (const uint2 *)(ws + pl.rs_mword); q.rowflag = (const uint32_t *)(ws + pl.rs_rowflag);
        q.visit = (uint64_t *)(ws + pl.rs_visit); q.fneq = (uint32_t *)(ws + pl.rs_fneq);
        q.cnt = (unsigned long long *)ctx->dbg + 8;
        q.Nreg = (int)Nreg; q.U = (int)U; q.NBLK = NBLK; q.GW = g.GW; q.G = c.G;
        q.chain0 = a.chain0; q.sweep = a.sweep; q.seed = a.seed;
        q.tol = a.tol;
        q.x_lo = ctx->knobs.r_sure_x > R_SURE_X ? ctx->knobs.r_sure_x : R_SURE_X;
        fcd_prof_begin(ctx, FCD_PROF_RSTEP, s);
        hipLaunchKernelGGL(gibbs_r_range_kernel, dim3((unsigned)((Nreg + RS_WAVES - 1) / RS_WAVES), (unsigned)g.GW), dim3(64 * RS_WAVES), 0, s, q);
        hipLaunchKernelGGL(gibbs_r_sparse_kernel, dim3((unsigned)(U * g.GW)), dim3(64), rs_walk_lds(NBLK), s, q);
        fcd_prof_end(ctx, FCD_PROF_RSTEP, s);
        FCD_LAUNCH_CHECK();
        ctx->r_form_last = 4;
        ctx->n_rsure_pass += 1;
        return FCD_OK;
    }
    const int nUC = (int)((U + ub - 1) / ub);
    bool pipe = false;
    r_pipe_init pinit;
    pinit.marks = nullptr; pinit.P[0] = pinit.P[1] = nullptr;
    a.dsplit = 0;
    if (ctx->knobs.r_path != 3 && ctx->dev_err) {
        a.nD = (int)U;
        a.nP = R_NB * nUC;
        a.npad = (!ctx->knobs.r_nopad && a.nD <= a.ncu && a.nD + a.nP > a.ncu) ? a.nD : 0;
        if (ctx->knobs.r_dsplit != 1 && a.wpb > 8 && 2 * a.nD <= a.ncu) {
            a.dsplit = 1;
            a.nD = 2 * (int)U;
            a.npad = 0;
        }
        rc = with_ub(ub, [&](auto UB, auto WPE) { return launch_pipe<UB, WPE>(ctx, a, shmem, &pipe, false, s); });
        if (rc) return rc;
        if (!pipe && a.npad) {
            a.npad = 0;
            rc = with_ub(ub, [&](auto UB, auto WPE) { return launch_pipe<UB, WPE>(ctx, a, shmem, &pipe, false, s); });
            if (rc) return rc;
        }
        if (pipe) {
            pinit.marks = (uint32_t *)(ws + pl.marks);
            const bool keep = st.sentinels_in_place && ctx->r_form_last == 2 && !ctx->knobs.r_refill;
            pinit.P[0] = keep ? nullptr : a.Pbuf[0];
            pinit.P[1] = keep ? nullptr : a.Pbuf[1];
        } else {
            a.dsplit = 0;
        }
    }
    const bool packed = st.f_packed && st.r_packed && (!pipe || (pinit.P[0] == nullptr && pinit.P[1] == nullptr));
    if (!packed) {
        const int fb = st.fsq ? 2 : 1;
        dim3 pgrid((unsigned)(((NBLK + fb - 1) / fb + 3) / 4), (unsigned)(Nreg + U), (unsigned)g.GW);
        fcd_tally_f tf;
        tf.f_state = nullptr; tf.C = 0; tf.G = 0; tf.GW = 0; tf.acc = nullptr; tf.cnt_f = nullptr;
        if (st.tally_f && g.C * g.GW <= 600000) {
            tf = *st.tally_f;
            const int64_t per_row = (int64_t)pgrid.x * pgrid.z;
            int64_t want = (g.C + 15) / 16;
            if (want > 2 * (int64_t)ctx->num_cu) want = 2 * (int64_t)ctx->num_cu;
            int64_t ty = (want + per_row - 1) / per_row;
            if (ty < 1) ty = 1;
            if (pgrid.y + ty <= 65535) {
                pgrid.y += (unsigned)ty;
                st.tally_f_done = true;
            } else {
                tf.f_state = nullptr;
            }
        }
        fcd_prof_begin(ctx, FCD_PROF_PACK, s);
        if (st.fsq)
            hipLaunchKernelGGL(pack_f_kernel<true>, pgrid, dim3(256), 0, s, st.fsq, (int)Nreg, NBLK, (int)g.C, edge_mode, f_S,
                               c.r_bits, (int)U, r_S, pinit, tf);
        else
            hipLaunchKernelGGL(pack_f_kernel<false>, pgrid, dim3(256), 0, s, c.f_state, (int)Nreg, NBLK, (int)g.C, edge_mode, f_S,
                               c.r_bits, (int)U, r_S, pinit, tf);
        fcd_prof_end(ctx, FCD_PROF_PACK, s);
        FCD_LAUNCH_CHECK();
        ctx->n_pack += 1;
        if (st.tally_f_done) ctx->n_pack_tally += 1;
    }
    ctx->r_form_last = pipe ? 2 : 1;
    if (pipe) {
        a.flags = pinit.marks;
        bool ride = false;
        if (st.tally_f && !st.tally_f_done && ctx->knobs.tally_in_r != 1 && a.wpb == 16) {
            const int64_t rounds = ((g.C + 64 * (int64_t)a.nD - 1) / (64 * (int64_t)a.nD)) * ((g.GW + 15) / 16);
            ride = ctx->knobs.tally_in_r == 2 || rounds <= R_TALLY_MAX_ROUNDS;
        }
        if (ride) a.tf = *st.tally_f;
        rc = with_ub(ub, [&](auto UB, auto WPE) { return launch_pipe<UB, WPE>(ctx, a, shmem, &pipe, true, s); });
        if (rc) return rc;
        if (pipe) {
            if (ride) {
                st.tally_f_done = true;
                ctx->n_r_tally += 1;
            }
            return FCD_OK;
        }
        ctx->r_form_last = 1;
        a.flags = nullptr;
        a.dsplit = 0;
        a.tf.f_state = nullptr;
    }
    for (int step = 0; step <= NBLK; ++step) {
        const int rows = step < NBLK ? (int)((Nreg - (int64_t)step * R_NB < R_NB) ? (Nreg - (int64_t)step * R_NB) : R_NB) : 0;
        a.s = step;
        a.nD = step >= 1 ? (int)U * a.nWG : 0;
        a.nP = rows * nUC * a.nWG;
        a.npad = (!ctx->knobs.r_nopad && a.nD > 0 && a.nD <= a.ncu && a.nD + a.nP > a.ncu) ? a.nD : 0;
        if (a.nD + a.nP == 0) continue;
        rc = with_ub(ub, [&](auto UB, auto WPE) { return launch_step<UB, WPE>(ctx, a, shmem, s, true); });
        if (rc) return rc;
    }
    return FCD_OK;
}
```

### profiles/f_sure_cost.py

```python
#!/usr/bin/env python3
import argparse
import json
import os
import sys
import time

import numpy as np
import torch

ROOT = os.path.dirname(os.path.dirname(os.path.abspath(__file__)))
sys.path.insert(0, ROOT)


def main():
    ap = argparse.ArgumentParser()
    ap.add_argument("--data", choices=("weak", "cfg3", "mixed"), default="weak")
    ap.add_argument("--sweeps", type=int, default=300)
    ap.add_argument("--runs", type=int, default=5)
    ap.add_argument("--off", action="store_true", help="knob f_sure = 1: never the decided-tile path")
    args = ap.parse_args()
    import fcdiff_amd
    from fcdiff_amd.gibbs import GibbsEngine
    (Nreg, U, G) = (200, 50, 1024)
    H = {"weak": 2, "cfg3": 50, "mixed": 20}[args.data]
    model = fcdiff_amd.UnsharedRegionModel()
    if args.data == "weak":
        model.sigma = np.array([0.2, 0.25, 0.3])
        model.mu = np.array([-0.05, 0.0, 0.05])
    (_r, _t, _f, _ft, b, bt) = model.sample_fast(Nreg, H, U, seed=0)
    fit = fcdiff_amd.fit.UnsharedRegionFit()
    fit.model, fit.b, fit.bt = model, b, bt
    fit._init_lps(Nreg, H, U)
    fit._update_lps()
    ctx = fit._context()
    if args.off:
        ctx.set_knob("f_sure", 1)
    eng = GibbsEngine(fit._d["S_B"], fit._d["lM"], Nreg, U, G, seed=1, ctx=ctx)
    eng.set_hyper(model.gamma, model.pi2())
    eng.init(float(model.pi))
    eng.run(0, 64, mstep_every=1)
    torch.cuda.synchronize()

    def stat(name):
        try:
            return ctx.stat(name)
        except Exception:
            return None
    names = ("f_rec_passes", "f_sure_passes", "f_run_passes", "f_sure_tiles", "f_sure_fallbacks", "f_repeats")
    s0 = [stat(k) for k in names]
    ms = []
    sweep = 64
    for _ in range(args.runs):
        t0 = time.perf_counter()
        eng.run(sweep, args.sweeps, mstep_every=1)
        torch.cuda.synchronize()
        ms.append((time.perf_counter() - t0) / args.sweeps * 1e3)
        sweep += args.sweeps
    rise = {k: (None if a is None else stat(k) - a) for (k, a) in zip(names, s0)}
    i = (Nreg + 1) // 2
    tiles = (i // 2) * (i // 2 + 1) if i % 2 == 0 else (i // 2 + 1) ** 2
    out = {"data": args.data, "f_sure_off": bool(args.off), "lib": os.environ.get("FCDIFF_HIP_LIB", "default"),
           "ms_per_sweep": [round(x, 5) for x in ms], "min": round(min(ms), 5), "range": round(max(ms) - min(ms), 5), "rise": rise,
           "tiles_per_pass": tiles,
           "share_on_path": None if not rise["f_sure_tiles"] else rise["f_sure_tiles"] / float(tiles * rise["f_rec_passes"])}
    print(json.dumps(out))


if __name__ == "__main__":
    main()
```

Before: 8.424 million.

## Fold f-state tally into the f run kernel with per-lane slot accumulation

Moves the per-sweep f-state count tally (global accumulator and per-cell counts) into the gibbs_f_run_kernel when the decided-run path is taken. Counts come from ballots over the sampled labels and land in 64 spread atomic slots, which a later kernel (the r sparse kernel's first block or a tiny fold kernel) reduces into the accumulator. This removes the separate tally work in the pack or r pass. In exchange the f kernel does extra ballots, shared memory and atomics, and the sweep loop now runs the f pass after the tally setup.

```diff
diff --git a/fcdiff_amd/csrc/fcd_api.hip b/fcdiff_amd/csrc/fcd_api.hip
--- a/fcdiff_amd/csrc/fcd_api.hip
+++ b/fcdiff_amd/csrc/fcd_api.hip
@@ -164,6 +164,7 @@
     ctx->pt_with_rs = 0;
     ctx->acc = nullptr;
     ctx->nan_slots = nullptr;
+    ctx->f_slots = nullptr;
     ctx->dbg = nullptr;
     ctx->comm = nullptr;
     ctx->comm_world = ctx->comm_rank = 0;
@@ -199,6 +200,7 @@
     ctx->knobs.f_runs = 0;
     ctx->knobs.r_sure = 0;
     ctx->knobs.r_sure_x = 0.0;
+    ctx->knobs.tally_in_f = 0;
     ctx->knobs.partial_chunk = 0;
     ctx->knobs.tangent_chunk = 0;
     ctx->knobs.tally_in_r = (int)knob_env("FCD_TALLY_IN_R");
@@ -207,6 +209,7 @@
     ctx->n_pack = 0;
     ctx->n_pack_tally = 0;
     ctx->n_r_tally = 0;
+    ctx->n_f_tally = 0;
     ctx->n_frec_pass = ctx->n_frec_build = ctx->n_fsure_pass = ctx->n_frun_pass = 0;
     ctx->n_rsure_pass = ctx->n_rsure_build = 0;
     int rc = fcd_ws_reserve(ctx, 1u << 20);
@@ -240,6 +243,9 @@
         if (e == hipSuccess) e = hipMalloc(&ctx->acc, 8 * sizeof(unsigned long long));
         ctx->n_alloc += 1;
         if (e == hipSuccess) e = hipMemset(ctx->acc, 0, 8 * sizeof(unsigned long long));
+        if (e == hipSuccess) e = hipMalloc(&ctx->f_slots, FCD_F_SLOTS * 8 * sizeof(unsigned long long));
+        ctx->n_alloc += 1;
+        if (e == hipSuccess) e = hipMemset(ctx->f_slots, 0, FCD_F_SLOTS * 8 * sizeof(unsigned long long));
         if (e == hipSuccess) e = hipMalloc(&ctx->nan_slots, FCD_NAN_SLOTS * 16 * sizeof(unsigned long long));
         ctx->n_alloc += 1;
         if (e == hipSuccess) e = hipMemset(ctx->nan_slots, 0, FCD_NAN_SLOTS * 16 * sizeof(unsigned long long));
@@ -272,6 +278,7 @@
     if (ctx->pg_dev) (void)hipFree(ctx->pg_dev);
     if (ctx->pt_dev) (void)hipFree(ctx->pt_dev);
     if (ctx->acc) (void)hipFree(ctx->acc);
+    if (ctx->f_slots) (void)hipFree(ctx->f_slots);
     if (ctx->nan_slots) (void)hipFree(ctx->nan_slots);
     if (ctx->dbg) (void)hipFree(ctx->dbg);
     if (ctx->corr_tickets) (void)hipFree(ctx->corr_tickets);
@@ -324,6 +331,7 @@
     else if (!strcmp(name, "partial_chunk")) k.partial_chunk = (int)value;
     else if (!strcmp(name, "tangent_chunk")) k.tangent_chunk = (int)value;
     else if (!strcmp(name, "tally_in_r")) k.tally_in_r = (int)value;
+    else if (!strcmp(name, "tally_in_f")) k.tally_in_f = (int)value;
     else if (!strcmp(name, "r_keep_words")) k.r_keep_words = (int)value;
     else if (!strcmp(name, "r_poll_limit")) k.r_poll_limit = (int)value;
     else if (!strcmp(name, "r_withhold")) k.r_withhold = (int)value;
@@ -344,6 +352,7 @@
     if (!ctx) return FCD_ERR_ARG;
     if (ctx->dev_err) *ctx->dev_err = 0u;
     if (ctx->acc) FCD_HIP_TRY(hipMemset(ctx->acc, 0, 8 * sizeof(unsigned long long)));
+    if (ctx->f_slots) FCD_HIP_TRY(hipMemset(ctx->f_slots, 0, FCD_F_SLOTS * 8 * sizeof(unsigned long long)));
     if (ctx->nan_slots) FCD_HIP_TRY(hipMemset(ctx->nan_slots, 0, FCD_NAN_SLOTS * 16 * sizeof(unsigned long long)));
     if (ctx->corr_tickets && ctx->corr_tickets_n > 0)
         FCD_HIP_TRY(hipMemset(ctx->corr_tickets, 0, (size_t)ctx->corr_tickets_n * sizeof(unsigned)));
@@ -359,6 +368,7 @@
     else if (!strcmp(name, "pack_launches")) *out = ctx->n_pack;
     else if (!strcmp(name, "tally_f_in_pack")) *out = ctx->n_pack_tally;
     else if (!strcmp(name, "tally_f_in_r")) *out = ctx->n_r_tally;
+    else if (!strcmp(name, "tally_f_in_f")) *out = ctx->n_f_tally;
     else if (!strcmp(name, "tally_in_r_max_rounds")) *out = R_TALLY_MAX_ROUNDS;
     else if (!strcmp(name, "f_rec_passes")) *out = ctx->n_frec_pass;
     else if (!strcmp(name, "f_rec_builds")) *out = ctx->n_frec_build;
diff --git a/fcdiff_amd/csrc/fcd_common.h b/fcdiff_amd/csrc/fcd_common.h
--- a/fcdiff_amd/csrc/fcd_common.h
+++ b/fcdiff_amd/csrc/fcd_common.h
@@ -31,6 +31,7 @@
     int f_sure;
     int f_runs;
     int tally_in_r;
+    int tally_in_f;
     int partial_chunk;
     int tangent_chunk;
     int r_keep_words;
@@ -47,6 +48,7 @@
        FCD_KA_N = FCD_KA_EIGH + 1 };
 
 #define FCD_NAN_SLOTS 256
+#define FCD_F_SLOTS 64
 
 enum { FCD_ACC_PAIR, FCD_ACC_COUNT, FCD_ACC_COANOMALY, FCD_ACC_REGION_SET, FCD_ACC_PATIENT_GROUP, FCD_ACC_PATIENT_TRAIT, FCD_ACC_N };
 struct fcd_sweep_acc {
@@ -71,6 +73,7 @@
     long long n_pack;
     long long n_pack_tally;
     long long n_r_tally;
+    long long n_f_tally;
     long long n_frec_pass;
     long long n_frec_build;
     long long n_fsure_pass;
@@ -81,6 +84,7 @@
     void *log_tab;
     volatile unsigned *dev_err;
     void *acc;
+    void *f_slots;
     void *nan_slots;
     void *comm;
     int comm_world, comm_rank;
@@ -383,6 +387,18 @@
     return y;
 }
 
+__device__ __forceinline__ void fcd_f_slots_fold(unsigned long long *slots, unsigned long long *acc, int lane) {
+    static_assert(FCD_F_SLOTS == 64, "one line per lane");
+    unsigned long long v[3];
+#pragma unroll
+    for (int k = 0; k < 3; ++k) v[k] = atomicExch(&slots[lane * 8 + k], 0ull);
+#pragma unroll
+    for (int k = 0; k < 3; ++k) {
+        for (int o = 32; o > 0; o >>= 1) v[k] += __shfl_xor(v[k], o, 64);
+        if (lane == 0 && v[k]) (void)__hip_atomic_fetch_add(acc + 1 + k, v[k], __ATOMIC_RELAXED, __HIP_MEMORY_SCOPE_AGENT);
+    }
+}
+
 template <int WAVES>
 __device__ __forceinline__ void fcd_tally_f_block(const fcd_tally_f &a, int lin, int nblk, unsigned long long (*red)[3]) {
     const uint8_t *__restrict__ f_state = a.f_state;
@@ -581,12 +597,13 @@
     bool sentinels_in_place;
     const fcd_tally_f *tally_f;
     bool tally_f_done;
+    bool f_fold;
     bool r_flip;
     bool f_sure;
     bool f_all;
     bool r_sure;
 };
-int fcd_gibbs_f_pass(fcd_ctx *ctx, const fcd_sweep_call &c, const fcd_sweep_step &st);
+int fcd_gibbs_f_pass(fcd_ctx *ctx, const fcd_sweep_call &c, fcd_sweep_step &st);
 int fcd_gibbs_r_pass(fcd_ctx *ctx, const fcd_sweep_call &c, fcd_sweep_step &st);
 #define R_SURE_T 16.0
 #define R_SURE_X 1e-6
diff --git a/fcdiff_amd/csrc/fcd_gibbs.hip b/fcdiff_amd/csrc/fcd_gibbs.hip
--- a/fcdiff_amd/csrc/fcd_gibbs.hip
+++ b/fcdiff_amd/csrc/fcd_gibbs.hip
@@ -911,10 +911,13 @@
                                                            uint32_t chain0, uint64_t seed, uint32_t sweep, float margin,
                                                            uint2 *__restrict__ f_S, int NBLK, unsigned long long *__restrict__ dbg,
                                                            const char *__restrict__ frec, const double *__restrict__ lM, int n_tiles,
-                                                           unsigned *__restrict__ votes) {
+                                                           unsigned *__restrict__ votes, int64_t G,
+                                                           unsigned long long *__restrict__ slots, uint32_t *__restrict__ cnt_f) {
     static_assert(16 % FR_WAVES == 0, "a workgroup's chain words lie in one group of 16");
     static_assert(FR_W == R_NB && FR_W == 16 && FT_W == 4, "a run is one block of the r pass's f words: sixteen columns, four tiles");
     __shared__ uint32_t vote[FR_WAVES];
+    __shared__ uint32_t pairs[FR_WAVES][2 * FR_W];
+    const bool counting = slots != nullptr || cnt_f != nullptr;
     const int NPAIR = (U + 1) >> 1;
     const fpr_run R = fpr_locate((int)blockIdx.x, Nreg);
     const int lane = threadIdx.x & 63;
@@ -996,6 +999,22 @@
                 else K0 = (K0 & ~(3u << (2 * j))) | (k << (2 * j));
             }
         }
+        if (counting) {
+            const uint64_t act = fcd_active_mask(w, G);
+            const uint32_t nvalid = (uint32_t)__popcll(act);
+            uint32_t pair = 0;
+            if (lane < 2 * FR_W) pair = ((m1 >> lane) & 1u) ? nvalid : (((m2 >> lane) & 1u) ? nvalid << 16 : 0u);
+            uint32_t x = X;
+#pragma unroll 1
+            while (x != 0u) {
+                const int e = __builtin_ctz(x);
+                x &= x - 1u;
+                const uint32_t k = (((e >> 4) ? K1 : K0) >> (2 * (e & (FR_W - 1)))) & 3u;
+                const uint32_t n1 = (uint32_t)__popcll(__ballot(k == 1u) & act), n2 = (uint32_t)__popcll(__ballot(k == 2u) & act);
+                if (lane == e) pair = n1 | (n2 << 16);
+            }
+            if (lane < 2 * FR_W) pairs[wv][lane] = pair;
+        }
 #pragma unroll
         for (int r = 0; r < 2; ++r) {
             const int cnt = r ? R.cnt1 : R.cnt0;
@@ -1042,6 +1061,36 @@
         if (oe & (0x000F000Fu << (FT_W * q))) ot |= 1u << q;
     if (lane == 0) vote[wv] = ot;
     __syncthreads();
+    if (counting && wv == (int)(blockDim.x >> 6) - 1) {
+        const int w0 = (int)(blockIdx.y * (blockDim.x >> 6));
+        const int nwv = min((int)(blockDim.x >> 6), GW - w0);
+        const int64_t rem = G - (int64_t)w0 * 64;
+        const uint32_t nv = (uint32_t)(rem < (int64_t)nwv * 64 ? rem : (int64_t)nwv * 64);
+        uint32_t sum = 0;
+        if (present)
+            for (int q = 0; q < nwv; ++q) sum += pairs[q][lane];
+        const uint32_t ones = sum & 0xFFFFu, twos = sum >> 16;
+        if (cnt_f && present) {
+            uint32_t *ctr = cnt_f + ((lr ? R.cr1 : R.cr0) + lj) * 3;
+            const uint32_t zeros = nv - ones - twos;
+            if (zeros) (void)__hip_atomic_fetch_add(ctr + 0, zeros, __ATOMIC_RELAXED, __HIP_MEMORY_SCOPE_AGENT);
+            if (ones) (void)__hip_atomic_fetch_add(ctr + 1, ones, __ATOMIC_RELAXED, __HIP_MEMORY_SCOPE_AGENT);
+            if (twos) (void)__hip_atomic_fetch_add(ctr + 2, twos, __ATOMIC_RELAXED, __HIP_MEMORY_SCOPE_AGENT);
+        }
+        if (slots) {
+            uint32_t tot = sum;
+#pragma unroll
+            for (int o = 16; o > 0; o >>= 1) tot += (uint32_t)__shfl_xor((int)tot, o, 64);
+            if (lane == 0) {
+                unsigned long long *line = slots + ((blockIdx.x + 29u * blockIdx.y) & (FCD_F_SLOTS - 1)) * 8;
+                const unsigned long long t1 = tot & 0xFFFFu, t2 = tot >> 16;
+                const unsigned long long t0 = (unsigned long long)__popc(pm) * nv - t1 - t2;
+                if (t0) (void)__hip_atomic_fetch_add(line + 0, t0, __ATOMIC_RELAXED, __HIP_MEMORY_SCOPE_AGENT);
+                if (t1) (void)__hip_atomic_fetch_add(line + 1, t1, __ATOMIC_RELAXED, __HIP_MEMORY_SCOPE_AGENT);
+                if (t2) (void)__hip_atomic_fetch_add(line + 2, t2, __ATOMIC_RELAXED, __HIP_MEMORY_SCOPE_AGENT);
+            }
+        }
+    }
     if (wv == 0) {
         const uint32_t v = lane < (int)(blockDim.x >> 6) ? vote[lane & (FR_WAVES - 1)] : 0u;
         uint32_t bm = 0;
@@ -1580,10 +1629,11 @@
     fcd_sweep_call c = {S_B, lM, lMf, nullptr, hyper, f_state, const_cast<uint64_t *>(r_bits) , Nreg, U, G,
                         chain0, seed, FCD_EDGE_SYMMETRIC, (hipStream_t)stream};
     int rc = fcd_sweep_call_check(ctx, c, true, false, "fcd_gibbs_f_step");
-    return rc ? rc : fcd_gibbs_f_pass(ctx, c, fcd_sweep_step{sweep});
-}
-
-int fcd_gibbs_f_pass(fcd_ctx *ctx, const fcd_sweep_call &c, const fcd_sweep_step &st) {
+    fcd_sweep_step st = {sweep};
+    return rc ? rc : fcd_gibbs_f_pass(ctx, c, st);
+}
+
+int fcd_gibbs_f_pass(fcd_ctx *ctx, const fcd_sweep_call &c, fcd_sweep_step &st) {
     const fcd_sweep_plan &pl = c.pl;
     const fcd_geo &g = c.g;
     const int64_t Nreg = c.Nreg, U = c.U;
@@ -1637,11 +1687,21 @@
         if (sure && ctx->knobs.f_runs != 1 && (st.f_all || ctx->knobs.f_runs == 2)) {
             const int rw = wpb < FR_WAVES ? wpb : FR_WAVES;
             dim3 rgrid((unsigned)fpr_runs((Nreg + 1) / 2), (unsigned)((g.GW + rw - 1) / rw));
+            const fcd_tally_f *tf = nullptr;
+            if (st.tally_f && !st.tally_f_done && ctx->knobs.tally_in_f != 1 && (st.r_sure || ctx->knobs.tally_in_f == 2))
+                tf = st.tally_f;
             fcd_prof_begin(ctx, FCD_PROF_F, s);
             hipLaunchKernelGGL(gibbs_f_run_kernel, rgrid, dim3(64 * rw), 0, s, c.S_B, c.lMf, c.hyper, c.f_state, r_U, (int)Nreg, (int)U, g.C,
                                g.GW, (uint32_t)c.chain0, c.seed, (uint32_t)st.sweep, margin, f_S, NBLK, (unsigned long long *)ctx->dbg,
-                               (const char *)st.f_rec, c.lM, (int)grid.x, (unsigned *)((char *)st.f_rec + pl.frec_votes));
+                               (const char *)st.f_rec, c.lM, (int)grid.x, (unsigned *)((char *)st.f_rec + pl.frec_votes), c.G,
+                               (tf && tf->acc) ? (unsigned long long *)ctx->f_slots : nullptr, tf ? tf->cnt_f : nullptr);
             fcd_prof_end(ctx, FCD_PROF_F, s);
+            FCD_LAUNCH_CHECK();
+            if (tf) {
+                st.tally_f_done = true;
+                st.f_fold = tf->acc != nullptr;
+                ctx->n_f_tally += 1;
+            }
             ctx->n_frec_pass += 1;
             ctx->n_fsure_pass += 1;
             ctx->n_frun_pass += 1;
@@ -1900,8 +1960,6 @@
             }
         }
         st.r_sure = rs_state == 2 && st.f_packed && st.r_packed;
-        int rc = fcd_gibbs_f_pass(ctx, c, st);
-        if (rc) return rc;
         const bool last = i + 1 == n_sweeps;
         const bool do_m = mstep_every > 0 && (i + 1) % mstep_every == 0;
         const bool do_a = cnt_f && st.sweep >= accumulate_from;
@@ -1910,9 +1968,14 @@
         tf.acc = (do_m || (last && counts)) ? (unsigned long long *)ctx->acc : nullptr;
         tf.cnt_f = do_a ? cnt_f : nullptr;
         st.tally_f = (tf.acc || tf.cnt_f) ? &tf : nullptr;
+        st.tally_f_done = false;
+        st.f_fold = false;
+        int rc = fcd_gibbs_f_pass(ctx, c, st);
+        if (rc) return rc;
         rc = fcd_gibbs_r_pass(ctx, c, st);
         if (rc) {
             if (tf.acc) (void)hipMemsetAsync(ctx->acc, 0, 8 * sizeof(unsigned long long), s);
+            if (st.f_fold) (void)hipMemsetAsync(ctx->f_slots, 0, FCD_F_SLOTS * 8 * sizeof(unsigned long long), s);
             return rc;
         }
         st.sentinels_in_place = pair_form && ctx->r_form_last == 2;
diff --git a/fcdiff_amd/csrc/fcd_gibbs_r.hip b/fcdiff_amd/csrc/fcd_gibbs_r.hip
--- a/fcdiff_amd/csrc/fcd_gibbs_r.hip
+++ b/fcdiff_amd/csrc/fcd_gibbs_r.hip
@@ -1169,6 +1169,8 @@
     uint64_t *visit;
     uint32_t *fneq;
     unsigned long long *cnt;
+    unsigned long long *fold_slots;
+    unsigned long long *fold_acc;
     int Nreg, U, NBLK, GW;
     int64_t G;
     uint32_t chain0, sweep;
@@ -1274,10 +1276,15 @@
                        __ATOMIC_RELEASE, __HIP_MEMORY_SCOPE_SYSTEM);
 }
 
+__global__ __launch_bounds__(64) void gibbs_f_fold_kernel(unsigned long long *slots, unsigned long long *acc) {
+    fcd_f_slots_fold(slots, acc, (int)threadIdx.x);
+}
+
 __global__ __launch_bounds__(64 * RS_WAVES) void gibbs_r_range_kernel(const r_sparse_args a) {
     __shared__ unsigned red[2];
     if (threadIdx.x < 2) red[threadIdx.x] = 0u;
     __syncthreads();
+    if (a.fold_slots && blockIdx.x == 0 && blockIdx.y == 0 && threadIdx.x < 64) fcd_f_slots_fold(a.fold_slots, a.fold_acc, (int)threadIdx.x);
     const int lane = threadIdx.x & 63;
     const int n = __builtin_amdgcn_readfirstlane((int)(blockIdx.x * RS_WAVES + (threadIdx.x >> 6)));
     const int w = (int)blockIdx.y;
@@ -1762,8 +1769,12 @@
 }
 
 int fcd_gibbs_r_pass(fcd_ctx *ctx, const fcd_sweep_call &c, fcd_sweep_step &st) {
-    st.tally_f_done = false;
     if (ctx->dev_err && *ctx->dev_err) return fcd_fail(ctx, FCD_ERR_DEVICE, "r pass: a device-side wait was abandoned in an earlier call");
+    if (st.f_fold && !st.r_sure) {
+        hipLaunchKernelGGL(gibbs_f_fold_kernel, dim3(1), dim3(64), 0, c.s, (unsigned long long *)ctx->f_slots, (unsigned long long *)ctx->acc);
+        FCD_LAUNCH_CHECK();
+        st.f_fold = false;
+    }
     const fcd_sweep_plan &pl = c.pl;
     const fcd_geo &g = c.g;
     const int64_t Nreg = c.Nreg, U = c.U;
@@ -1814,6 +1825,8 @@
         q.mword = (const uint2 *)(ws + pl.rs_mword); q.rowflag = (const uint32_t *)(ws + pl.rs_rowflag);
         q.visit = (uint64_t *)(ws + pl.rs_visit); q.fneq = (uint32_t *)(ws + pl.rs_fneq);
         q.cnt = (unsigned long long *)ctx->dbg + 8;
+        q.fold_slots = st.f_fold ? (unsigned long long *)ctx->f_slots : nullptr;
+        q.fold_acc = (unsigned long long *)ctx->acc;
         q.Nreg = (int)Nreg; q.U = (int)U; q.NBLK = NBLK; q.GW = g.GW; q.G = c.G;
         q.chain0 = a.chain0; q.sweep = a.sweep; q.seed = a.seed;
         q.tol = a.tol;
@@ -1823,6 +1836,7 @@
         hipLaunchKernelGGL(gibbs_r_sparse_kernel, dim3((unsigned)(U * g.GW)), dim3(64), rs_walk_lds(NBLK), s, q);
         fcd_prof_end(ctx, FCD_PROF_RSTEP, s);
         FCD_LAUNCH_CHECK();
+        st.f_fold = false;
         ctx->r_form_last = 4;
         ctx->n_rsure_pass += 1;
         return FCD_OK;
@@ -1863,7 +1877,8 @@
         dim3 pgrid((unsigned)(((NBLK + fb - 1) / fb + 3) / 4), (unsigned)(Nreg + U), (unsigned)g.GW);
         fcd_tally_f tf;
         tf.f_state = nullptr; tf.C = 0; tf.G = 0; tf.GW = 0; tf.acc = nullptr; tf.cnt_f = nullptr;
-        if (st.tally_f && g.C * g.GW <= 600000) {
+        bool carried = false;
+        if (st.tally_f && !st.tally_f_done && g.C * g.GW <= 600000) {
             tf = *st.tally_f;
             const int64_t per_row = (int64_t)pgrid.x * pgrid.z;
             int64_t want = (g.C + 15) / 16;
@@ -1872,7 +1887,7 @@
             if (ty < 1) ty = 1;
             if (pgrid.y + ty <= 65535) {
                 pgrid.y += (unsigned)ty;
-                st.tally_f_done = true;
+                carried = true;
             } else {
                 tf.f_state = nullptr;
             }
@@ -1887,7 +1902,10 @@
         fcd_prof_end(ctx, FCD_PROF_PACK, s);
         FCD_LAUNCH_CHECK();
         ctx->n_pack += 1;
-        if (st.tally_f_done) ctx->n_pack_tally += 1;
+        if (carried) {
+            st.tally_f_done = true;
+            ctx->n_pack_tally += 1;
+        }
     }
     ctx->r_form_last = pipe ? 2 : 1;
     if (pipe) {
diff --git a/profiles/f_sure_cost.py b/profiles/f_sure_cost.py
--- a/profiles/f_sure_cost.py
+++ b/profiles/f_sure_cost.py
@@ -46,7 +46,7 @@
             return ctx.stat(name)
         except Exception:
             return None
-    names = ("f_rec_passes", "f_sure_passes", "f_run_passes", "f_sure_tiles", "f_sure_fallbacks", "f_repeats")
+    names = ("f_rec_passes", "f_sure_passes", "f_run_passes", "f_sure_tiles", "f_sure_fallbacks", "f_repeats", "tally_f_in_f")
     s0 = [stat(k) for k in names]
     ms = []
     sweep = 64
```

Measured after the change: 8.966 million (median of 6 runs). 6.4% higher.
